# adityabalu/DiffNet

Measured on AMD Instinct MI355X. Metric: elements*gauss_pts/sec (FEM loss+grad), higher is better.
Workload: dtype f32; 1 GPU; 2-D Poisson energy loss + gradient wrt u, Q1, 512^2 nodes, 3^2 Gauss pts, batch 64/GPU, nu+f nodal fields, Dirichlet mask on all boundary faces held as one bit per node and sample (a general mask array), fused single pass (BASELINE.json configs[1] mesh); every step evaluates the next of 4 different batches in rotation (nu, f and the mask stream from HBM with non-temporal loads; of the 4 x 67 MB of; batch_per_gpu=64, parallelism=batch-sharded x1, batches_in_rotation=4, mask_format=bits

## Files before the change

### diffnet_amd/_lib.py

```python
import ctypes as C
import os

HERE = os.path.dirname(os.path.abspath(__file__))
LIB_PATH = os.environ.get("DN_LIB_PATH") or os.path.join(HERE, "libdiffnet_hip.so")
ABI_VERSION = 10

DN_E = {-1: "DN_E_BADARG", -2: "DN_E_UNSUPPORTED", -3: "DN_E_WORKSPACE", -4: "DN_E_HANDOVER"}


class DnMesh(C.Structure):
    _fields_ = [("nsd", C.c_int32), ("degree", C.c_int32), ("ngp", C.c_int32), ("batch", C.c_int32),
                ("nx", C.c_int32), ("ny", C.c_int32), ("nz", C.c_int32),
                ("scale", C.c_float * 3), ("gpw", C.c_float * 4),
                ("basis", (C.c_float * 4) * 4), ("dbasis", (C.c_float * 4) * 4)]


class DnDirichlet(C.Structure):
    _fields_ = [("mask", C.c_void_p), ("field", C.c_void_p), ("value", C.c_float),
                ("mask_kind", C.c_int32), ("mask_batched", C.c_int32), ("field_batched", C.c_int32),
                ("box_faces", C.c_int32), ("row_words", C.c_int32)]


MASK_F32, MASK_U8, MASK_BITS, MASK_BOX = 0, 1, 2, 3
FACE_XLO, FACE_XHI, FACE_YLO, FACE_YHI, FACE_ZLO, FACE_ZHI = 1, 2, 4, 8, 16, 32


class DnPoissonArgs(C.Structure):
    _fields_ = [("u", C.c_void_p), ("nu", C.c_void_p), ("f", C.c_void_p), ("f_gp", C.c_void_p),
                ("nu_batched", C.c_int32), ("f_batched", C.c_int32),
                ("bc", DnDirichlet * 2),
                ("alpha", C.c_float), ("beta", C.c_float), ("c", C.c_float), ("wscale", C.c_float),
                ("out_scale", C.c_float),
                ("out", C.c_void_p), ("energy", C.c_void_p), ("sumsq", C.c_void_p),
                ("workspace", C.c_void_p), ("workspace_bytes", C.c_int64),
                ("energy_f32", C.c_void_p), ("energy_scale", C.c_double), ("strip_select", C.c_int32), ("accumulate_sums", C.c_int32), ("defer_sums", C.c_int32),
                ("fold_prev", C.c_void_p), ("f_is_load", C.c_int32)]


class DnFsdtArgs(C.Structure):
    _fields_ = [("w", C.c_void_p), ("phi_x", C.c_void_p), ("phi_y", C.c_void_p),
                ("bc_mask", C.c_void_p), ("mask_is_u8", C.c_int32), ("mask_batched", C.c_int32),
                ("bc_field", C.c_void_p * 3), ("bc_field_batched", C.c_int32 * 3), ("bc_value", C.c_float * 3),
                ("D11", C.c_float), ("D12", C.c_float), ("D22", C.c_float), ("D66", C.c_float), ("A44", C.c_float),
                ("A55", C.c_float), ("q", C.c_float), ("wscale", C.c_float),
                ("out", C.c_void_p * 3), ("sumsq", C.c_void_p), ("workspace", C.c_void_p), ("workspace_bytes", C.c_int64),
                ("in_scale", C.c_void_p), ("norms", C.c_void_p), ("in_num", C.c_void_p), ("in_den", C.c_void_p),
                ("defer_sums", C.c_int32), ("den_ticket", C.c_int32), ("den_workspace", C.c_void_p)]


class DnStokesArgs(C.Structure):
    _fields_ = [("u", C.c_void_p), ("v", C.c_void_p), ("p", C.c_void_p),
                ("bc_mask", C.c_void_p * 3), ("mask_is_u8", C.c_int32 * 3), ("mask_batched", C.c_int32 * 3),
                ("bc_field", C.c_void_p * 3), ("bc_field_batched", C.c_int32 * 3), ("bc_value", C.c_float * 3),
                ("f_gp", C.c_void_p * 2), ("f_batched", C.c_int32 * 2), ("f_value", C.c_float * 2),
                ("visco", C.c_float), ("pspg", C.c_float), ("wscale", C.c_float), ("transpose", C.c_int32),
                ("out", C.c_void_p * 3), ("sumsq", C.c_void_p), ("norms", C.c_void_p), ("in_num", C.c_void_p), ("in_den", C.c_void_p),
                ("workspace", C.c_void_p), ("workspace_bytes", C.c_int64)]


class DnNsArgs(C.Structure):
    _fields_ = [("u", C.c_void_p), ("v", C.c_void_p), ("p", C.c_void_p),
                ("bc_mask", C.c_void_p * 3), ("mask_is_u8", C.c_int32 * 3), ("mask_batched", C.c_int32 * 3),
                ("bc_field", C.c_void_p * 3), ("bc_field_batched", C.c_int32 * 3), ("bc_value", C.c_float * 3),
                ("f_gp", C.c_void_p * 2), ("f_batched", C.c_int32 * 2), ("f_value", C.c_float * 2),
                ("visco", C.c_float), ("wscale", C.c_float), ("tau_h", C.c_float * 2), ("cinv", C.c_float), ("vjp", C.c_int32),
                ("cot", C.c_void_p * 3),
                ("out", C.c_void_p * 3), ("sumsq", C.c_void_p), ("norms", C.c_void_p), ("in_num", C.c_void_p), ("in_den", C.c_void_p),
                ("workspace", C.c_void_p), ("workspace_bytes", C.c_int64)]


class DnTransportArgs(C.Structure):
    _fields_ = [("u", C.c_void_p), ("nu", C.c_void_p), ("nu_batched", C.c_int32), ("r_first_wins", C.c_int32),
                ("bc_mask", C.c_void_p * 2), ("mask_is_u8", C.c_int32 * 2), ("mask_batched", C.c_int32 * 2),
                ("bc_field", C.c_void_p * 2), ("bc_field_batched", C.c_int32 * 2), ("bc_value", C.c_float * 2),
                ("f_gp", C.c_void_p), ("f_batched", C.c_int32), ("f_value", C.c_float),
                ("adv", C.c_float * 2), ("kappa", C.c_float * 2), ("tau", C.c_float), ("react", C.c_float * 4), ("wscale", C.c_float),
                ("vjp", C.c_int32),
                ("cot", C.c_void_p), ("out", C.c_void_p), ("sumsq", C.c_void_p), ("norm", C.c_void_p),
                ("in_num", C.c_void_p), ("in_den", C.c_void_p), ("workspace", C.c_void_p), ("workspace_bytes", C.c_int64)]


class DnStrongformArgs(C.Structure):
    _fields_ = [("u", C.c_void_p), ("f", C.c_void_p), ("f_gp", C.c_void_p), ("f_batched", C.c_int32), ("f_value", C.c_float),
                ("bc", DnDirichlet * 2),
                ("ax", C.c_float), ("ay", C.c_float), ("b", C.c_float), ("dxx", C.c_float), ("dyy", C.c_float), ("fs", C.c_float),
                ("wscale", C.c_float), ("out_scale", C.c_float), ("d2basis", (C.c_float * 4) * 4),
                ("in_scale", C.c_void_p), ("grad", C.c_void_p), ("sum", C.c_void_p), ("workspace", C.c_void_p), ("workspace_bytes", C.c_int64)]


class DnFoslsArgs(C.Structure):
    _fields_ = [("u", C.c_void_p), ("mx", C.c_void_p), ("my", C.c_void_p), ("field_stride", C.c_int64),
                ("nu", C.c_void_p), ("nu_batched", C.c_int32), ("nu_value", C.c_float),
                ("f", C.c_void_p), ("f_gp", C.c_void_p), ("f_batched", C.c_int32), ("f_value", C.c_float),
                ("bc", DnDirichlet * 2),
                ("wq", C.c_float), ("wd", C.c_float), ("fs", C.c_float), ("wscale", C.c_float), ("out_scale", C.c_float),
                ("in_scale", C.c_void_p), ("grad_u", C.c_void_p), ("grad_mx", C.c_void_p), ("grad_my", C.c_void_p), ("grad_stride", C.c_int64),
                ("sum", C.c_void_p), ("workspace", C.c_void_p), ("workspace_bytes", C.c_int64)]


class DnHelmholtzArgs(C.Structure):
    _fields_ = [("u", C.c_void_p), ("nu", C.c_void_p), ("sigma", C.c_void_p), ("f", C.c_void_p), ("f_gp", C.c_void_p),
                ("nu_batched", C.c_int32), ("sigma_batched", C.c_int32), ("f_batched", C.c_int32),
                ("sigma_value", C.c_float), ("f_value", C.c_float),
                ("bc", DnDirichlet * 2),
                ("c", C.c_float), ("cr", C.c_float), ("fs", C.c_float), ("alpha", C.c_float), ("gamma", C.c_float), ("beta", C.c_float),
                ("wscale", C.c_float), ("out_scale", C.c_float),
                ("out", C.c_void_p), ("energy", C.c_void_p), ("sumsq", C.c_void_p), ("workspace", C.c_void_p), ("workspace_bytes", C.c_int64)]


class DnEikonalArgs(C.Structure):
    _fields_ = [("u", C.c_void_p), ("bc", DnDirichlet * 2),
                ("f", C.c_void_p), ("f_gp", C.c_void_p), ("f_batched", C.c_int32), ("f_value", C.c_float),
                ("tau", C.c_float), ("sq", C.c_float), ("wscale", C.c_float), ("vjp", C.c_int32),
                ("cot", C.c_void_p), ("in_num", C.c_void_p), ("in_den", C.c_void_p),
                ("out", C.c_void_p), ("sumsq", C.c_void_p), ("norm", C.c_void_p), ("workspace", C.c_void_p), ("workspace_bytes", C.c_int64)]


class DnCoefGradArgs(C.Structure):
    _fields_ = [("u", C.c_void_p), ("v", C.c_void_p), ("bc", DnDirichlet * 2),
                ("a_nu", C.c_float), ("a_f", C.c_float), ("wscale", C.c_float),
                ("in_scale", C.c_void_p), ("g_nu", C.c_void_p), ("g_f", C.c_void_p)]


I32x3 = C.c_int32 * 3

SYMBOLS = {
    "dn_abi_version": (C.c_int, []),
    "dn_build_info": (C.c_char_p, []),
    "dn_config_set": (C.c_int, [C.c_char_p, C.c_char_p]),
    "dn_config_get": (C.c_char_p, [C.c_char_p]),
    "dn_probe_stream": (C.c_int, [C.c_void_p, C.c_void_p, C.c_void_p, C.c_void_p, C.c_int64, C.c_int32, C.c_void_p]),
    "dn_probe_march": (C.c_int, [C.c_void_p, C.c_void_p, C.c_void_p, C.c_void_p, C.c_int32, C.c_int32, C.c_int32, C.c_int32, C.c_int32, C.c_void_p]),
    "dn_probe_tile": (C.c_int, [C.c_void_p, C.c_void_p, C.c_void_p, C.c_void_p, C.c_int32, C.c_int32, C.c_int32, C.c_int32, C.c_int32, C.c_void_p]),
    "dn_poisson_workspace_bytes": (C.c_int64, [C.POINTER(DnMesh)]),
    "dn_poisson_apply": (C.c_int, [C.POINTER(DnMesh), C.POINTER(DnPoissonArgs), C.c_void_p]),
    "dn_poisson_finish_sums": (C.c_int, [C.POINTER(DnMesh), C.POINTER(DnPoissonArgs), C.c_void_p]),
    "dn_workspace_status": (C.c_int, [C.c_void_p, C.c_void_p]),
    "dn_gauss_pt_eval_fwd": (C.c_int, [C.c_void_p, C.c_void_p, C.c_void_p, C.c_int32, C.c_int32, I32x3, C.c_int32,
                                       C.c_int32, C.c_int32, C.c_void_p]),
    "dn_gauss_pt_eval_bwd": (C.c_int, [C.c_void_p, C.c_void_p, C.c_void_p, C.c_int32, C.c_int32, I32x3, C.c_int32,
                                       C.c_int32, C.c_int32, C.c_void_p]),
    "dn_assemble": (C.c_int, [C.c_void_p, C.c_void_p, C.c_int32, C.c_int32, I32x3, C.c_int32, C.c_int32, C.c_int32,
                              C.c_void_p]),
    "dn_assemble_bwd": (C.c_int, [C.c_void_p, C.c_void_p, C.c_int32, C.c_int32, I32x3, C.c_int32, C.c_int32,
                                  C.c_void_p]),
    "dn_fdm_stencil_fwd": (C.c_int, [C.c_void_p, C.c_void_p, C.c_int32, C.c_int32, C.c_int32, C.POINTER(C.c_float), C.c_int32,
                                     C.c_float, C.c_float, C.c_void_p]),
    "dn_fdm_stencil_bwd": (C.c_int, [C.c_void_p, C.c_void_p, C.c_int32, C.c_int32, C.c_int32, C.POINTER(C.c_float), C.c_int32,
                                     C.c_float, C.c_float, C.c_void_p]),
    "dn_fdm_fused_fwd": (C.c_int, [C.c_void_p, C.c_void_p, C.c_int32, C.c_int32, C.c_int32, C.POINTER(C.c_float), C.c_int32,
                                   C.c_float, C.c_float, C.c_void_p]),
    "dn_fdm_fused_bwd": (C.c_int, [C.c_void_p, C.c_void_p, C.c_int32, C.c_int32, C.c_int32, C.POINTER(C.c_float), C.c_int32,
                                   C.c_float, C.c_float, C.c_void_p]),
    "dn_fsdt_workspace_bytes": (C.c_int64, [C.POINTER(DnMesh)]),
    "dn_fsdt_apply": (C.c_int, [C.POINTER(DnMesh), C.POINTER(DnFsdtArgs), C.c_void_p]),
    "dn_stokes_workspace_bytes": (C.c_int64, [C.POINTER(DnMesh)]),
    "dn_stokes_apply": (C.c_int, [C.POINTER(DnMesh), C.POINTER(DnStokesArgs), C.c_void_p]),
    "dn_ns_workspace_bytes": (C.c_int64, [C.POINTER(DnMesh)]),
    "dn_ns_apply": (C.c_int, [C.POINTER(DnMesh), C.POINTER(DnNsArgs), C.c_void_p]),
    "dn_transport_workspace_bytes": (C.c_int64, [C.POINTER(DnMesh)]),
    "dn_transport_apply": (C.c_int, [C.POINTER(DnMesh), C.POINTER(DnTransportArgs), C.c_void_p]),
    "dn_strongform_workspace_bytes": (C.c_int64, [C.POINTER(DnMesh)]),
    "dn_strongform_apply": (C.c_int, [C.POINTER(DnMesh), C.POINTER(DnStrongformArgs), C.c_void_p]),
    "dn_fosls_workspace_bytes": (C.c_int64, [C.POINTER(DnMesh)]),
    "dn_fosls_apply": (C.c_int, [C.POINTER(DnMesh), C.POINTER(DnFoslsArgs), C.c_void_p]),
    "dn_helmholtz_workspace_bytes": (C.c_int64, [C.POINTER(DnMesh)]),
    "dn_helmholtz_apply": (C.c_int, [C.POINTER(DnMesh), C.POINTER(DnHelmholtzArgs), C.c_void_p]),
    "dn_eikonal_workspace_bytes": (C.c_int64, [C.POINTER(DnMesh)]),
    "dn_eikonal_apply": (C.c_int, [C.POINTER(DnMesh), C.POINTER(DnEikonalArgs), C.c_void_p]),
    "dn_eikonal3d_workspace_bytes": (C.c_int64, [C.POINTER(DnMesh)]),
    "dn_eikonal3d_apply": (C.c_int, [C.POINTER(DnMesh), C.POINTER(DnEikonalArgs), C.c_void_p]),
    "dn_poisson_coef_grad": (C.c_int, [C.POINTER(DnMesh), C.POINTER(DnCoefGradArgs), C.c_void_p]),
    "dn_upconv_out_workspace_bytes": (C.c_int64, [C.c_int64, C.c_int64, C.c_int64, C.c_int64]),
    "dn_upconv_out_fwd": (C.c_int, [C.c_void_p, C.c_void_p, C.c_void_p, C.c_void_p, C.c_int64, C.c_int64, C.c_int64, C.c_int64, C.c_int,
                                    C.c_void_p, C.c_int64, C.c_void_p]),
    "dn_upconv_out_bwd": (C.c_int, [C.c_void_p, C.c_void_p, C.c_void_p, C.c_void_p, C.c_void_p, C.c_void_p, C.c_void_p, C.c_int64,
                                    C.c_int64, C.c_int64, C.c_int64, C.c_int, C.c_void_p, C.c_int64, C.c_void_p]),
    "dn_upconv3d_out_workspace_bytes": (C.c_int64, [C.c_int64] * 5),
    "dn_upconv3d_out_fwd": (C.c_int, [C.c_void_p, C.c_void_p, C.c_void_p, C.c_void_p, C.c_int64, C.c_int64, C.c_int64, C.c_int64, C.c_int64,
                                      C.c_int, C.c_void_p, C.c_int64, C.c_void_p]),
    "dn_upconv3d_out_bwd": (C.c_int, [C.c_void_p, C.c_void_p, C.c_void_p, C.c_void_p, C.c_void_p, C.c_void_p, C.c_void_p, C.c_int64,
                                      C.c_int64, C.c_int64, C.c_int64, C.c_int64, C.c_int, C.c_void_p, C.c_int64, C.c_void_p]),
    "dn_conv3d_k4s2_wrw_workspace_bytes": (C.c_int64, [C.c_int64] * 6),
    "dn_conv3d_k4s2_wrw": (C.c_int, [C.c_void_p, C.c_void_p, C.c_void_p, C.c_int64, C.c_int64, C.c_int64, C.c_int64, C.c_int64, C.c_int64,
                                     C.c_void_p, C.c_int64, C.c_void_p]),
    "dn_conv2d_k4s2_down": (C.c_int, [C.c_void_p, C.c_void_p, C.c_void_p] + [C.c_int64] * 5 + [C.c_void_p]),
    "dn_conv2d_k4s2_up": (C.c_int, [C.c_void_p, C.c_void_p, C.c_void_p] + [C.c_int64] * 5 + [C.c_void_p]),
    "dn_conv2d_k4s2_wrw_workspace_bytes": (C.c_int64, [C.c_int64] * 5),
    "dn_conv2d_k4s2_wrw": (C.c_int, [C.c_void_p, C.c_void_p, C.c_void_p] + [C.c_int64] * 5 + [C.c_void_p, C.c_int64, C.c_void_p]),
    "dn_conv3d_k4s2_down": (C.c_int, [C.c_void_p, C.c_void_p, C.c_void_p] + [C.c_int64] * 6 + [C.c_void_p]),
    "dn_conv3d_k4s2_up": (C.c_int, [C.c_void_p, C.c_void_p, C.c_void_p] + [C.c_int64] * 6 + [C.c_void_p]),
    "dn_conv3d_k4s2_workspace_bytes": (C.c_int64, [C.c_int32] + [C.c_int64] * 6),
    "dn_conv3d_k4s2_down_ws": (C.c_int, [C.c_void_p, C.c_void_p, C.c_void_p] + [C.c_int64] * 6 + [C.c_void_p, C.c_int64, C.c_void_p]),
    "dn_conv3d_k4s2_up_ws": (C.c_int, [C.c_void_p, C.c_void_p, C.c_void_p] + [C.c_int64] * 6 + [C.c_void_p, C.c_int64, C.c_void_p]),
    "dn_conv2d_valid_fwd": (C.c_int, [C.c_void_p] * 4 + [C.c_int64] * 6 + [C.c_void_p]),
    "dn_conv2d_valid_bwd_data": (C.c_int, [C.c_void_p] * 3 + [C.c_int64] * 6 + [C.c_void_p]),
    "dn_conv2d_valid_bwd_weight": (C.c_int, [C.c_void_p] * 4 + [C.c_int64] * 6 + [C.c_void_p]),
    "dn_instnorm_workspace_bytes": (C.c_int64, [C.c_int64, C.c_int64]),
    "dn_instnorm_act_fwd": (C.c_int, [C.c_void_p, C.c_void_p, C.c_void_p, C.c_void_p, C.c_int64, C.c_int64, C.c_float, C.c_float,
                                      C.c_void_p, C.c_int64, C.c_void_p]),
    "dn_instnorm_act_bwd": (C.c_int, [C.c_void_p, C.c_void_p, C.c_void_p, C.c_void_p, C.c_void_p, C.c_int64, C.c_int64, C.c_float,
                                      C.c_int64, C.c_int64, C.c_void_p, C.c_int64, C.c_void_p]),
    "dn_pack_mask_bits": (C.c_int, [C.c_void_p, C.c_int32, C.c_int64, C.c_int32, C.c_int32, C.c_void_p, C.c_void_p]),
    "dn_unpack_mask_bits": (C.c_int, [C.c_void_p, C.c_int64, C.c_int32, C.c_int32, C.c_void_p, C.c_void_p]),
    "dn_winding_nodes": (C.c_int, [C.c_void_p, C.c_void_p, C.c_void_p, C.c_void_p, C.c_int32, C.c_int32, C.c_int32, C.c_int32,
                                   C.c_void_p]),
}

_LIB = None


class DiffNetHipError(RuntimeError):
    pass


def lib():
    global _LIB
    if _LIB is not None:
        return _LIB
    if not os.path.exists(LIB_PATH):
        raise DiffNetHipError(
            f"{LIB_PATH} is missing: build it with `python -m diffnet_amd.build` (hipcc, gfx950). "
            "There is no CPU fallback for the FEM hot path.")
    try:
        h = C.CDLL(LIB_PATH)
    except OSError as e:
        raise DiffNetHipError(f"cannot load {LIB_PATH}: {e}") from e
    for name, (res, args) in SYMBOLS.items():
        try:
            fn = getattr(h, name)
        except AttributeError as e:
            raise DiffNetHipError(f"{LIB_PATH} does not export {name}; rebuild it") from e
        fn.restype = res
        fn.argtypes = args
    v = h.dn_abi_version()
    if v != ABI_VERSION:
        raise DiffNetHipError(f"ABI mismatch: library {v}, binding {ABI_VERSION}")
    _LIB = h
    return h


_HIP = None


def hip_runtime():
    global _HIP
    if _HIP is None:
        path = next((ln.split()[-1] for ln in open("/proc/self/maps") if "libamdhip64.so" in ln), None)
        if path is None:
            raise DiffNetHipError("the HIP runtime is not loaded in this process (no GPU build of torch?)")
        h = C.CDLL(path)
        h.hipEventCreateWithFlags.argtypes = [C.POINTER(C.c_void_p), C.c_uint]
        h.hipEventRecord.argtypes = [C.c_void_p, C.c_void_p]
        h.hipStreamWaitEvent.argtypes = [C.c_void_p, C.c_void_p, C.c_uint]
        h.hipEventSynchronize.argtypes = [C.c_void_p]
        h.hipEventDestroy.argtypes = [C.c_void_p]
        _HIP = h
    return _HIP


def new_event():
    e = C.c_void_p()
    rc = hip_runtime().hipEventCreateWithFlags(C.byref(e), C.c_uint(0x2 | 0x20000000))
    if rc != 0:
        raise DiffNetHipError(f"hipEventCreateWithFlags: hipError_t {rc}")
    return e


def check(rc, what):
    if rc == 0:
        return
    if rc < 0:
        if rc == -4:
            raise DiffNetHipError(f"{what}: DN_E_HANDOVER (a chained-strip launch ran a bounded LDS hand-over poll to its limit: its results are NaN)")
        raise DiffNetHipError(f"{what}: {DN_E.get(rc, rc)} (argument not supported by the HIP kernels)")
    raise DiffNetHipError(f"{what}: hipError_t {rc}")


CONFIG_MIRROR = {k[3:]: v for k, v in os.environ.items() if k.startswith("DN_")}


def config_set(key, value):
    rc = lib().dn_config_set(key.encode(), (value or "").encode())
    if rc != 0:
        raise DiffNetHipError(f"dn_config_set: unknown switch {key!r} or value too long")
    CONFIG_MIRROR[key] = value or ""
    import sys
    ops = sys.modules.get(__package__ + ".ops")
    if ops is not None:
        ops.call_cache_clear()


def config_get(key):
    v = lib().dn_config_get(key.encode())
    if v is None:
        raise DiffNetHipError(f"dn_config_get: unknown switch {key!r}")
    return v.decode()
```

### diffnet_amd/csrc/dn_api.hip

```cpp
#include <cstdlib>
#include <cstring>

#include "dn_reduce.h"

#define DN_STR2(x) #x
#define DN_STR(x) DN_STR2(x)

extern "C" int dn_abi_version(void) { return DN_ABI_VERSION; }

extern "C" const char* dn_build_info(void) {
    return "libdiffnet_hip abi " DN_STR(DN_ABI_VERSION) " target gfx950 (CDNA4, wave64) hip " DN_STR(HIP_VERSION_MAJOR) "." DN_STR(
        HIP_VERSION_MINOR) " built " __DATE__;
}

namespace {
const char* const kKeys[dn::CFG_COUNT] = {"PLAN2D", "PLAN3D", "PLAN_FSDT", "Q1_RULE_KERNEL", "GPE_GATHER", "GPE_TILED", "Q1_3D_T16", "Q1_3D_E1SUM", "FSDT_GENERIC", "Q1_3D_E1", "HANDOVER_SPIN_LIMIT", "CONV2D_V1", "CONV_WRW_WGS", "Q1_3D_N2", "FSDT_FORM"};
constexpr int kHostCount = 1;
const char* const kHostKeys[kHostCount] = {"COEF_GRAD"};
constexpr int kAllCount = dn::CFG_COUNT + kHostCount;
char g_cfg[kAllCount][64];

const char* key_name(int k) { return k < dn::CFG_COUNT ? kKeys[k] : kHostKeys[k - dn::CFG_COUNT]; }

int key_index(const char* key) {
    if (!key) return -1;
    for (int k = 0; k < kAllCount; ++k)
        if (std::strcmp(key, key_name(k)) == 0) return k;
    return -1;
}

struct ConfigInit {
    ConfigInit() {
        for (int k = 0; k < kAllCount; ++k) {
            char name[80] = "DN_";
            std::strncat(name, key_name(k), sizeof(name) - 4);
            const char* e = std::getenv(name);
            g_cfg[k][0] = 0;
            if (e && std::strlen(e) < sizeof(g_cfg[k])) std::strcpy(g_cfg[k], e);
        }
    }
} g_cfg_init;
}

namespace dn {
const char* config(ConfigKey k) { return g_cfg[k][0] ? g_cfg[k] : nullptr; }
}

extern "C" int dn_config_set(const char* key, const char* value) {
    const int k = key_index(key);
    if (k < 0) return DN_E_BADARG;
    if (value && std::strlen(value) >= sizeof(g_cfg[k])) return DN_E_BADARG;
    g_cfg[k][0] = 0;
    if (value) std::strcpy(g_cfg[k], value);
    return 0;
}

extern "C" const char* dn_config_get(const char* key) {
    const int k = key_index(key);
    return k < 0 ? nullptr : g_cfg[k];
}

extern "C" int dn_workspace_status(void* workspace, void* stream) {
    if (!workspace) return DN_E_BADARG;
    hipStream_t s = reinterpret_cast<hipStream_t>(stream);
    unsigned* word = reinterpret_cast<unsigned*>(workspace) + dn::DN_WS_ERRWORD;
    unsigned v = 0u;
    hipError_t e = hipMemcpyAsync(&v, word, sizeof(v), hipMemcpyDeviceToHost, s);
    if (e == hipSuccess) e = hipStreamSynchronize(s);
    if (e != hipSuccess) return (int)e;
    if (v == 0u) return 0;
    e = hipMemsetAsync(word, 0, sizeof(v), s);
    if (e == hipSuccess) e = hipStreamSynchronize(s);
    if (e != hipSuccess) return (int)e;
    return DN_E_HANDOVER;
}

namespace dn {
__global__ void __launch_bounds__(256) pack_mask_bits_kernel(const void* __restrict__ mask, int is_u8, long long rows, int nx, int row_words,
                                                             uint32_t* __restrict__ bits) {
    const long long w = (long long)blockIdx.x * blockDim.x + threadIdx.x;
    if (w >= rows * row_words) return;
    const long long row = w / row_words;
    const int x0 = (int)(w % row_words) * 32;
    uint32_t v = 0u;
    for (int i = 0; i < 32 && x0 + i < nx; ++i) {
        const long long idx = row * nx + x0 + i;
        const bool set = is_u8 ? reinterpret_cast<const uint8_t*>(mask)[idx] != 0 : reinterpret_cast<const float*>(mask)[idx] > 0.5f;
        v |= set ? (1u << i) : 0u;
    }
    bits[w] = v;
}
__global__ void __launch_bounds__(256) unpack_mask_bits_kernel(const uint32_t* __restrict__ bits, long long rows, int nx, int row_words,
                                                               uint8_t* __restrict__ mask) {
    const long long i = (long long)blockIdx.x * blockDim.x + threadIdx.x;
    if (i >= rows * nx) return;
    const long long row = i / nx;
    const int x = (int)(i % nx);
    mask[i] = (uint8_t)((bits[row * row_words + (x >> 5)] >> (x & 31)) & 1u);
}
}

extern "C" int dn_pack_mask_bits(const void* mask, int32_t mask_kind, int64_t rows, int32_t nx, int32_t row_words, uint32_t* bits, void* stream) {
    if (!mask || !bits || rows < 0 || nx < 1 || row_words < (nx + 31) / 32 || (mask_kind != DN_MASK_F32 && mask_kind != DN_MASK_U8)) return DN_E_BADARG;
    const long long n = (long long)rows * row_words;
    if (n == 0) return 0;
    if ((n + 255) / 256 >= (1ll << 31)) return DN_E_UNSUPPORTED;
    hipLaunchKernelGGL(dn::pack_mask_bits_kernel, dim3((unsigned)((n + 255) / 256)), dim3(256), 0, reinterpret_cast<hipStream_t>(stream), mask,
                       (int)(mask_kind == DN_MASK_U8), (long long)rows, (int)nx, (int)row_words, bits);
    DN_LAUNCH_CHECK();
    return 0;
}

extern "C" int dn_unpack_mask_bits(const uint32_t* bits, int64_t rows, int32_t nx, int32_t row_words, uint8_t* mask_u8, void* stream) {
    if (!mask_u8 || !bits || rows < 0 || nx < 1 || row_words < (nx + 31) / 32) return DN_E_BADARG;
    const long long n = (long long)rows * nx;
    if (n == 0) return 0;
    if ((n + 255) / 256 >= (1ll << 31)) return DN_E_UNSUPPORTED;
    hipLaunchKernelGGL(dn::unpack_mask_bits_kernel, dim3((unsigned)((n + 255) / 256)), dim3(256), 0, reinterpret_cast<hipStream_t>(stream), bits,
                       (long long)rows, (int)nx, (int)row_words, mask_u8);
    DN_LAUNCH_CHECK();
    return 0;
}
```

### diffnet_amd/csrc/dn_common.h

```cpp
#pragma once
#include <hip/hip_runtime.h>
#include <stdint.h>

#include "../../include/diffnet_hip.h"

#define DN_WAVE 64

#define DN_LAUNCH_CHECK()                         \
    do {                                          \
        hipError_t e__ = hipGetLastError();       \
        if (e__ != hipSuccess) return (int)e__;   \
    } while (0)

namespace dn {

enum ConfigKey : int { CFG_PLAN2D = 0, CFG_PLAN3D, CFG_PLAN_FSDT, CFG_Q1_RULE_KERNEL, CFG_GPE_GATHER, CFG_GPE_TILED, CFG_Q1_3D_T16, CFG_Q1_3D_E1SUM, CFG_FSDT_GENERIC, CFG_Q1_3D_E1, CFG_HANDOVER_SPIN_LIMIT, CFG_CONV2D_V1, CFG_CONV_WRW_WGS, CFG_Q1_3D_N2, CFG_FSDT_FORM, CFG_COUNT };
const char* config(ConfigKey k);

__device__ __forceinline__ double wave_sum(double v) {
#pragma unroll
    for (int off = DN_WAVE / 2; off > 0; off >>= 1) v += __shfl_down(v, off, DN_WAVE);
    return v;
}

__device__ __forceinline__ double block_sum(double v, double* scratch, int tid, int nthreads) {
    v = wave_sum(v);
    const int lane = tid & (DN_WAVE - 1), wave = tid / DN_WAVE;
    if (lane == 0) scratch[wave] = v;
    __syncthreads();
    double r = 0.0;
    if (tid == 0) {
        const int nw = (nthreads + DN_WAVE - 1) / DN_WAVE;
        for (int w = 0; w < nw; ++w) r += scratch[w];
    }
    __syncthreads();
    return r;
}

__device__ __forceinline__ void block_sum2(double& a, double& b, double* scratch, int tid, int nthreads) {
    a = wave_sum(a);
    b = wave_sum(b);
    const int lane = tid & (DN_WAVE - 1), wave = tid / DN_WAVE;
    const int nw = (nthreads + DN_WAVE - 1) / DN_WAVE;
    if (lane == 0) { scratch[wave] = a; scratch[nw + wave] = b; }
    __syncthreads();
    double ra = 0.0, rb = 0.0;
    if (tid == 0) {
        for (int w = 0; w < nw; ++w) { ra += scratch[w]; rb += scratch[nw + w]; }
    }
    __syncthreads();
    a = ra; b = rb;
}

template <int N>
struct VecT;
template <>
struct VecT<1> { using type = float; };
template <>
struct VecT<2> { using type = float2; };
template <>
struct VecT<4> { using type = float4; };

#ifndef DN_NT_STORES
#define DN_NT_STORES 0
#endif
template <typename V, typename T>
__device__ __forceinline__ V ld_at(const T* __restrict__ base, unsigned index) {
    return *reinterpret_cast<const V*>(reinterpret_cast<const char*>(base) + (index * (unsigned)sizeof(T)));
}
template <typename V, typename T>
__device__ __forceinline__ void st_at(T* __restrict__ base, unsigned index, const V& v) {
#if DN_NT_STORES
    char* a = reinterpret_cast<char*>(base) + (index * (unsigned)sizeof(T));
    if constexpr (sizeof(V) == 16) {
        typedef float v4f __attribute__((ext_vector_type(4)));
        __builtin_nontemporal_store(__builtin_bit_cast(v4f, v), reinterpret_cast<v4f*>(a));
    } else if constexpr (sizeof(V) == 8) {
        typedef float v2f __attribute__((ext_vector_type(2)));
        __builtin_nontemporal_store(__builtin_bit_cast(v2f, v), reinterpret_cast<v2f*>(a));
    } else {
        __builtin_nontemporal_store(v, reinterpret_cast<V*>(a));
    }
#else
    *reinterpret_cast<V*>(reinterpret_cast<char*>(base) + (index * (unsigned)sizeof(T))) = v;
#endif
}

template <int NW, bool VEC, typename T>
__device__ __forceinline__ void load_seg(const T* __restrict__ base, unsigned rowoff, int x0, int nx, T (&dst)[NW + 1]) {
    if constexpr (VEC && (NW == 2 || NW == 4)) {
        const unsigned xl = (unsigned)min(x0, nx - NW);
        if constexpr (sizeof(T) == 4) {
            using V = typename VecT<NW>::type;
            const V v = ld_at<V>(base, rowoff + xl);
            const T* vf = reinterpret_cast<const T*>(&v);
#pragma unroll
            for (int k = 0; k < NW; ++k) dst[k] = vf[k];
        } else {
            static_assert(sizeof(T) == 1, "load_seg: 1- or 4-byte elements");
            if constexpr (NW == 4) {
                const uint32_t w = ld_at<uint32_t>(base, rowoff + xl);
#pragma unroll
                for (int k = 0; k < 4; ++k) dst[k] = (T)((w >> (8 * k)) & 0xffu);
            } else {
                const uint16_t w = ld_at<uint16_t>(base, rowoff + xl);
                dst[0] = (T)(w & 0xffu);
                dst[1] = (T)(w >> 8);
            }
        }
    } else {
#pragma unroll
        for (int k = 0; k < NW; ++k) dst[k] = ld_at<T>(base, rowoff + (unsigned)min(x0 + k, nx - 1));
    }
    dst[NW] = ld_at<T>(base, rowoff + (unsigned)min(x0 + NW, nx - 1));
}

template <int NW, bool VEC, typename T>
__device__ __forceinline__ void load_seg_stream(const T* __restrict__ base, unsigned rowoff, int x0, int nx, T (&dst)[NW + 1]) {
    if constexpr (VEC && NW == 4 && sizeof(T) == 4) {
        typedef T v4t __attribute__((ext_vector_type(4)));
        const unsigned xl = (unsigned)min(x0, nx - NW);
        const v4t v = __builtin_nontemporal_load(reinterpret_cast<const v4t*>(reinterpret_cast<const char*>(base) + (rowoff + xl) * 4u));
        dst[0] = v.x; dst[1] = v.y; dst[2] = v.z; dst[3] = v.w;
        dst[NW] = ld_at<T>(base, rowoff + (unsigned)min(x0 + NW, nx - 1));
    } else if constexpr (VEC && NW == 4 && sizeof(T) == 1) {
        const unsigned xl = (unsigned)min(x0, nx - NW);
        const uint32_t w = __builtin_nontemporal_load(reinterpret_cast<const uint32_t*>(reinterpret_cast<const char*>(base) + (rowoff + xl)));
#pragma unroll
        for (int k = 0; k < 4; ++k) dst[k] = (T)((w >> (8 * k)) & 0xffu);
        dst[NW] = ld_at<T>(base, rowoff + (unsigned)min(x0 + NW, nx - 1));
    } else {
        load_seg<NW, VEC>(base, rowoff, x0, nx, dst);
    }
}

template <int NW, bool VEC, typename T>
__device__ __forceinline__ void load_own(const T* __restrict__ base, unsigned rowoff, int x0, int nx, T (&dst)[NW]) {
    if constexpr (VEC && (NW == 2 || NW == 4)) {
        const unsigned xl = (unsigned)min(x0, nx - NW);
        if constexpr (sizeof(T) == 4) {
            using V = typename VecT<NW>::type;
            const V v = ld_at<V>(base, rowoff + xl);
            const T* vf = reinterpret_cast<const T*>(&v);
#pragma unroll
            for (int k = 0; k < NW; ++k) dst[k] = vf[k];
        } else {
            if constexpr (NW == 4) {
                const uint32_t w = ld_at<uint32_t>(base, rowoff + xl);
#pragma unroll
                for (int k = 0; k < 4; ++k) dst[k] = (T)((w >> (8 * k)) & 0xffu);
            } else {
                const uint16_t w = ld_at<uint16_t>(base, rowoff + xl);
                dst[0] = (T)(w & 0xffu);
                dst[1] = (T)(w >> 8);
            }
        }
    } else {
#pragma unroll
        for (int k = 0; k < NW; ++k) dst[k] = ld_at<T>(base, rowoff + (unsigned)min(x0 + k, nx - 1));
    }
}

template <int NW, bool VEC>
__device__ __forceinline__ void store_seg(float* __restrict__ base, unsigned rowoff, int x0, int nx, const float (&src)[NW]) {
    if constexpr (VEC && (NW == 2 || NW == 4)) {
        if (x0 + NW <= nx) {
            using V = typename VecT<NW>::type;
            V v;
            float* vf = reinterpret_cast<float*>(&v);
#pragma unroll
            for (int k = 0; k < NW; ++k) vf[k] = src[k];
            st_at<V>(base, rowoff + (unsigned)x0, v);
        }
    } else {
#pragma unroll
        for (int k = 0; k < NW; ++k)
            if (x0 + k < nx) st_at<float>(base, rowoff + (unsigned)(x0 + k), src[k]);
    }
}

}
```

### diffnet_amd/csrc/poisson2d_q1_cf.hip

```cpp
#include <cstdlib>
#include <type_traits>

#define DN_NT_STORES 1
#include "poisson_common.h"

namespace dn {

enum : int { CF_NU = 1, CF_F = 2, CF_BC = 8, CF_BC_U8C = 16, CF_BC_PACKED = 32, CF_PK_NB1 = 64, CF_PK_NB2 = 128, CF_UA = 256, CF_ONE = 512 };

template <int E>
struct CfRow {
    float u[E + 1], n[E + 1], f[E + 1];
    float g[E + 1];
    float du[E], pn[E];
    float keep[E];
    float keepx;
    BcRaw<E> bc;
    uint32_t m8[2][2];
    uint32_t mb[2];
    uint32_t bx[2];
};

constexpr int CF_W = 4;
constexpr int CF_TS = 128;
constexpr int CF_NSLOT = 64;
constexpr unsigned CF_SPIN_MAX = 1u << 20;

__device__ __forceinline__ unsigned lds_addr(const void* p) { return (unsigned)(uintptr_t)(__attribute__((address_space(3))) const void*)p; }
__device__ __forceinline__ void lds_st(unsigned a, float v) { asm volatile("ds_write_b32 %0, %1" ::"v"(a), "v"(v) : "memory"); }
__device__ __forceinline__ void lds_st(unsigned a, unsigned v) { asm volatile("ds_write_b32 %0, %1" ::"v"(a), "v"(v) : "memory"); }
__device__ __forceinline__ void lds_ld_nowait(float& d, unsigned a) { asm volatile("ds_read_b32 %0, %1" : "=v"(d) : "v"(a) : "memory"); }
__device__ __forceinline__ unsigned lds_ld_u(unsigned a) {
    unsigned d;
    asm volatile("ds_read_b32 %0, %1\n\ts_waitcnt lgkmcnt(0)" : "=v"(d) : "v"(a) : "memory");
    return d;
}
__device__ __forceinline__ float lds_ld(unsigned a) {
    float d;
    asm volatile("ds_read_b32 %0, %1\n\ts_waitcnt lgkmcnt(0)" : "=v"(d) : "v"(a) : "memory");
    return d;
}
template <int N>
__device__ __forceinline__ void lds_wait(float (&v)[N]) {
    if constexpr (N == 5) asm volatile("s_waitcnt lgkmcnt(0)" : "+v"(v[0]), "+v"(v[1]), "+v"(v[2]), "+v"(v[3]), "+v"(v[4])::"memory");
    else if constexpr (N == 4) asm volatile("s_waitcnt lgkmcnt(0)" : "+v"(v[0]), "+v"(v[1]), "+v"(v[2]), "+v"(v[3])::"memory");
    else if constexpr (N == 3) asm volatile("s_waitcnt lgkmcnt(0)" : "+v"(v[0]), "+v"(v[1]), "+v"(v[2])::"memory");
    else if constexpr (N == 2) asm volatile("s_waitcnt lgkmcnt(0)" : "+v"(v[0]), "+v"(v[1])::"memory");
    else { static_assert(N == 1, "lds_wait: 1..5 values"); asm volatile("s_waitcnt lgkmcnt(0)" : "+v"(v[0])::"memory"); }
}

template <int E, bool VEC, int FL, int W>
__global__ void __launch_bounds__(W > 1 ? CF_TS * W : 256, W > 1 ? 4 : 2) poisson2d_q1_cf_kernel(const PoissonParams p) {
    constexpr int NW = E;
    constexpr bool HAS_NU = (FL & CF_NU) != 0, HAS_F = (FL & CF_F) != 0;
    constexpr bool BC_ANY = (FL & (CF_BC | CF_BC_U8C | CF_BC_PACKED)) != 0, BC_U8C = (FL & CF_BC_U8C) != 0, BC_PACKED = (FL & CF_BC_PACKED) != 0;
    constexpr bool UA = (FL & CF_UA) != 0, ONE = (FL & CF_ONE) != 0;
    static_assert(!ONE || ((BC_PACKED || BC_U8C) && (FL & CF_PK_NB2) == 0), "CF_ONE: one packed or uint8-constant condition");
    static_assert(!UA || (E == 4 && VEC && W == 1), "CF_UA: four elements per thread, vector accesses, one strip per workgroup");
    const int T = W > 1 ? CF_TS : (int)blockDim.x;
    const int sub = W > 1 ? __builtin_amdgcn_readfirstlane((int)threadIdx.x / CF_TS) : 0;
    const int tid = W > 1 ? (int)threadIdx.x - sub * CF_TS : (int)threadIdx.x;
    const int chunk = blockIdx.x, strip = W > 1 ? (int)blockIdx.y * W + sub : selected_strip(p, (int)blockIdx.y), b = blockIdx.z;
    const bool active = W == 1 || strip < p.nstrips;
    const bool chain_dn = W > 1 && sub > 0;
    const bool chain_up = W > 1 && sub + 1 < W && strip + 1 < p.nstrips;
    const int q = chunk * (T - 1) + tid;
    const int ex0 = q * E;
    const int x0 = ex0;
    const bool col_owner = !(chunk > 0 && tid == 0);
    const bool lastcol = UA && x0 + NW == p.nx - 1;
    const int64_t nps = (int64_t)p.nx * p.ny;
    const SampleBases sb = sample_bases(p, b, nps);
    const int R = p.rows_per_strip;
    const int sb0 = strip * R, sc0 = min(sb0 + R, p.nely);
    const int ey_begin = (sb0 > 0 && !chain_dn) ? sb0 - 1 : sb0;
    const int ey_end = sc0;
    const int r_from = sb0;
    const int e_from = sb0, e_until = p.nely;
    const bool top_row = sc0 == p.nely;

    __shared__ float xch[2][256];
    __shared__ double red[W > 1 ? 4 * W : 8];
    __shared__ int last_flag;
    constexpr int CW = W > 1 ? W : 2, SEAM_WORDS = 6 * (E + 1);
    __shared__ float cf_edge[W > 1 ? W : 1][W > 1 ? CF_NSLOT : 1];
    __shared__ unsigned cf_xflag[W > 1 ? W : 1];
    __shared__ float cf_seam[CW - 1][W > 1 ? SEAM_WORDS : 1][W > 1 ? CF_TS : 1];
    __shared__ unsigned cf_sflag[CW - 1][2][2];
    const int lane = tid & 63, wv = __builtin_amdgcn_readfirstlane(tid >> 6);
    unsigned seq = 0u;
    if constexpr (W > 1) {
        static_assert(CF_TS == 128, "two waves per sub-strip");
        if (threadIdx.x < (unsigned)W) cf_xflag[threadIdx.x] = 0u;
        if (threadIdx.x < 4u * (W - 1)) (&cf_sflag[0][0][0])[threadIdx.x] = 0u;
        __syncthreads();
    }
    if ((blockIdx.x | blockIdx.y | blockIdx.z) == 0u) fold_prev_sums(p, (int)threadIdx.x, (int)blockDim.x, red);
    float spin_poison = 0.f;
    auto spin_until = [&](const unsigned* flag, unsigned want) {
        const unsigned fa = lds_addr(flag);
        const unsigned lim = p.spin_limit > 0 ? (unsigned)p.spin_limit : CF_SPIN_MAX;
        unsigned n = 0;
        for (; n < lim; ++n) {
            if ((unsigned)__builtin_amdgcn_readfirstlane((int)lds_ld_u(fa)) >= want) break;
            __builtin_amdgcn_s_sleep(1);
        }
        if (n == lim) spin_poison = __builtin_nanf("");
    };

    const bool has_mask[2] = {sb.mask[0] != nullptr, sb.mask[1] != nullptr};
    const uint8_t* mask8[2];
    mask8[0] = reinterpret_cast<const uint8_t*>(has_mask[0] ? sb.mask[0] : sb.mask[1]);
    mask8[1] = reinterpret_cast<const uint8_t*>(has_mask[1] ? sb.mask[1] : sb.mask[0]);

    constexpr unsigned NBITS = (1u << (NW + 1)) - 1u;
    constexpr int NB = !BC_PACKED ? 0 : ((FL & CF_PK_NB2) ? 2 : ((FL & CF_PK_NB1) ? 1 : 0));
    const bool isbits[2] = {p.bc[0].kind == DN_MASK_BITS, p.bc[1].kind == DN_MASK_BITS};
    const unsigned bsel[2] = {isbits[0] ? NBITS : 0u, isbits[1] ? NBITS : 0u};
    const int src0 = (NB == 2 || isbits[0]) ? 0 : 1;
    const int kone = p.bc[0].kind >= 0 ? 0 : 1;
    const uint32_t* bptr[2] = {reinterpret_cast<const uint32_t*>(sb.mask[src0]), reinterpret_cast<const uint32_t*>(sb.mask[1])};
    const unsigned brow[2] = {(unsigned)p.bc[src0].row_bytes / 4u, (unsigned)p.bc[1].row_bytes / 4u};
    unsigned bw0[2], bw1[2];
#pragma unroll
    for (int j = 0; j < 2; ++j) {
        const int rw = max((int)brow[j], 1);
        bw0[j] = (unsigned)min(x0 >> 5, rw - 1);
        bw1[j] = (unsigned)min((x0 >> 5) + 1, rw - 1);
    }
    const unsigned bsh = (unsigned)x0 & 31u;
    unsigned boxx[2] = {0u, 0u};
#pragma unroll
    for (int k = 0; k < 2; ++k) {
        const int faces = p.bc[k].kind == DN_MASK_BOX ? p.bc[k].box_faces : 0;
#pragma unroll
        for (int n = 0; n <= NW; ++n) {
            const bool on = ((faces & DN_FACE_XLO) && x0 + n == 0) || ((faces & DN_FACE_XHI) && x0 + n == p.nx - 1);
            boxx[k] |= on ? (1u << n) : 0u;
        }
    }
    const int ylo[2] = {(p.bc[0].kind == DN_MASK_BOX && (p.bc[0].box_faces & DN_FACE_YLO)) ? 0 : -1,
                        (p.bc[1].kind == DN_MASK_BOX && (p.bc[1].box_faces & DN_FACE_YLO)) ? 0 : -1};
    const int yhi[2] = {(p.bc[0].kind == DN_MASK_BOX && (p.bc[0].box_faces & DN_FACE_YHI)) ? p.ny - 1 : -1,
                        (p.bc[1].kind == DN_MASK_BOX && (p.bc[1].box_faces & DN_FACE_YHI)) ? p.ny - 1 : -1};
    auto packed_issue = [&](int yc, CfRow<E>& r) {
#pragma unroll
        for (int j = 0; j < NB; ++j) {
            const unsigned ro = (unsigned)yc * brow[j];
            const uint32_t w0 = ld_at<uint32_t>(bptr[j], ro + bw0[j]), w1 = ld_at<uint32_t>(bptr[j], ro + bw1[j]);
            r.mb[j] = __builtin_amdgcn_alignbit(w1, w0, bsh);
        }
        if constexpr (ONE) {
            if constexpr (NB == 0) r.bx[0] = (yc == (kone ? ylo[1] : ylo[0]) || yc == (kone ? yhi[1] : yhi[0])) ? NBITS : (kone ? boxx[1] : boxx[0]);
        } else {
#pragma unroll
            for (int k = 0; k < 2; ++k) r.bx[k] = (yc == ylo[k] || yc == yhi[k]) ? NBITS : boxx[k];
        }
    };

    auto row_issue = [&](int yr, CfRow<E>& r) {
        const int yp = min(yr, p.ny - 1);
        const unsigned rowoff = (unsigned)yp * (unsigned)p.nx;
        load_seg<NW, VEC>(sb.u, rowoff, x0, p.nx, r.u);
        if constexpr (HAS_NU) load_seg_stream<NW, VEC>(sb.nu, rowoff, x0, p.nx, r.n);
        if constexpr (HAS_F) load_seg_stream<NW, VEC>(sb.f, rowoff, x0, p.nx, r.f);
        if constexpr (BC_PACKED) {
            packed_issue(yp, r);
        } else if constexpr (BC_U8C && ONE) {
            uint8_t t[NW + 1];
            load_seg_stream<NW, VEC>(mask8[0], rowoff, x0, p.nx, t);
            uint32_t w = 0u;
#pragma unroll
            for (int n = 0; n < NW; ++n) w |= (uint32_t)t[n] << (8 * n);
            r.m8[0][0] = w;
            r.m8[0][1] = t[NW];
        } else if constexpr (BC_U8C) {
#pragma unroll
            for (int k = 0; k < 2; ++k) {
                if (has_mask[k]) {
                    uint8_t t[NW + 1];
                    load_seg_stream<NW, VEC>(mask8[k], rowoff, x0, p.nx, t);
                    uint32_t w = 0u;
#pragma unroll
                    for (int n = 0; n < NW; ++n) w |= (uint32_t)t[n] << (8 * n);
                    r.m8[k][0] = w;
                    r.m8[k][1] = t[NW];
                }
            }
        } else if constexpr (BC_ANY) {
            bc_issue<NW, VEC>(p, sb, rowoff, x0, r.bc);
        }
    };
    auto row_bc = [&](CfRow<E>& r) {
#pragma unroll
        for (int n = 0; n < NW; ++n) r.keep[n] = 1.f;
        if constexpr (UA) r.keepx = 1.f;
        if constexpr ((BC_PACKED || BC_U8C) && ONE) {
            const float v = kone ? p.bc[1].value : p.bc[0].value;
            unsigned b = 0u;
            if constexpr (BC_PACKED) b = NB == 1 ? r.mb[0] : r.bx[0];
#pragma unroll
            for (int n = 0; n <= NW; ++n) {
                bool set;
                if constexpr (BC_PACKED) set = (b & (1u << n)) != 0u;
                else set = n < NW ? ((r.m8[0][0] >> (8 * n)) & 0xffu) != 0u : r.m8[0][1] != 0u;
                r.u[n] = set ? v : r.u[n];
                if (n < NW) r.keep[n] = set ? 0.f : 1.f;
                else if constexpr (UA) r.keepx = set ? 0.f : 1.f;
            }
        } else if constexpr (BC_PACKED) {
            unsigned b0 = r.bx[0], b1 = r.bx[1];
            if constexpr (NB == 2) { b0 |= r.mb[0] & bsel[0]; b1 |= r.mb[1] & bsel[1]; }
            if constexpr (NB == 1) { b0 |= r.mb[0] & bsel[0]; b1 |= r.mb[0] & bsel[1]; }
            const float v0 = p.bc[0].value, v1 = p.bc[1].value;
#pragma unroll
            for (int n = 0; n <= NW; ++n) {
                r.u[n] = (b0 & (1u << n)) ? v0 : r.u[n];
                r.u[n] = (b1 & (1u << n)) ? v1 : r.u[n];
                if (n < NW) r.keep[n] = ((b0 | b1) & (1u << n)) ? 0.f : 1.f;
            }
            if constexpr (UA) r.keepx = ((b0 | b1) & (1u << NW)) ? 0.f : 1.f;
        } else if constexpr (BC_U8C) {
#pragma unroll
            for (int k = 0; k < 2; ++k) {
                if (has_mask[k]) {
                    const float val = p.bc[k].value;
#pragma unroll
                    for (int n = 0; n <= NW; ++n) {
                        const bool set = has_mask[k] && (n < NW ? ((r.m8[k][0] >> (8 * n)) & 0xffu) != 0u : r.m8[k][1] != 0u);
                        r.u[n] = set ? val : r.u[n];
                        if (n < NW) r.keep[n] = set ? 0.f : r.keep[n];
                        else if constexpr (UA) r.keepx = set ? 0.f : r.keepx;
                    }
                }
            }
        } else if constexpr (BC_ANY) {
            if constexpr (UA) {
                float k5[NW + 1];
                bc_apply_all<NW>(p, sb, r.bc, r.u, k5);
#pragma unroll
                for (int n = 0; n < NW; ++n) r.keep[n] = k5[n];
                r.keepx = k5[NW];
            } else {
                bc_apply<NW>(p, sb, r.bc, r.u, r.keep);
            }
        }
    };

    float e1_acc = 0.f, e2_acc = 0.f, sq_acc = 0.f;
    int par = 0;

    float pend_v[NW];
    unsigned pend_row = 0u;
    bool pend_st = false;
    float pend_x = 0.f;
    auto flush_store = [&]() {
        if (pend_st) store_seg<NW, VEC>(sb.out, pend_row, x0, p.nx, pend_v);
        if constexpr (UA) {
            if (pend_st && lastcol) st_at<float>(sb.out, pend_row + (unsigned)(p.nx - 1), pend_x);
        }
        pend_st = false;
    };
    auto emit_row = [&](const float (&o)[NW + 1], const float (&keep)[NW], int yr, bool owned_row, float keepx = 1.f) {
        float left;
        if constexpr (W > 1) {
            const float up = __shfl_up(o[NW], 1, 64);
            const unsigned ea = lds_addr(&cf_edge[sub][seq & (CF_NSLOT - 1)]);
            float edge = 0.f;
            if (wv == 0) {
                if (lane == 63) { lds_st(ea, o[NW]); lds_st(lds_addr(&cf_xflag[sub]), seq + 1u); }
            } else {
                spin_until(&cf_xflag[sub], seq + 1u);
                edge = lds_ld(ea);
            }
            left = lane > 0 ? up : edge;
            ++seq;
        } else {
            xch[par][tid] = o[NW];
            asm volatile("s_waitcnt lgkmcnt(0)\n\ts_barrier" ::: "memory");
            left = (tid > 0) ? xch[par][tid - 1] : 0.f;
            par ^= 1;
        }
        const bool st = owned_row && col_owner && (!UA || x0 + NW <= p.nx - 1);
#pragma unroll
        for (int n = 0; n < NW; ++n) {
            const float t = (o[n] + (n == 0 ? left : 0.f)) * keep[n];
            sq_acc = st ? fmaf(t, t, sq_acc) : sq_acc;
            pend_v[n] = t * p.out_scale;
            if constexpr (W > 1) pend_v[n] += spin_poison;
        }
        if constexpr (UA) {
            const float t = o[NW] * keepx;
            sq_acc = (st && lastcol) ? fmaf(t, t, sq_acc) : sq_acc;
            pend_x = t * p.out_scale;
        }
        pend_row = (unsigned)yr * (unsigned)p.nx;
        pend_st = st && sb.out != nullptr;
        flush_store();
    };

    const float mx0 = p.T.mxs[0], mx1 = p.T.mxs[1], mx2 = p.T.mxs[2], mx3 = p.T.mxs[3];
    const float my0 = p.T.m[0], my1 = p.T.m[1], my2 = p.T.m[2], my3 = p.T.m[3];
    const float k0 = p.T.q1c[0], k1 = p.T.q1c[1], h0 = p.T.q1c[2], h1 = p.T.q1c[3], nb = -p.T.beta;
    constexpr bool ROWSTAGED = (FL & CF_BC) == 0, STAGE_DU = W == 1;
    const float xm[4] = {p.T.q1xm[0], p.T.q1xm[1], p.T.q1xm[2], p.T.q1xm[3]}, ym[4] = {p.T.q1ym[0], p.T.q1ym[1], p.T.q1ym[2], p.T.q1ym[3]};
    const float px0 = p.T.q1px[0], px1 = p.T.q1px[1], sy0 = p.T.q1sy[0], sy1 = p.T.q1sy[1];

    constexpr bool FMASS = HAS_F && ROWSTAGED;
    const float cx00 = p.T.q1mx[0], cx01 = p.T.q1mx[1], cx11 = p.T.q1mx[2], cy00 = p.T.q1my[0], cy01 = p.T.q1my[1], cy11 = p.T.q1my[2];
    const float alpha = p.T.alpha;
    auto fstage = [&](CfRow<E>& r) {
        if constexpr (FMASS) {
#pragma unroll
            for (int n = 0; n <= NW; ++n) r.g[n] = 0.f;
#pragma unroll
            for (int e = 0; e < E; ++e) {
                if (ex0 + e < p.nelx) {
                    r.g[e] = fmaf(cx01, r.f[e + 1], fmaf(cx00, r.f[e], r.g[e]));
                    r.g[e + 1] = fmaf(cx11, r.f[e + 1], cx01 * r.f[e]);
                }
            }
        }
    };

    auto sstage = [&](CfRow<E>& r) {
        if constexpr (ROWSTAGED) {
#pragma unroll
            for (int e = 0; e < E; ++e) {
                if constexpr (HAS_NU) {
                    q1cf_stage(px0, px1, r.u[e], r.u[e + 1], r.n[e], r.n[e + 1], r.du[e], r.pn[e]);
                } else {
                    r.du[e] = r.u[e + 1] - r.u[e];
                    r.pn[e] = mx0;
                }
            }
        }
    };

    auto layer = [&](auto fresh, int ey, const CfRow<E>& L, CfRow<E>& U, const float (&cin)[NW + 1], float (&cout)[NW + 1]) {
        const bool own_layer = ey >= e_from && ey <= e_until;
        const float cnt = (own_layer && col_owner) ? 1.f : 0.f;
        if constexpr (decltype(fresh)::value) { row_bc(U); fstage(U); }
        sstage(U);
        float o[NW + 1], le1 = 0.f, le2 = 0.f;
#pragma unroll
        for (int n = 0; n <= NW; ++n) { o[n] = cin[n]; cout[n] = 0.f; }
        if constexpr (FMASS) {
#pragma unroll
            for (int n = 0; n <= NW; ++n) {
                const float tlo = fmaf(cy01, U.g[n], cy00 * L.g[n]), tup = fmaf(cy11, U.g[n], cy01 * L.g[n]);
                o[n] = fmaf(nb, tlo, o[n]);
                cout[n] = nb * tup;
                le2 = fmaf(U.u[n], tup, fmaf(L.u[n], tlo, le2));
            }
        }
        if constexpr (ROWSTAGED) {
            float V[NW + 1], S[NW + 1];
#pragma unroll
            for (int n = 0; n <= NW; ++n) {
                V[n] = U.u[n] - L.u[n];
                S[n] = HAS_NU ? fmaf(sy1, U.n[n], sy0 * L.n[n]) : my0;
            }
#pragma unroll
            for (int e = 0; e < E; ++e) {
                if (ex0 + e < p.nelx) {
                    const float a = STAGE_DU ? L.du[e] : L.u[e + 1] - L.u[e], b = STAGE_DU ? U.du[e] : U.u[e + 1] - U.u[e];
                    q1cf_elem(xm, ym, a, b, L.pn[e], U.pn[e], V[e], V[e + 1], S[e], S[e + 1], alpha, o[e], o[e + 1], cout[e], cout[e + 1], le1);
                }
            }
        } else {
#pragma unroll
            for (int e = 0; e < E; ++e) {
                if (ex0 + e < p.nelx) {
                    const float U0 = L.u[e], UX = L.u[e + 1] - L.u[e], UY = U.u[e] - L.u[e], UXY = (U.u[e + 1] - U.u[e]) - UX;
                    float P = mx0, Q = 0.f, Pp = my0, Qp = 0.f;
                    if constexpr (HAS_NU) {
                        const float N0 = L.n[e], NX = L.n[e + 1] - N0, NY = U.n[e] - N0, NXY = (U.n[e + 1] - U.n[e]) - NX;
                        P = fmaf(mx1, NX, mx0 * N0);
                        Q = fmaf(mx1, NXY, mx0 * NY);
                        Pp = fmaf(my1, NY, my0 * N0);
                        Qp = fmaf(my1, NXY, my0 * NX);
                    }
                    const float A0 = fmaf(Q, my1, P * my0), A1 = fmaf(Q, my2, P * my1), A2 = fmaf(Q, my3, P * my2);
                    const float B0 = fmaf(Qp, mx1, Pp * mx0), B1 = fmaf(Qp, mx2, Pp * mx1), B2 = fmaf(Qp, mx3, Pp * mx2);
                    const float tX0 = fmaf(UXY, A1, UX * A0), tX1 = fmaf(UXY, A2, UX * A1);
                    const float tY0 = fmaf(UXY, B1, UY * B0), tY1 = fmaf(UXY, B2, UY * B1);
                    le1 += fmaf(h1, fmaf(UXY, tY1, UY * tY0), h0 * fmaf(UXY, tX1, UX * tX0));
                    float cU0 = 0.f, cUX = k0 * tX0, cUY = k1 * tY0, cUXY = fmaf(k0, tX1, k1 * tY1);
                    if constexpr (HAS_F) {
                        const float F0 = L.f[e], FX = L.f[e + 1] - F0, FY = U.f[e] - F0, FXY = (U.f[e + 1] - U.f[e]) - FX;
                        const float S0 = fmaf(mx1, FX, mx0 * F0), S1 = fmaf(mx1, FXY, mx0 * FY);
                        const float T0 = fmaf(mx2, FX, mx1 * F0), T1 = fmaf(mx2, FXY, mx1 * FY);
                        const float L0 = fmaf(my1, S1, my0 * S0), LX = fmaf(my1, T1, my0 * T0);
                        const float LY = fmaf(my2, S1, my1 * S0), LXY = fmaf(my2, T1, my1 * T0);
                        le2 += fmaf(LXY, UXY, fmaf(LY, UY, fmaf(LX, UX, L0 * U0)));
                        cU0 = nb * L0;
                        cUX = fmaf(nb, LX, cUX);
                        cUY = fmaf(nb, LY, cUY);
                        cUXY = fmaf(nb, LXY, cUXY);
                    }
                    const float g01 = cUX - cUXY, g10 = cUY - cUXY;
                    o[e] += (cU0 - cUX) - g10;
                    o[e + 1] += g01;
                    cout[e] += g10;
                    cout[e + 1] += cUXY;
                }
            }
        }
        e1_acc = fmaf(cnt, le1, e1_acc);
        e2_acc = fmaf(cnt, le2, e2_acc);
        if (W > 1 && chain_dn && ey == sb0) {
            const unsigned s0 = lds_addr(&cf_seam[W > 1 ? sub - 1 : 0][0][tid]);
#pragma unroll
            for (int n = 0; n <= NW; ++n) lds_st(s0 + (4 * NW + 4 + n) * CF_TS * 4, o[n]);
#pragma unroll
            for (int n = 0; n < NW; ++n) lds_st(s0 + (5 * NW + 5 + n) * CF_TS * 4, L.keep[n]);
        } else {
            emit_row(o, L.keep, ey, ey >= r_from, L.keepx);
        }
    };
    auto publish_row = [&](const CfRow<E>& r) {
        const unsigned s0 = lds_addr(&cf_seam[W > 1 ? sub - 1 : 0][0][tid]);
#pragma unroll
        for (int n = 0; n <= NW; ++n) {
            lds_st(s0 + n * CF_TS * 4, r.u[n]);
            if constexpr (HAS_NU) lds_st(s0 + (NW + 1 + n) * CF_TS * 4, r.n[n]);
            if constexpr (FMASS) lds_st(s0 + (2 * NW + 2 + n) * CF_TS * 4, r.g[n]);
            else if constexpr (HAS_F) lds_st(s0 + (2 * NW + 2 + n) * CF_TS * 4, r.f[n]);
        }
        if (lane == 0) lds_st(lds_addr(&cf_sflag[W > 1 ? sub - 1 : 0][0][wv]), 1u);
    };
    auto fetch_row = [&](CfRow<E>& r) {
        spin_until(&cf_sflag[sub][0][wv], 1u);
        const unsigned s0 = lds_addr(&cf_seam[sub][0][tid]);
#pragma unroll
        for (int n = 0; n <= NW; ++n) lds_ld_nowait(r.u[n], s0 + n * CF_TS * 4);
        lds_wait(r.u);
        if constexpr (HAS_NU) {
#pragma unroll
            for (int n = 0; n <= NW; ++n) lds_ld_nowait(r.n[n], s0 + (NW + 1 + n) * CF_TS * 4);
            lds_wait(r.n);
        }
        if constexpr (FMASS) {
#pragma unroll
            for (int n = 0; n <= NW; ++n) lds_ld_nowait(r.g[n], s0 + (2 * NW + 2 + n) * CF_TS * 4);
            lds_wait(r.g);
        } else if constexpr (HAS_F) {
#pragma unroll
            for (int n = 0; n <= NW; ++n) lds_ld_nowait(r.f[n], s0 + (2 * NW + 2 + n) * CF_TS * 4);
            lds_wait(r.f);
        }
    };
    auto publish_carry = [&](const float (&c)[NW + 1]) {
        const unsigned s0 = lds_addr(&cf_seam[sub][0][tid]);
#pragma unroll
        for (int n = 0; n <= NW; ++n) lds_st(s0 + (3 * NW + 3 + n) * CF_TS * 4, c[n]);
        if (lane == 0) lds_st(lds_addr(&cf_sflag[sub][1][wv]), 1u);
    };

    auto set_prio = [&](int e) {
        switch (((ey_end - e) >> 1) & 3) {
            case 0: __builtin_amdgcn_s_setprio(0); break;
            case 1: __builtin_amdgcn_s_setprio(1); break;
            case 2: __builtin_amdgcn_s_setprio(2); break;
            default: __builtin_amdgcn_s_setprio(3); break;
        }
    };

    constexpr std::true_type FRESH{};
    constexpr std::false_type LANDED{};
    if (active) {
    CfRow<E> RA, RB;
    float carryA[NW + 1], carryB[NW + 1];
#pragma unroll
    for (int n = 0; n <= NW; ++n) carryA[n] = carryB[n] = 0.f;
    row_issue(ey_begin, RA);
    row_bc(RA);
    fstage(RA);
    sstage(RA);
    if constexpr (W > 1) {
        if (chain_dn) publish_row(RA);
    }
    int ey = ey_begin;
    bool odd = false;
    const int n_main = chain_up ? ey_end - 1 : ey_end;
    for (; ey + 1 < n_main; ey += 2) {
        set_prio(ey);
        row_issue(ey + 1, RB);
        layer(FRESH, ey, RA, RB, carryA, carryB);
        row_issue(ey + 2, RA);
        layer(FRESH, ey + 1, RB, RA, carryB, carryA);
    }
    if (ey < n_main) {
        set_prio(ey);
        row_issue(ey + 1, RB);
        layer(FRESH, ey, RA, RB, carryA, carryB);
        odd = true;
        ++ey;
    }
    if constexpr (W > 1) {
        if (chain_up) {
            __builtin_amdgcn_s_setprio(0);
            if (odd) { fetch_row(RA); layer(LANDED, ey, RB, RA, carryB, carryA); publish_carry(carryA); }
            else { fetch_row(RB); layer(LANDED, ey, RA, RB, carryA, carryB); publish_carry(carryB); }
        }
    }
    if (top_row) {
        float o[NW + 1], keep[NW];
#pragma unroll
        for (int n = 0; n <= NW; ++n) o[n] = odd ? carryB[n] : carryA[n];
#pragma unroll
        for (int n = 0; n < NW; ++n) keep[n] = odd ? RB.keep[n] : RA.keep[n];
        emit_row(o, keep, p.ny - 1, true, odd ? RB.keepx : RA.keepx);
        flush_store();
    }
    if constexpr (W > 1) {
        if (chain_dn) {
            spin_until(&cf_sflag[sub - 1][1][wv], 1u);
            const unsigned s0 = lds_addr(&cf_seam[sub - 1][0][tid]);
            float o[NW + 1], cy[NW + 1], keep[NW];
#pragma unroll
            for (int n = 0; n <= NW; ++n) lds_ld_nowait(o[n], s0 + (4 * NW + 4 + n) * CF_TS * 4);
            lds_wait(o);
#pragma unroll
            for (int n = 0; n <= NW; ++n) lds_ld_nowait(cy[n], s0 + (3 * NW + 3 + n) * CF_TS * 4);
            lds_wait(cy);
#pragma unroll
            for (int n = 0; n < NW; ++n) lds_ld_nowait(keep[n], s0 + (5 * NW + 5 + n) * CF_TS * 4);
            lds_wait(keep);
#pragma unroll
            for (int n = 0; n <= NW; ++n) o[n] += cy[n];
            emit_row(o, keep, sb0, true);
            flush_store();
        }
    }
    }

    if constexpr (W > 1) {
        e1_acc += spin_poison;
        sq_acc += spin_poison;
        if (spin_poison != spin_poison && p.counter != nullptr && (threadIdx.x & 63u) == 0u) atomicOr(p.counter + DN_WS_ERRWORD, 1u);
    }
    if (p.want_sums) finish_sums(p, e1_acc, e2_acc, sq_acc, (int)threadIdx.x, (int)blockDim.x, red, &last_flag);
}

template <int E, bool VEC, int FL>
static void cf_launch_one(const PoissonParams& pp, const Geom2D& g, int batch, hipStream_t s) {
    if constexpr (E == 4 && VEC && (FL & CF_UA) == 0) {
        if (g.W == CF_W) {
            hipLaunchKernelGGL((poisson2d_q1_cf_kernel<E, VEC, FL, CF_W>), dim3(g.chunks, (g.strips + CF_W - 1) / CF_W, batch),
                               dim3(CF_TS * CF_W), 0, s, pp);
            return;
        }
    }
    hipLaunchKernelGGL((poisson2d_q1_cf_kernel<E, VEC, FL, 1>), dim3(g.chunks, g.strips, batch), dim3(g.T), 0, s, pp);
}

template <int E, bool VEC, int UAF = 0>
static void cf_launch_flags(const PoissonParams& pp, const Geom2D& g, int batch, hipStream_t s) {
    const bool any = pp.bc[0].kind >= 0 || pp.bc[1].kind >= 0;
    bool u8c = any, packed = false;
    for (int k = 0; k < 2; ++k) {
        if (pp.bc[k].kind >= 0 && (!pp.bc[k].mask_is_u8 || pp.bc[k].field)) u8c = false;
        if (pp.bc[k].kind == DN_MASK_BITS || pp.bc[k].kind == DN_MASK_BOX) packed = true;
    }
    const int nbits = (pp.bc[0].kind == DN_MASK_BITS) + (pp.bc[1].kind == DN_MASK_BITS);
    const bool one = (pp.bc[0].kind >= 0) != (pp.bc[1].kind >= 0);
    const int nf = (pp.nu ? CF_NU : 0) | (pp.f ? CF_F : 0);
#define DN_CF(FLAGS)                                                                         \
    (!any ? cf_launch_one<E, VEC, (FLAGS) | UAF>(pp, g, batch, s)                                  \
          : packed ? (nbits == 2 ? cf_launch_one<E, VEC, (FLAGS) | UAF | CF_BC_PACKED | CF_PK_NB2>(pp, g, batch, s)          \
                     : nbits == 1 ? (one ? cf_launch_one<E, VEC, (FLAGS) | UAF | CF_BC_PACKED | CF_PK_NB1 | CF_ONE>(pp, g, batch, s)        \
                                         : cf_launch_one<E, VEC, (FLAGS) | UAF | CF_BC_PACKED | CF_PK_NB1>(pp, g, batch, s))        \
                     : one ? cf_launch_one<E, VEC, (FLAGS) | UAF | CF_BC_PACKED | CF_ONE>(pp, g, batch, s)                   \
                           : cf_launch_one<E, VEC, (FLAGS) | UAF | CF_BC_PACKED>(pp, g, batch, s))                   \
          : u8c ? (one ? cf_launch_one<E, VEC, (FLAGS) | UAF | CF_BC_U8C | CF_ONE>(pp, g, batch, s)                \
                       : cf_launch_one<E, VEC, (FLAGS) | UAF | CF_BC_U8C>(pp, g, batch, s))                \
                : cf_launch_one<E, VEC, (FLAGS) | UAF | CF_BC>(pp, g, batch, s))
    switch (nf) {
        case 0: DN_CF(0); break;
        case CF_NU: DN_CF(CF_NU); break;
        case CF_F: DN_CF(CF_F); break;
        default: DN_CF(CF_NU | CF_F); break;
    }
#undef DN_CF
}

int poisson2d_q1_cf_chain() { return CF_W; }

int launch_poisson2d_q1_cf(const PoissonParams& pp, const Geom2D& g, int batch, bool vec, hipStream_t s) {
    if (g.W > 1 && !(g.W == poisson2d_q1_cf_chain() && g.E == 4 && vec && g.T == CF_TS && g.R + 3 <= CF_NSLOT)) return DN_E_BADARG;
    if (g.ua) {
        if (g.E != 4 || g.W != 1 || (pp.nx & 3) != 1 || pp.nx < 9) return DN_E_BADARG;
        cf_launch_flags<4, true, CF_UA>(pp, g, batch, s);
        return 0;
    }
    if (g.E == 4 && vec) { cf_launch_flags<4, true>(pp, g, batch, s); return 0; }
    if (g.E == 2 && vec) { cf_launch_flags<2, true>(pp, g, batch, s); return 0; }
    if (g.E == 2) { cf_launch_flags<2, false>(pp, g, batch, s); return 0; }
    return DN_E_UNSUPPORTED;
}

}
```

### diffnet_amd/csrc/poisson_common.h

```cpp
#pragma once
#include "dn_reduce.h"
#include "poisson_elem.h"

namespace dn {

struct DirichletDev {
    const void* mask;
    const float* field;
    float value;
    int mask_is_u8, mask_batched, field_batched;
    int kind;
    int box_faces;
    int row_bytes;
};

struct PoissonParams {
    ElemTab T;
    const float* u;
    const float* nu;
    const float* f;
    const float* fgp;
    int nu_batched, f_batched;
    int f_is_load;
    DirichletDev bc[2];
    float out_scale;
    float* out;
    double* part_energy;
    double* part_sumsq;
    unsigned* counter;
    double* energy;
    double* sumsq;
    float* energy_f32;
    double energy_scale;
    int nx, ny, nz;
    int nelx, nely, nelz;
    int rows_per_strip;
    int nstrips;
    int strip_sel;
    int acc_sums;
    int defer_sums;
    int want_sums;
    const double* fold_pe;
    const double* fold_ps;
    double* fold_energy;
    double* fold_sumsq;
    float* fold_energy_f32;
    double fold_scale;
    int fold_n, fold_acc;
    int spin_limit;
};

__device__ __forceinline__ void write_sums(double e, double s, int acc, double* energy, double* sumsq, float* energy_f32, double energy_scale) {
    if (acc) { e += *energy; s += *sumsq; }
    if (energy) *energy = e;
    if (sumsq) *sumsq = s;
    if (energy_f32) *energy_f32 = (float)(e * energy_scale);
}

__device__ __forceinline__ int selected_strip(const PoissonParams& p, int idx) {
    return p.strip_sel == 1 ? (idx == 0 ? 0 : p.nstrips - 1) : (p.strip_sel == 2 ? idx + 1 : idx);
}

struct SampleBases {
    const float* u;
    const float* nu;
    const float* f;
    float* out;
    const void* mask[2];
    const float* field[2];
};

__device__ __forceinline__ SampleBases sample_bases(const PoissonParams& p, int b, int64_t nps) {
    SampleBases s;
    s.u = p.u + (int64_t)b * nps;
    s.nu = p.nu ? p.nu + (p.nu_batched ? (int64_t)b * nps : 0) : nullptr;
    s.f = p.f ? p.f + (p.f_batched ? (int64_t)b * nps : 0) : nullptr;
    s.out = p.out ? p.out + (int64_t)b * nps : nullptr;
#pragma unroll
    for (int k = 0; k < 2; ++k) {
        const DirichletDev& d = p.bc[k];
        const int64_t mo = d.mask_batched ? (int64_t)b * nps : 0;
        if (d.kind == DN_MASK_BITS)
            s.mask[k] = reinterpret_cast<const uint8_t*>(d.mask) + (d.mask_batched ? (int64_t)b * ((int64_t)p.ny * p.nz) * d.row_bytes : 0);
        else
            s.mask[k] = d.mask ? (d.mask_is_u8 ? (const void*)(reinterpret_cast<const uint8_t*>(d.mask) + mo)
                                               : (const void*)(reinterpret_cast<const float*>(d.mask) + mo))
                               : nullptr;
        s.field[k] = d.field ? d.field + (d.field_batched ? (int64_t)b * nps : 0) : nullptr;
    }
    return s;
}

template <int NW, bool VEC>
__device__ __forceinline__ unsigned load_apply_bc(const PoissonParams& p, const SampleBases& sb, unsigned rowoff, int x0,
                                                  float (&u)[NW + 1]) {
    uint8_t m8[2][NW + 1];
    float mf[2][NW + 1], fv[2][NW + 1];
#pragma unroll
    for (int k = 0; k < 2; ++k) {
        if (sb.mask[k] != nullptr) {
            if (p.bc[k].mask_is_u8) load_seg<NW, VEC>(reinterpret_cast<const uint8_t*>(sb.mask[k]), rowoff, x0, p.nx, m8[k]);
            else load_seg<NW, VEC>(reinterpret_cast<const float*>(sb.mask[k]), rowoff, x0, p.nx, mf[k]);
            if (sb.field[k]) load_seg<NW, VEC>(sb.field[k], rowoff, x0, p.nx, fv[k]);
        }
    }
    unsigned bits = 0u;
#pragma unroll
    for (int k = 0; k < 2; ++k) {
        if (sb.mask[k] != nullptr) {
            unsigned kb = 0u;
            if (p.bc[k].mask_is_u8) {
#pragma unroll
                for (int n = 0; n <= NW; ++n) kb |= (m8[k][n] != 0) ? (1u << n) : 0u;
            } else {
#pragma unroll
                for (int n = 0; n <= NW; ++n) kb |= (mf[k][n] > 0.5f) ? (1u << n) : 0u;
            }
            if (sb.field[k]) {
#pragma unroll
                for (int n = 0; n <= NW; ++n) u[n] = (kb & (1u << n)) ? fv[k][n] : u[n];
            } else {
                const float val = p.bc[k].value;
#pragma unroll
                for (int n = 0; n <= NW; ++n) u[n] = (kb & (1u << n)) ? val : u[n];
            }
            bits |= kb;
        }
    }
    return bits;
}

__device__ __forceinline__ void finish_sums(const PoissonParams& p, float e1, float e2, float sq, int tid, int nthreads,
                                            double* red, int* flag, double escale = 1.0) {
    double mine[2] = {escale * ((double)p.T.c * (double)e1 - (double)e2), (double)sq}, tot[2];
    block_sum2(mine[0], mine[1], red, tid, nthreads);
    double* const part[2] = {p.part_energy, p.part_sumsq};
    if (p.defer_sums) {
        if (tid == 0) store_partials<2, false>(part, workgroup_index(), mine);
        return;
    }
    if (!last_arriver_sums<2, 16, true, false>(part, p.counter, mine, tid, nthreads, flag, tot)) return;
    block_sum2(tot[0], tot[1], red, tid, nthreads);
    if (tid == 0) {
        write_sums(tot[0], tot[1], p.acc_sums, p.energy, p.sumsq, p.energy_f32, p.energy_scale);
        arrival_reset(p.counter);
    }
}

__device__ __forceinline__ void fold_prev_sums(const PoissonParams& p, int tid, int nthreads, double* red) {
    if (p.fold_n <= 0) return;
    const double* const part[2] = {p.fold_pe, p.fold_ps};
    double tot[2];
    sum_partials<2, 16, false, false>(part, p.fold_n, tid, nthreads, tot);
    block_sum2(tot[0], tot[1], red, tid, nthreads);
    if (tid == 0) write_sums(tot[0], tot[1], p.fold_acc, p.fold_energy, p.fold_sumsq, p.fold_energy_f32, p.fold_scale);
}

template <int NW>
struct BcRaw {
    uint32_t m[2][NW + 1];
    float fv[2][NW + 1];
};

template <int NW, bool VEC>
__device__ __forceinline__ void bc_issue(const PoissonParams& p, const SampleBases& sb, unsigned rowoff, int x0, BcRaw<NW>& r) {
#pragma unroll
    for (int k = 0; k < 2; ++k) {
        if (sb.mask[k] != nullptr) {
            if (p.bc[k].mask_is_u8) {
                uint8_t t[NW + 1];
                load_seg_stream<NW, VEC>(reinterpret_cast<const uint8_t*>(sb.mask[k]), rowoff, x0, p.nx, t);
#pragma unroll
                for (int n = 0; n <= NW; ++n) r.m[k][n] = t[n];
            } else {
                load_seg_stream<NW, VEC>(reinterpret_cast<const uint32_t*>(sb.mask[k]), rowoff, x0, p.nx, r.m[k]);
            }
            if (sb.field[k]) load_seg<NW, VEC>(sb.field[k], rowoff, x0, p.nx, r.fv[k]);
        }
    }
}

template <int NW>
__device__ __forceinline__ void bc_apply_all(const PoissonParams& p, const SampleBases& sb, const BcRaw<NW>& r, float (&u)[NW + 1],
                                             float (&keep)[NW + 1]) {
#pragma unroll
    for (int n = 0; n <= NW; ++n) keep[n] = 1.f;
#pragma unroll
    for (int k = 0; k < 2; ++k) {
        if (sb.mask[k] != nullptr) {
            const bool u8 = p.bc[k].mask_is_u8 != 0;
            const bool hasf = sb.field[k] != nullptr;
            const float val = p.bc[k].value;
#pragma unroll
            for (int n = 0; n <= NW; ++n) {
                const bool set = u8 ? (r.m[k][n] != 0u) : (__uint_as_float(r.m[k][n]) > 0.5f);
                u[n] = set ? (hasf ? r.fv[k][n] : val) : u[n];
                keep[n] = set ? 0.f : keep[n];
            }
        }
    }
}

template <int NW>
__device__ __forceinline__ void bc_apply(const PoissonParams& p, const SampleBases& sb, const BcRaw<NW>& r, float (&u)[NW + 1],
                                         float (&keep)[NW]) {
    float k[NW + 1];
    bc_apply_all<NW>(p, sb, r, u, k);
#pragma unroll
    for (int n = 0; n < NW; ++n) keep[n] = k[n];
}

template <int N, bool VEC>
__device__ __forceinline__ void bc_nodes(const PoissonParams& p, const SampleBases& sb, unsigned rowoff, int x0, float (&u)[N],
                                         float (&keep)[N]) {
    uint32_t m[2][N];
    float fv[2][N];
#pragma unroll
    for (int k = 0; k < 2; ++k) {
        if (sb.mask[k] != nullptr) {
            if (p.bc[k].mask_is_u8) {
                uint8_t t[N];
                load_own<N, VEC>(reinterpret_cast<const uint8_t*>(sb.mask[k]), rowoff, x0, p.nx, t);
#pragma unroll
                for (int n = 0; n < N; ++n) m[k][n] = t[n];
            } else {
                load_own<N, VEC>(reinterpret_cast<const uint32_t*>(sb.mask[k]), rowoff, x0, p.nx, m[k]);
            }
            if (sb.field[k]) load_own<N, VEC>(sb.field[k], rowoff, x0, p.nx, fv[k]);
        }
    }
#pragma unroll
    for (int n = 0; n < N; ++n) keep[n] = 1.f;
#pragma unroll
    for (int k = 0; k < 2; ++k) {
        if (sb.mask[k] != nullptr) {
            const bool u8 = p.bc[k].mask_is_u8 != 0;
            const bool hasf = sb.field[k] != nullptr;
            const float val = p.bc[k].value;
#pragma unroll
            for (int n = 0; n < N; ++n) {
                const bool set = u8 ? (m[k][n] != 0u) : (__uint_as_float(m[k][n]) > 0.5f);
                u[n] = set ? (hasf ? fv[k][n] : val) : u[n];
                keep[n] = set ? 0.f : keep[n];
            }
        }
    }
}

struct Geom2D { int T, E, chunks, strips, R, W = 1; bool ua = false; };
struct Geom3D { int TX, TY, E, chunks, tiles, strips, R; };

int launch_poisson2d_q1_g2(const PoissonParams& pp, const Geom2D& g, int batch, bool vec, hipStream_t s);
int launch_poisson2d_q1_g3(const PoissonParams& pp, const Geom2D& g, int batch, bool vec, hipStream_t s);
int launch_poisson2d_q1_g4(const PoissonParams& pp, const Geom2D& g, int batch, bool vec, hipStream_t s);
int launch_poisson2d_q1_cf(const PoissonParams& pp, const Geom2D& g, int batch, bool vec, hipStream_t s);
int poisson2d_q1_cf_chain();
int launch_poisson3d_q1_g2(const PoissonParams& pp, const Geom3D& g, int batch, bool vec, hipStream_t s);
int launch_poisson3d_q1_g3(const PoissonParams& pp, const Geom3D& g, int batch, bool vec, hipStream_t s);
int launch_poisson3d_q1_g4(const PoissonParams& pp, const Geom3D& g, int batch, bool vec, hipStream_t s);

bool poisson3d_q1_cf_ok(const PoissonParams& pp);
int launch_poisson3d_q1_cf(const PoissonParams& pp, const Geom3D& g, int batch, hipStream_t s);

void gen3d_layout(const dn_mesh* m, long long& n1, long long& n2, long long& elem_floats);
int launch_poisson3d_gen(const PoissonParams& pp, const dn_mesh* m, void* workspace, int64_t workspace_bytes, hipStream_t s);

}
```

### diffnet_amd/csrc/poisson_elem.h

```cpp
#pragma once
#include "dn_common.h"

namespace dn {

typedef float v2f __attribute__((ext_vector_type(2)));
__device__ __forceinline__ float vfma(float a, float b, float c) { return fmaf(a, b, c); }
__device__ __forceinline__ v2f vfma(v2f a, v2f b, v2f c) { return __builtin_elementwise_fma(a, b, c); }
__device__ __forceinline__ v2f vfma(float a, v2f b, v2f c) { return __builtin_elementwise_fma((v2f)(a), b, c); }

struct ElemTab {
    float b[4][4];
    float dx[4][4];
    float dy[4][4];
    float dz[4][4];
    float w[4];
    float wx[4];
    float w2[4][4];
    float hs[3];
    float ahs[3];
    float alpha, beta, c;
    float m[4];
    float mxs[4];
    float kx[3][4];
    float q1c[4];
    float wb[4];
    float kap[3];
    float hs2[3];
    float m01, m12;
    float esc;
    float nbw;
    float q1mx[3], q1my[3];
    float q1xm[4];
    float q1ym[4];
    float q1px[2];
    float q1sy[2];
};

template <int P, int NGP, bool FGP>
__device__ __forceinline__ void elem2d(const ElemTab& T, const float (&u)[P + 1][P + 1], const float (&nu)[P + 1][P + 1],
                                       const float (&f)[P + 1][P + 1], const float* fg, float (&g)[P + 1][P + 1],
                                       float& e1, float& e2) {
    constexpr int NB = P + 1;
    float a1 = 0.f, a2 = 0.f;
    static_assert(P >= 2, "Q1 elements run through the marching kernels (q1_layer_2d / q1_layer_3d)");
#pragma unroll
    for (int jb = 0; jb < NB; ++jb)
#pragma unroll
        for (int ib = 0; ib < NB; ++ib) g[jb][ib] = 0.f;
#pragma unroll
    for (int ig = 0; ig < NGP; ++ig) {
        float tv[NB], td[NB], tn[NB], tf[NB], rv[NB], rd[NB];
#pragma unroll
        for (int jb = 0; jb < NB; ++jb) {
            float a = 0.f, d = 0.f, n = 0.f, q = 0.f;
#pragma unroll
            for (int ib = 0; ib < NB; ++ib) {
                a = fmaf(T.b[ig][ib], u[jb][ib], a);
                d = fmaf(T.dx[ig][ib], u[jb][ib], d);
                n = fmaf(T.b[ig][ib], nu[jb][ib], n);
                if constexpr (!FGP) q = fmaf(T.b[ig][ib], f[jb][ib], q);
            }
            tv[jb] = a; td[jb] = d; tn[jb] = n; tf[jb] = q; rv[jb] = 0.f; rd[jb] = 0.f;
        }
#pragma unroll
        for (int jg = 0; jg < NGP; ++jg) {
            float val = 0.f, ux = 0.f, uy = 0.f, nuv = 0.f, fv = 0.f;
#pragma unroll
            for (int jb = 0; jb < NB; ++jb) {
                val = fmaf(T.b[jg][jb], tv[jb], val);
                ux = fmaf(T.b[jg][jb], td[jb], ux);
                uy = fmaf(T.dy[jg][jb], tv[jb], uy);
                nuv = fmaf(T.b[jg][jb], tn[jb], nuv);
                if constexpr (!FGP) fv = fmaf(T.b[jg][jb], tf[jb], fv);
            }
            if constexpr (FGP) fv = fg[jg * NGP + ig];
            const float Wn = T.w2[jg][ig] * nuv, Wf = T.w2[jg][ig] * fv;
            a1 = fmaf(Wn, ux * ux + uy * uy, a1);
            a2 = fmaf(Wf, val, a2);
            const float qx = T.alpha * Wn * ux, qy = T.alpha * Wn * uy, qv = -T.beta * Wf;
#pragma unroll
            for (int jb = 0; jb < NB; ++jb) {
                rv[jb] = fmaf(T.b[jg][jb], qv, rv[jb]);
                rv[jb] = fmaf(T.dy[jg][jb], qy, rv[jb]);
                rd[jb] = fmaf(T.b[jg][jb], qx, rd[jb]);
            }
        }
#pragma unroll
        for (int jb = 0; jb < NB; ++jb)
#pragma unroll
            for (int ib = 0; ib < NB; ++ib) {
                g[jb][ib] = fmaf(T.b[ig][ib], rv[jb], g[jb][ib]);
                g[jb][ib] = fmaf(T.dx[ig][ib], rd[jb], g[jb][ib]);
            }
    }
    e1 = a1;
    e2 = a2;
}

template <int NGP, bool FGP>
__device__ __forceinline__ void q1_layer_2d(const ElemTab& T, const float (&TU0)[NGP], const float (&TU1)[NGP], const float DX0,
                                            const float DX1, const float (&TN0)[NGP], const float (&TN1)[NGP],
                                            const float (&TF0)[NGP], const float (&TF1)[NGP], const float* fg,
                                            float (&ct0)[NGP], float (&ct1)[NGP], float& cdx0, float& cdx1, float& e1,
                                            float& e2) {
    float a1x = 0.f, a1y = 0.f, a2 = 0.f;
    float S0 = 0.f, S1 = 0.f, dyn[NGP];
#pragma unroll
    for (int i = 0; i < NGP; ++i) {
        dyn[i] = TN1[i] - TN0[i];
        S0 = fmaf(T.wx[i], TN0[i], S0);
        S1 = fmaf(T.wx[i], dyn[i], S1);
    }
    const float ddx = DX1 - DX0;
    float c1s = 0.f, css = 0.f;
#pragma unroll
    for (int jg = 0; jg < NGP; ++jg) {
        const float r = fmaf(T.b[jg][1], ddx, DX0);
        const float t = fmaf(T.b[jg][1], S1, S0) * r;
        a1x = fmaf(T.w[jg] * t, r, a1x);
        const float cx = T.w[jg] * t;
        css += cx;
        c1s = fmaf(T.b[jg][1], cx, c1s);
    }
    const float kx = T.q1c[0];
    cdx1 = kx * c1s;
    cdx0 = kx * css - cdx1;
    const float nb = -T.beta, ky = T.q1c[1];
#pragma unroll
    for (int ig = 0; ig < NGP; ++ig) {
        const float dyv = TU1[ig] - TU0[ig];
        const float t = fmaf(T.kx[1][ig], dyn[ig], T.kx[0][ig] * TN0[ig]) * dyv;
        a1y = fmaf(t, dyv, a1y);
        float cs, c1;
        if constexpr (FGP) {
            cs = 0.f; c1 = 0.f;
#pragma unroll
            for (int jg = 0; jg < NGP; ++jg) {
                const float wf = T.w2[jg][ig] * fg[jg * NGP + ig];
                cs += wf;
                c1 = fmaf(T.b[jg][1], wf, c1);
            }
        } else {
            const float dyf = TF1[ig] - TF0[ig];
            cs = fmaf(T.kx[1][ig], dyf, T.kx[0][ig] * TF0[ig]);
            c1 = fmaf(T.kx[2][ig], dyf, T.kx[1][ig] * TF0[ig]);
        }
        a2 = fmaf(cs, TU0[ig], a2);
        a2 = fmaf(c1, dyv, a2);
        ct1[ig] = fmaf(nb, c1, ky * t);
        ct0[ig] = fmaf(nb, cs, -ct1[ig]);
    }
    e1 = fmaf(T.q1c[2], a1x, T.q1c[3] * a1y);
    e2 = a2;
}

__host__ __device__ __forceinline__ void q1cf_stage(const float px0, const float px1, const float u0, const float u1, const float n0, const float n1,
                                                    float& du, float& pn) {
    du = u1 - u0;
    pn = fmaf(px1, n1, px0 * n0);
}

__host__ __device__ __forceinline__ void q1cf_elem(const float (&xm)[4], const float (&ym)[4], const float a, const float b, const float p,
                                                   const float q, const float V0, const float V1, const float S0, const float S1,
                                                   const float alpha, float& gL0, float& gL1, float& gU0, float& gU1, float& e) {
    const float X0 = fmaf(q, xm[1], p * xm[0]), X1 = fmaf(q, xm[2], p * xm[1]), X2 = fmaf(q, xm[3], p * xm[2]);
    const float ta = fmaf(b, X1, a * X0), tb = fmaf(b, X2, a * X1);
    const float Y0 = fmaf(S1, ym[1], S0 * ym[0]), Y1 = fmaf(S1, ym[2], S0 * ym[1]), Y2 = fmaf(S1, ym[3], S0 * ym[2]);
    const float t0 = fmaf(V1, Y1, V0 * Y0), t1 = fmaf(V1, Y2, V0 * Y1);
    e = fmaf(b, tb, fmaf(a, ta, e));
    e = fmaf(V1, t1, fmaf(V0, t0, e));
    gL0 = fmaf(-alpha, ta + t0, gL0);
    gL1 = fmaf(alpha, ta - t1, gL1);
    gU0 = fmaf(alpha, t0 - tb, gU0);
    gU1 = fmaf(alpha, tb + t1, gU1);
}

template <int NGP, bool FGP>
__device__ __forceinline__ void q1_layer_3d(const ElemTab& T, const float (&LU)[NGP][NGP], const float (&UU)[NGP][NGP],
                                            const float (&LX)[NGP], const float (&UX)[NGP], const float (&LY)[NGP],
                                            const float (&UY)[NGP], const float (&LN)[NGP][NGP], const float (&UN)[NGP][NGP],
                                            const float (&LF)[NGP][NGP], const float (&UF)[NGP][NGP], const float* fg,
                                            float (&cUL)[NGP][NGP], float (&cUU)[NGP][NGP], float (&cXL)[NGP], float (&cXU)[NGP],
                                            float (&cYL)[NGP], float (&cYU)[NGP], float& e1, float& e2) {
    float a1 = 0.f, a2 = 0.f;
    float A0[NGP], A1[NGP], B0[NGP], B1[NGP];
#pragma unroll
    for (int i = 0; i < NGP; ++i) A0[i] = A1[i] = B0[i] = B1[i] = 0.f;
    const float nb = -T.beta;
#pragma unroll
    for (int jg = 0; jg < NGP; ++jg) {
#pragma unroll
        for (int ig = 0; ig < NGP; ++ig) {
            const float w2 = T.w2[jg][ig];
            const float dzu = UU[jg][ig] - LU[jg][ig];
            const float uz = T.hs[2] * dzu;
            const float dzn = UN[jg][ig] - LN[jg][ig];
            const float wn0 = w2 * LN[jg][ig], wn1 = w2 * dzn;
            A0[jg] += wn0; A1[jg] += wn1; B0[ig] += wn0; B1[ig] += wn1;
            const float Qz = fmaf(T.m[1], wn1, T.m[0] * wn0);
            const float qzu = Qz * uz;
            a1 = fmaf(qzu, uz, a1);
            const float cz = T.ahs[2] * qzu;
            float cs, c1;
            if constexpr (FGP) {
                cs = 0.f; c1 = 0.f;
#pragma unroll
                for (int kg = 0; kg < NGP; ++kg) {
                    const float wf = T.w[kg] * w2 * fg[(kg * NGP + jg) * NGP + ig];
                    cs += wf;
                    c1 = fmaf(T.b[kg][1], wf, c1);
                }
            } else {
                const float dzf = UF[jg][ig] - LF[jg][ig];
                const float wf0 = w2 * LF[jg][ig], wf1 = w2 * dzf;
                cs = fmaf(T.m[1], wf1, T.m[0] * wf0);
                c1 = fmaf(T.m[2], wf1, T.m[1] * wf0);
            }
            a2 = fmaf(cs, LU[jg][ig], a2);
            a2 = fmaf(c1, dzu, a2);
            cUU[jg][ig] = fmaf(nb, c1, cz);
            cUL[jg][ig] = fmaf(nb, cs, -cUU[jg][ig]);
        }
    }
#pragma unroll
    for (int jg = 0; jg < NGP; ++jg) {
        const float dv = UX[jg] - LX[jg];
        float sx = 0.f, tx = 0.f;
#pragma unroll
        for (int kg = 0; kg < NGP; ++kg) {
            const float ux = T.hs[0] * fmaf(T.b[kg][1], dv, LX[jg]);
            const float Qx = T.w[kg] * fmaf(T.b[kg][1], A1[jg], A0[jg]);
            const float qxu = Qx * ux;
            a1 = fmaf(qxu, ux, a1);
            const float cx = T.ahs[0] * qxu;
            sx += cx;
            tx = fmaf(T.b[kg][1], cx, tx);
        }
        cXU[jg] = tx;
        cXL[jg] = sx - tx;
    }
#pragma unroll
    for (int ig = 0; ig < NGP; ++ig) {
        const float dv = UY[ig] - LY[ig];
        float sy = 0.f, ty = 0.f;
#pragma unroll
        for (int kg = 0; kg < NGP; ++kg) {
            const float uy = T.hs[1] * fmaf(T.b[kg][1], dv, LY[ig]);
            const float Qy = T.w[kg] * fmaf(T.b[kg][1], B1[ig], B0[ig]);
            const float qyu = Qy * uy;
            a1 = fmaf(qyu, uy, a1);
            const float cy = T.ahs[1] * qyu;
            sy += cy;
            ty = fmaf(T.b[kg][1], cy, ty);
        }
        cYU[ig] = ty;
        cYL[ig] = sy - ty;
    }
    e1 = a1;
    e2 = a2;
}

template <int NGP, bool FGP, bool HAS_F, bool UW, typename V = float>
__device__ __forceinline__ void q1_layer_3d_w(const ElemTab& T, const V (&LU)[NGP][NGP], const V (&UU)[NGP][NGP],
                                              const V (&LX)[NGP], const V (&UX)[NGP], const V (&LY)[NGP],
                                              const V (&UY)[NGP], const V (&LN)[NGP][NGP], const V (&UN)[NGP][NGP],
                                              const V (&LF)[NGP][NGP], const V (&UF)[NGP][NGP],
                                              const float* fg, V (&cU)[NGP][NGP], V (&cX)[NGP], V (&cY)[NGP],
                                              V (&tU)[NGP][NGP], V (&tX)[NGP], V (&tY)[NGP], V& e1, V& e2) {
    V a1z = 0.f, a1x = 0.f, a1y = 0.f, a2 = 0.f;
    const float nb = T.nbw;
    V LA[NGP], UA[NGP], LB[NGP], UB[NGP];
#pragma unroll
    for (int j = 0; j < NGP; ++j) {
        V la = 0.f, ua = 0.f, lb = 0.f, ub = 0.f;
#pragma unroll
        for (int i = 0; i < NGP; ++i) { la += LN[j][i]; ua += UN[j][i]; lb += LN[i][j]; ub += UN[i][j]; }
        LA[j] = la; UA[j] = ua; LB[j] = lb; UB[j] = ub;
    }
#pragma unroll
    for (int j = 0; j < NGP; ++j) {
#pragma unroll
        for (int i = 0; i < NGP; ++i) {
            const V dzu = UU[j][i] - LU[j][i];
            const V Qz = vfma(T.m[1], UN[j][i], T.m01 * LN[j][i]);
            const V qz = Qz * dzu;
            a1z = vfma(qz, dzu, a1z);
            V up = T.kap[2] * qz;
            V lo = cU[j][i] - up;
            if constexpr (FGP) {
                V cs = 0.f, c1 = 0.f;
#pragma unroll
                for (int k = 0; k < NGP; ++k) {
                    const float wf = T.w[k] * T.w[j] * T.w[i] * fg[(k * NGP + j) * NGP + i];
                    cs += wf;
                    c1 = vfma(T.b[k][1], wf, c1);
                }
                a2 = vfma(cs, LU[j][i], a2);
                a2 = vfma(c1, dzu, a2);
                up = vfma(nb, c1, up);
                lo = vfma(nb, cs - c1, lo);
            } else if constexpr (HAS_F) {
                const V cs = vfma(T.m[1], UF[j][i], T.m01 * LF[j][i]);
                const V c1 = vfma(T.m[2], UF[j][i], T.m12 * LF[j][i]);
                a2 = vfma(cs, LU[j][i], a2);
                a2 = vfma(c1, dzu, a2);
                up = vfma(nb, c1, up);
                lo = vfma(nb, cs - c1, lo);
            }
            tU[j][i] = lo;
            cU[j][i] = up;
        }
    }
#pragma unroll
    for (int j = 0; j < NGP; ++j) {
        const V dX = UX[j] - LX[j], dA = UA[j] - LA[j];
        V sx = 0.f, tx = 0.f;
#pragma unroll
        for (int k = 0; k < NGP; ++k) {
            const V ux = vfma(T.b[k][1], dX, LX[j]);
            const V Qx = vfma(T.b[k][1], dA, LA[j]);
            const V qx = UW ? Qx * ux : (T.w[k] * Qx) * ux;
            a1x = vfma(qx, ux, a1x);
            sx += qx;
            tx = vfma(T.b[k][1], qx, tx);
        }
        const V up = T.kap[0] * tx;
        tX[j] = vfma(T.kap[0], sx, cX[j] - up);
        cX[j] = up;
    }
#pragma unroll
    for (int i = 0; i < NGP; ++i) {
        const V dY = UY[i] - LY[i], dB = UB[i] - LB[i];
        V sy = 0.f, ty = 0.f;
#pragma unroll
        for (int k = 0; k < NGP; ++k) {
            const V uy = vfma(T.b[k][1], dY, LY[i]);
            const V Qy = vfma(T.b[k][1], dB, LB[i]);
            const V qy = UW ? Qy * uy : (T.w[k] * Qy) * uy;
            a1y = vfma(qy, uy, a1y);
            sy += qy;
            ty = vfma(T.b[k][1], qy, ty);
        }
        const V up = T.kap[1] * ty;
        tY[i] = vfma(T.kap[1], sy, cY[i] - up);
        cY[i] = up;
    }
    e1 = vfma(T.hs2[2], a1z, vfma(T.hs2[0], a1x, T.hs2[1] * a1y));
    e2 = a2;
}

}
```

### diffnet_amd/csrc/poisson_fused.hip

```cpp
#include <algorithm>
#include <cmath>
#include <cstdio>
#include <cstdlib>

#include "poisson_common.h"

namespace dn {

template <int P, int NGP, int E, bool VEC, bool FGP>
__global__ void __launch_bounds__(256) poisson2d_kernel(const PoissonParams p) {
    constexpr int NB = P + 1;
    constexpr int NW = E * P;
    const int T = blockDim.x;
    const int tid = threadIdx.x;
    const int chunk = blockIdx.x, strip = selected_strip(p, (int)blockIdx.y), b = blockIdx.z;
    const int q = chunk * (T - 1) + tid;
    const int ex0 = q * E;
    const int x0 = ex0 * P;
    const bool col_owner = !(chunk > 0 && tid == 0);
    const int64_t nps = (int64_t)p.nx * p.ny;
    const unsigned eps = (unsigned)(p.nelx * p.nely);
    const SampleBases sb = sample_bases(p, b, nps);
    const float* fgp = FGP ? p.fgp + (p.f_batched ? (int64_t)b * eps * (NGP * NGP) : 0) : nullptr;
    const int R = p.rows_per_strip;
    const int ey_own = strip * R;
    const int ey_begin = ey_own > 0 ? ey_own - 1 : 0;
    const int ey_end = min(ey_own + R, p.nely);
    const bool any_bc = sb.mask[0] != nullptr || sb.mask[1] != nullptr;

    __shared__ float xch[2][P][256];
    __shared__ double red[8];
    __shared__ int last_flag;

    float cu[NB][NW + 1], cn[NB][NW + 1], cf[NB][NW + 1];
    unsigned fixed[NB];
    float acc[NB][NW + 1];
#pragma unroll
    for (int r = 0; r < NB; ++r) {
        fixed[r] = 0u;
#pragma unroll
        for (int n = 0; n <= NW; ++n) { acc[r][n] = 0.f; cn[r][n] = 1.f; cf[r][n] = 0.f; }
    }

    auto load_row = [&](int r, int yr) {
        const unsigned rowoff = (unsigned)yr * (unsigned)p.nx;
        load_seg<NW, VEC>(sb.u, rowoff, x0, p.nx, cu[r]);
        if (sb.nu) load_seg<NW, VEC>(sb.nu, rowoff, x0, p.nx, cn[r]);
        if (sb.f) load_seg<NW, VEC>(sb.f, rowoff, x0, p.nx, cf[r]);
        fixed[r] = any_bc ? load_apply_bc<NW, VEC>(p, sb, rowoff, x0, cu[r]) : 0u;
    };

    float e1_acc = 0.f, e2_acc = 0.f, sq_acc = 0.f;
    int par = 0;

    auto emit_row = [&](int r, int yr, bool owned_row) {
        xch[par][r % P][tid] = acc[r][NW];
        asm volatile("s_waitcnt lgkmcnt(0)\n\ts_barrier" ::: "memory");
        const float left = (tid > 0) ? xch[par][r % P][tid - 1] : 0.f;
        if (owned_row && col_owner) {
            float o[NW];
#pragma unroll
            for (int n = 0; n < NW; ++n) {
                float v = acc[r][n] + (n == 0 ? left : 0.f);
                v = (fixed[r] & (1u << n)) ? 0.f : v;
                sq_acc = (x0 + n < p.nx) ? fmaf(v, v, sq_acc) : sq_acc;
                o[n] = v * p.out_scale;
            }
            if (sb.out) store_seg<NW, VEC>(sb.out, (unsigned)yr * (unsigned)p.nx, x0, p.nx, o);
        }
    };

    load_row(0, ey_begin * P);
    for (int ey = ey_begin; ey < ey_end; ++ey) {
#pragma unroll
        for (int r = 1; r <= P; ++r) load_row(r, ey * P + r);
        const bool own_layer = ey >= ey_own;
        const bool count = own_layer && col_owner;
#pragma unroll
        for (int e = 0; e < E; ++e) {
            if (ex0 + e < p.nelx) {
                float lu[NB][NB], ln[NB][NB], lf[NB][NB], g[NB][NB];
#pragma unroll
                for (int jb = 0; jb < NB; ++jb)
#pragma unroll
                    for (int ib = 0; ib < NB; ++ib) {
                        lu[jb][ib] = cu[jb][e * P + ib];
                        ln[jb][ib] = cn[jb][e * P + ib];
                        lf[jb][ib] = cf[jb][e * P + ib];
                    }
                float fg[NGP * NGP];
                if constexpr (FGP) {
                    const unsigned eo = (unsigned)ey * (unsigned)p.nelx + (unsigned)(ex0 + e);
#pragma unroll
                    for (int gi = 0; gi < NGP * NGP; ++gi) fg[gi] = fgp[eo + (unsigned)gi * eps];
                }
                float e1, e2;
                elem2d<P, NGP, FGP>(p.T, lu, ln, lf, fg, g, e1, e2);
                e1_acc += count ? e1 : 0.f;
                e2_acc += count ? e2 : 0.f;
#pragma unroll
                for (int jb = 0; jb < NB; ++jb)
#pragma unroll
                    for (int ib = 0; ib < NB; ++ib) acc[jb][e * P + ib] += g[jb][ib];
            }
        }
#pragma unroll
        for (int r = 0; r < P; ++r) emit_row(r, ey * P + r, own_layer);
        par ^= 1;
#pragma unroll
        for (int n = 0; n <= NW; ++n) {
            cu[0][n] = cu[P][n]; cn[0][n] = cn[P][n]; cf[0][n] = cf[P][n];
            acc[0][n] = acc[P][n];
#pragma unroll
            for (int r = 1; r <= P; ++r) acc[r][n] = 0.f;
        }
        fixed[0] = fixed[P];
    }
    if (ey_end == p.nely) emit_row(0, p.ny - 1, true);

    if (p.want_sums) finish_sums(p, e1_acc, e2_acc, sq_acc, tid, T, red, &last_flag);
}

}

namespace dn {


static inline int ceil_div(int a, int b) { return (a + b - 1) / b; }


static int chunks_for(int logical_threads, int T) {
    return logical_threads <= T ? 1 : ceil_div(logical_threads - 1, T - 1);
}

static Geom2D plan2d(const dn_mesh* m, int P, bool allow_e4 = true, bool chain_ok = false, bool allow_ua = false) {
    Geom2D g;
    const int nx = m->nx, nely = (m->ny - 1) / P;
    const bool ua = allow_ua && P == 1 && (nx & 3) == 1 && nx >= 321;
    const int maxE = (P == 1) ? 4 : (P == 2 ? 2 : 1);
    const int minE = (P == 1) ? 2 : 1;
    double best = -1.0;
    g.T = 64; g.E = minE; g.chunks = 1;
    for (int E = minE; E <= maxE; E *= 2) {
        const int NW = E * P;
        if (ua && E != 4) continue;
        if (P == 1 && E == 4 && !ua && (nx % 4 != 0 || !allow_e4)) continue;
        const int Q = ua ? (nx - 1) / NW : (nx - 1) / NW + 1;
        for (int T = 64; T <= 256; T += 64) {
            const int chunks = chunks_for(Q, T);
            const double util = (double)Q / ((double)chunks * T);
            const double score = util + 0.02 * NW + 0.0003 * T;
            if (score > best) { best = score; g.T = T; g.E = E; g.chunks = chunks; }
        }
    }
    const long long waves_per_strip = (long long)g.chunks * m->batch * (g.T / 64);
    int R = 32;
    while (R > 4 && waves_per_strip * ceil_div(nely, R) < 4096) R /= 2;
    if (R > nely) R = nely;
    g.R = R < 1 ? 1 : R;
    g.strips = ceil_div(nely, g.R);
    g.W = 1;
    g.ua = ua;
    const int cw = poisson2d_q1_cf_chain();
    if (chain_ok && !ua && P == 1 && cw > 1 && g.E == 4 && g.T == 128 && g.R < 16) {
        int Rc = 2;
        while (Rc < 16 && waves_per_strip * ceil_div(nely, Rc) > 6144) Rc *= 2;
        if (Rc < 16 && ceil_div(nely, Rc) >= cw) { g.R = Rc; g.strips = ceil_div(nely, Rc); g.W = cw; }
    }
    return g;
}

static Geom3D plan3d(const dn_mesh* m, bool allow_e2 = false) {
    Geom3D g;
    const int nx = m->nx, ny = m->ny, nelz = m->nz - 1;
    if (m->ngp == 2 && allow_e2) {
        g.TX = 16; g.TY = 16; g.E = 2;
        g.chunks = chunks_for(nx / 2, 16);
        g.tiles = chunks_for(ny, 16);
        const double cap = 256.0 * 3.0;
        const long long wg_per_strip = (long long)g.chunks * g.tiles * m->batch;
        double bestc = 1e300;
        g.R = nelz < 1 ? 1 : nelz;
        for (int R = 4; R <= 64 && R <= (nelz < 4 ? 4 : nelz); ++R) {
            const int strips = ceil_div(nelz, R);
            const double rounds = std::max(1.0, std::ceil(2.0 * (double)(wg_per_strip * strips) / cap) / 2.0);
            const double layers = (strips == 1 ? nelz : R + 1) + 1.5;
            const double cost = rounds * layers * (1.0 + 0.002 * R);
            if (cost < bestc) { bestc = cost; g.R = R; }
        }
        if (g.R > nelz) g.R = nelz < 1 ? 1 : nelz;
        g.strips = ceil_div(nelz, g.R);
        return g;
    }
    if (m->ngp == 2) {
        g.TX = 16; g.E = 1;
        g.chunks = chunks_for(nx, 16);
        double best = -1.0;
        g.TY = 16;
        for (int TY = 4; TY <= 16; TY += 4) {
            const int tiles = chunks_for(ny, TY);
            const double util = (double)ny / ((double)tiles * TY) + 0.002 * TY;
            if (util > best) { best = util; g.TY = TY; g.tiles = tiles; }
        }
        const double cap = 256.0 * 5.0 * (256.0 / (16.0 * g.TY)) ;
        const long long wg_per_strip = (long long)g.chunks * g.tiles * m->batch;
        double bestc = 1e300;
        g.R = nelz < 1 ? 1 : nelz;
        for (int R = 4; R <= 64 && R <= (nelz < 4 ? 4 : nelz); ++R) {
            const int strips = ceil_div(nelz, R);
            const double rounds = std::max(1.0, std::ceil(2.0 * (double)(wg_per_strip * strips) / cap) / 2.0);
            const double layers = (strips == 1 ? nelz : R + 1) + 1.5;
            const double cost = rounds * layers * (1.0 + 0.002 * R);
            if (cost < bestc) { bestc = cost; g.R = R; }
        }
        if (g.R > nelz) g.R = nelz < 1 ? 1 : nelz;
        g.strips = ceil_div(nelz, g.R);
        return g;
    }
    const int maxE = 1;
    double best = -1.0;
    g.TX = 16; g.TY = 16; g.E = 1; g.chunks = 1; g.tiles = 1;
    for (int E = 1; E <= maxE; E *= 2) {
        const int Q = (nx - 1) / E + 1;
        for (int TX = 8; TX <= 128; ++TX) {
            const int TY = 256 / TX;
            if (TX * TY < 192 || TY < 2) continue;
            const int chunks = chunks_for(Q, TX);
            const int tiles = chunks_for(ny, TY);
            const double util = ((double)Q / ((double)chunks * TX)) * ((double)ny / ((double)tiles * TY));
            const bool pow2 = (TX & (TX - 1)) == 0;
            const double score = util + 0.05 * E + (pow2 ? 0.04 + 0.0005 * TX : 0.0);
            if (score > best) { best = score; g.TX = TX; g.TY = TY; g.E = E; g.chunks = chunks; g.tiles = tiles; }
        }
    }
    const long long wg_per_strip = (long long)g.chunks * g.tiles * m->batch;
    int R = 32;
    while (R > 8 && wg_per_strip * ceil_div(nelz, R) < 2048) R /= 2;
    if (R > nelz) R = nelz;
    g.R = R < 1 ? 1 : R;
    g.strips = ceil_div(nelz, g.R);
    return g;
}

static Geom2D plan2d_env(const dn_mesh* m, int P, bool allow_e4 = true, bool chain_ok = false, bool allow_ua = false) {
    Geom2D g = plan2d(m, P, allow_e4, chain_ok, allow_ua);
    const char* e = config(CFG_PLAN2D);
    int T, E, R, W = 0;
    if (e && sscanf(e, "%d,%d,%d,%d", &T, &E, &R, &W) >= 3 && T >= 64 && T <= 256 && (E == 1 || E == 2 || E == 4) && R >= 1 &&
        !(P == 1 && (E == 1 || (E == 4 && !g.ua && (m->nx % 4 != 0 || !allow_e4)) || (g.ua && E != 4))) && !(P > 1 && E * P > 4)) {
        const int nely = (m->ny - 1) / P;
        g.T = T; g.E = E; g.R = R > nely ? nely : R;
        g.chunks = chunks_for(g.ua ? (m->nx - 1) / 4 : (m->nx - 1) / (E * P) + 1, T);
        g.strips = ceil_div(nely, g.R);
        const int cw = poisson2d_q1_cf_chain();
        g.W = (W >= 2 && !g.ua && cw > 1 && P == 1 && E == 4 && T == 128 && g.R + 3 <= 64 && g.R >= 2) ? cw : 1;
    }
    return g;
}

static Geom3D plan3d_env(const dn_mesh* m, bool allow_e2 = false, bool need_e2 = false) {
    Geom3D g = plan3d(m, allow_e2);
    const char* e = config(CFG_PLAN3D);
    int TX, TY, E, R;
    if (e && sscanf(e, "%d,%d,%d,%d", &TX, &TY, &E, &R) == 4 && TX * TY >= 64 && (E == 1 || (E == 2 && allow_e2 && TX == 16 && TY == 16)) && R >= 1 &&
        TX * TY <= 256 && !(need_e2 && allow_e2 && E == 1)) {
        const int nelz = m->nz - 1;
        g.TX = TX; g.TY = TY; g.E = E; g.R = R > nelz ? nelz : R;
        g.chunks = chunks_for((m->nx - 1) / E + 1, TX);
        g.tiles = chunks_for(m->ny, TY);
        g.strips = ceil_div(nelz, g.R);
    }
    return g;
}

static long long num_workgroups(const dn_mesh* m, bool allow_e4 = true) {
    if (m->nsd == 2) {
        const Geom2D g = plan2d_env(m, m->degree, allow_e4);
        const Geom2D gu = plan2d_env(m, m->degree, allow_e4, false, true);
        return std::max((long long)g.chunks * g.strips, (long long)gu.chunks * gu.strips) * m->batch;
    }
    const Geom3D g = plan3d_env(m, false);
    long long n = (long long)g.chunks * g.tiles * g.strips * m->batch;
    if (m->ngp == 2) {
        const Geom3D g2 = plan3d_env(m, true), g2n = plan3d_env(m, true, true);
        n = std::max(n, (long long)g2.chunks * g2.tiles * g2.strips * m->batch);
        n = std::max(n, (long long)g2n.chunks * g2n.tiles * g2n.strips * m->batch);
    }
    return n;
}

static int validate_mesh(const dn_mesh* m) {
    if (!m) return DN_E_BADARG;
    if (m->nsd != 2 && m->nsd != 3) return DN_E_BADARG;
    if (m->degree < 1 || m->degree > 3 || m->ngp < 1 || m->ngp > 4) return DN_E_BADARG;
    if (m->batch < 1 || m->nx < 2 || m->ny < 2 || (m->nsd == 3 && m->nz < 2)) return DN_E_BADARG;
    if ((m->nx - 1) % m->degree || (m->ny - 1) % m->degree || (m->nsd == 3 && (m->nz - 1) % m->degree)) return DN_E_BADARG;
    if (m->batch > 65535) return DN_E_BADARG;
    return 0;
}

template <int P, int NGP, int E>
static void launch2d_vec(const PoissonParams& pp, const Geom2D& g, int batch, bool vec, hipStream_t s) {
    dim3 grid(g.chunks, g.strips, batch), block(g.T);
    const bool fgp = pp.fgp != nullptr;
    constexpr bool CANVEC = (E * P == 2 || E * P == 4);
    const bool v = vec && CANVEC;
    if constexpr (P == 1) {
        (void)v;
    } else {
        if (v) {
            if (fgp) hipLaunchKernelGGL((poisson2d_kernel<P, NGP, E, CANVEC, true>), grid, block, 0, s, pp);
            else hipLaunchKernelGGL((poisson2d_kernel<P, NGP, E, CANVEC, false>), grid, block, 0, s, pp);
        } else {
            if (fgp) hipLaunchKernelGGL((poisson2d_kernel<P, NGP, E, false, true>), grid, block, 0, s, pp);
            else hipLaunchKernelGGL((poisson2d_kernel<P, NGP, E, false, false>), grid, block, 0, s, pp);
        }
    }
}

template <int P, int NGP>
static int launch2d_e(const PoissonParams& pp, const Geom2D& g, int batch, bool vec, hipStream_t s) {
    if constexpr (P == 1) {
        if (g.E == 4) { launch2d_vec<P, NGP, 4>(pp, g, batch, vec, s); return 0; }
    }
    if constexpr (P <= 2) {
        if (g.E == 2) { launch2d_vec<P, NGP, 2>(pp, g, batch, vec, s); return 0; }
    }
    if (g.E == 1) { launch2d_vec<P, NGP, 1>(pp, g, batch, vec, s); return 0; }
    return DN_E_UNSUPPORTED;
}

static int launch2d(const PoissonParams& pp, const Geom2D& g, int P, int ngp, int batch, bool vec, hipStream_t s) {
    const bool force_rule = config(CFG_Q1_RULE_KERNEL) != nullptr;
    if (P == 1 && pp.fgp == nullptr && !force_rule) return launch_poisson2d_q1_cf(pp, g, batch, vec, s);
    switch (P * 10 + ngp) {
        case 12: return launch_poisson2d_q1_g2(pp, g, batch, vec, s);
        case 13: return launch_poisson2d_q1_g3(pp, g, batch, vec, s);
        case 14: return launch_poisson2d_q1_g4(pp, g, batch, vec, s);
        case 23: return launch2d_e<2, 3>(pp, g, batch, vec, s);
        case 24: return launch2d_e<2, 4>(pp, g, batch, vec, s);
        case 33: return launch2d_e<3, 3>(pp, g, batch, vec, s);
        case 34: return launch2d_e<3, 4>(pp, g, batch, vec, s);
        default: return DN_E_UNSUPPORTED;
    }
}

}

static bool q1n2_ok(const dn_mesh* m, const dn_poisson_args* a) {
    if (m->nsd != 3 || m->degree != 1 || m->ngp != 2 || (m->nx & 1) || a->f_gp) return false;
    if (m->gpw[0] != 1.0f || m->gpw[1] != 1.0f) return false;
    if (dn::config(dn::CFG_Q1_3D_T16) != nullptr || dn::config(dn::CFG_Q1_3D_E1) != nullptr) return false;
    auto al = [](const void* p, uintptr_t bytes) { return p == nullptr || (reinterpret_cast<uintptr_t>(p) % bytes) == 0; };
    if (!al(a->u, 8) || !al(a->nu, 8) || !al(a->f, 8) || !al(a->out, 8)) return false;
    int kinds = 0;
    for (int k = 0; k < 2; ++k) {
        const dn_dirichlet& d = a->bc[k];
        if (!d.mask) continue;
        if (d.field) return false;
        if (d.mask_kind == DN_MASK_U8) { if (!al(d.mask, 2)) return false; kinds |= 1; }
        else if (d.mask_kind == DN_MASK_F32) { if (!al(d.mask, 8)) return false; kinds |= 2; }
        else return false;
    }
    return kinds != 3;
}

static bool q1n2_needed(const dn_poisson_args* a) {
    for (int k = 0; k < 2; ++k)
        if (a->bc[k].mask_kind == DN_MASK_BOX && a->bc[k].box_faces != 0) return true;
    return a->fold_prev != nullptr || (a->f_is_load && a->f);
}

namespace dn {
__global__ void __launch_bounds__(256) poisson_finish_sums_kernel(const double* __restrict__ part_energy, const double* __restrict__ part_sumsq, int n,
                                                                  double* energy, double* sumsq, float* energy_f32, double energy_scale, int acc) {
    __shared__ double red[2 * 4];
    const double* const part[2] = {part_energy, part_sumsq};
    double tot[2];
    sum_partials<2, 16, false, false>(part, n, (int)threadIdx.x, 256, tot);
    block_sum2(tot[0], tot[1], red, (int)threadIdx.x, 256);
    if (threadIdx.x == 0) write_sums(tot[0], tot[1], acc, energy, sumsq, energy_f32, energy_scale);
}
}

using namespace dn;

extern "C" int64_t dn_poisson_workspace_bytes(const dn_mesh* mesh) {
    if (validate_mesh(mesh) != 0) return DN_E_BADARG;
    if (mesh->nsd == 3 && mesh->degree > 1) {
        long long n1, n2, ef;
        gen3d_layout(mesh, n1, n2, ef);
        return DN_WS_HEADER + (int64_t)sizeof(double) * (n1 + n2) + (int64_t)sizeof(float) * ef;
    }
    const long long n = std::max(num_workgroups(mesh, true), num_workgroups(mesh, false));
    return DN_WS_HEADER + (int64_t)(2 * sizeof(double)) * n;
}

static long long launched_workgroups(const dn_mesh* m, const dn_poisson_args* a);

static bool poisson_vec_ok(const dn_mesh* m, const dn_poisson_args* a, int NW) {
    auto aligned = [](const void* p, int bytes) { return p == nullptr || (reinterpret_cast<uintptr_t>(p) % bytes) == 0; };
    bool ok = (NW == 2 || NW == 4) && (m->nx % NW == 0) && aligned(a->u, 4 * NW) && aligned(a->nu, 4 * NW) && aligned(a->f, 4 * NW) &&
              aligned(a->out, 4 * NW);
    for (int k = 0; k < 2; ++k)
        if (a->bc[k].mask_kind == DN_MASK_F32 || a->bc[k].mask_kind == DN_MASK_U8)
            ok = ok && aligned(a->bc[k].mask, a->bc[k].mask_kind == DN_MASK_U8 ? NW : 4 * NW) && aligned(a->bc[k].field, 4 * NW);
    return ok;
}

extern "C" int dn_poisson_apply(const dn_mesh* m, const dn_poisson_args* a, void* stream) {
    int rc = validate_mesh(m);
    if (rc) return rc;
    if (!a || !a->u) return DN_E_BADARG;
    if (a->f && a->f_gp) return DN_E_BADARG;
    if (!a->out && !a->energy && !a->sumsq && !a->energy_f32) return DN_E_BADARG;
    const int P = m->degree;
    const bool gen3d = m->nsd == 3 && P != 1;
    if (m->ngp < (P == 1 ? 2 : 3)) return DN_E_UNSUPPORTED;
    bool packed_bc = false;
    for (int k = 0; k < 2; ++k) {
        const dn_dirichlet& d = a->bc[k];
        if (d.mask_kind < DN_MASK_F32 || d.mask_kind > DN_MASK_BOX) return DN_E_BADARG;
        const bool present = d.mask_kind == DN_MASK_BOX ? d.box_faces != 0 : d.mask != nullptr;
        if (present && (d.mask_kind == DN_MASK_BITS || d.mask_kind == DN_MASK_BOX)) {
            packed_bc = true;
            if (d.field) return DN_E_BADARG;
            if (d.mask_kind == DN_MASK_BITS && d.row_words < (m->nx + 31) / 32) return DN_E_BADARG;
        }
    }
    if (packed_bc && m->nsd == 3) {
        for (int k = 0; k < 2; ++k)
            if (a->bc[k].mask_kind == DN_MASK_BITS) return DN_E_UNSUPPORTED;
        if (gen3d || !q1n2_ok(m, a)) return DN_E_UNSUPPORTED;
    } else if (packed_bc) {
        if (m->nsd != 2 || P != 1 || a->f_gp || config(CFG_Q1_RULE_KERNEL) != nullptr) return DN_E_UNSUPPORTED;
        for (int k = 0; k < 2; ++k) {
            const dn_dirichlet& d = a->bc[k];
            if (d.mask && (d.mask_kind == DN_MASK_F32 || d.mask_kind == DN_MASK_U8)) return DN_E_UNSUPPORTED;
        }
    }
    const bool want_red = a->energy || a->sumsq || a->energy_f32;
    auto vec_ok = [&](int NW) { return poisson_vec_ok(m, a, NW); };
    const bool allow_e4 = vec_ok(4);
    const long long nwg = gen3d ? 1 : num_workgroups(m, allow_e4);
    if (nwg >= (1ll << 31)) return DN_E_UNSUPPORTED;
    if (!gen3d && want_red && (!a->workspace || a->workspace_bytes < DN_WS_HEADER + (int64_t)(2 * sizeof(double)) * nwg)) return DN_E_WORKSPACE;
    if ((int64_t)m->nx * m->ny * (m->nsd == 3 ? m->nz : 1) >= (1ll << 30)) return DN_E_UNSUPPORTED;

    PoissonParams pp;
    for (int i = 0; i < 4; ++i) {
        for (int j = 0; j < 4; ++j) {
            pp.T.b[i][j] = m->basis[i][j];
            pp.T.dx[i][j] = m->dbasis[i][j] * m->scale[0];
            pp.T.dy[i][j] = m->dbasis[i][j] * m->scale[1];
            pp.T.dz[i][j] = m->dbasis[i][j] * m->scale[2];
        }
        pp.T.w[i] = m->gpw[i];
        pp.T.wx[i] = m->gpw[i] * a->wscale;
    }
    for (int i = 0; i < 4; ++i)
        for (int j = 0; j < 4; ++j) pp.T.w2[i][j] = pp.T.w[i] * pp.T.wx[j];
    for (int d = 0; d < 3; ++d) {
        pp.T.hs[d] = 0.5f * m->scale[d];
        pp.T.ahs[d] = a->alpha * pp.T.hs[d];
    }
    pp.T.q1c[0] = a->alpha * pp.T.hs[0] * pp.T.hs[0]; pp.T.q1c[1] = a->alpha * pp.T.hs[1] * pp.T.hs[1];
    pp.T.q1c[2] = pp.T.hs[0] * pp.T.hs[0];            pp.T.q1c[3] = pp.T.hs[1] * pp.T.hs[1];
    {
        double mm[4] = {0.0, 0.0, 0.0, 0.0};
        for (int g = 0; g < m->ngp; ++g) {
            const double bb = m->basis[g][1];
            mm[0] += m->gpw[g]; mm[1] += m->gpw[g] * bb; mm[2] += m->gpw[g] * bb * bb; mm[3] += m->gpw[g] * bb * bb * bb;
        }
        pp.T.q1my[0] = (float)(mm[0] - 2.0 * mm[1] + mm[2]); pp.T.q1my[1] = (float)(mm[1] - mm[2]); pp.T.q1my[2] = (float)mm[2];
        for (int r = 0; r < 3; ++r) pp.T.q1mx[r] = (float)((double)(r == 0 ? mm[0] - 2.0 * mm[1] + mm[2] : (r == 1 ? mm[1] - mm[2] : mm[2])) * (double)a->wscale);
        {
            const double rr[4] = {mm[0] - 3.0 * mm[1] + 3.0 * mm[2] - mm[3], mm[1] - 2.0 * mm[2] + mm[3], mm[2] - mm[3], mm[3]};
            const double hx = 0.5 * (double)m->scale[0], hy = 0.5 * (double)m->scale[1], ws = a->wscale;
            for (int r = 0; r < 4; ++r) {
                pp.T.q1xm[r] = (float)(hx * hx * rr[r]);
                pp.T.q1ym[r] = (float)(hy * hy * ws * rr[r]);
            }
            pp.T.q1px[0] = (float)((mm[0] - mm[1]) * ws); pp.T.q1px[1] = (float)(mm[1] * ws);
            pp.T.q1sy[0] = (float)(mm[0] - mm[1]);        pp.T.q1sy[1] = (float)mm[1];
        }
        for (int r = 0; r < 4; ++r) {
            pp.T.m[r] = (float)mm[r];
            pp.T.mxs[r] = (float)(mm[r] * (double)a->wscale);
            if (r < 3)
                for (int g = 0; g < 4; ++g) pp.T.kx[r][g] = (float)(mm[r] * (double)m->gpw[g] * (double)a->wscale);
        }
    }
    for (int g = 0; g < 4; ++g) pp.T.wb[g] = m->gpw[g] * m->basis[g][1];
    for (int d = 0; d < 3; ++d) {
        pp.T.hs2[d] = pp.T.hs[d] * pp.T.hs[d];
        pp.T.kap[d] = a->alpha * a->wscale * pp.T.hs2[d];
    }
    pp.T.m01 = pp.T.m[0] - pp.T.m[1]; pp.T.m12 = pp.T.m[1] - pp.T.m[2];
    pp.T.esc = a->wscale; pp.T.nbw = -a->beta * a->wscale;
    pp.T.alpha = a->alpha; pp.T.beta = a->beta; pp.T.c = a->c;
    pp.u = a->u; pp.nu = a->nu; pp.f = a->f; pp.fgp = a->f_gp;
    pp.nu_batched = a->nu_batched; pp.f_batched = a->f_batched;
    pp.f_is_load = (a->f_is_load && a->f) ? 1 : 0;
    if (pp.f_is_load && !(m->nsd == 3 && !gen3d && q1n2_ok(m, a))) return DN_E_UNSUPPORTED;
    for (int k = 0; k < 2; ++k) {
        const dn_dirichlet& d = a->bc[k];
        const bool present = d.mask_kind == DN_MASK_BOX ? d.box_faces != 0 : d.mask != nullptr;
        pp.bc[k].mask = d.mask_kind == DN_MASK_BOX ? nullptr : d.mask; pp.bc[k].field = d.field; pp.bc[k].value = d.value;
        pp.bc[k].mask_is_u8 = d.mask_kind == DN_MASK_U8; pp.bc[k].mask_batched = d.mask_batched;
        pp.bc[k].field_batched = d.field_batched;
        pp.bc[k].kind = present ? d.mask_kind : -1;
        pp.bc[k].box_faces = d.box_faces; pp.bc[k].row_bytes = 4 * d.row_words;
    }
    pp.out_scale = a->out_scale; pp.out = a->out;
    pp.counter = reinterpret_cast<unsigned*>(a->workspace);
    pp.part_energy = a->workspace ? reinterpret_cast<double*>(reinterpret_cast<char*>(a->workspace) + DN_WS_HEADER) : nullptr;
    pp.part_sumsq = pp.part_energy ? pp.part_energy + nwg : nullptr;
    pp.energy = a->energy; pp.sumsq = a->sumsq;
    pp.energy_f32 = a->energy_f32; pp.energy_scale = a->energy_scale;
    pp.nx = m->nx; pp.ny = m->ny; pp.nz = m->nsd == 3 ? m->nz : 1;
    pp.nelx = (m->nx - 1) / P; pp.nely = (m->ny - 1) / P; pp.nelz = m->nsd == 3 ? (m->nz - 1) / P : 1;
    pp.want_sums = want_red ? 1 : 0;
    pp.spin_limit = config(CFG_HANDOVER_SPIN_LIMIT) ? std::atoi(config(CFG_HANDOVER_SPIN_LIMIT)) : 0;
    hipStream_t s = reinterpret_cast<hipStream_t>(stream);
    pp.fold_n = 0;
    if (a->fold_prev) {
        const dn_poisson_args* q = a->fold_prev;
        if (gen3d || !q->defer_sums || !q->workspace || !(q->energy || q->sumsq || q->energy_f32)) return DN_E_BADARG;
        if (q->accumulate_sums && !(q->energy && q->sumsq)) return DN_E_BADARG;
        if (q->workspace == a->workspace && want_red) return DN_E_BADARG;
        const long long qn = launched_workgroups(m, q), qstride = num_workgroups(m, poisson_vec_ok(m, q, 4));
        if (q->workspace_bytes < DN_WS_HEADER + (int64_t)(2 * sizeof(double)) * qstride || qn > qstride) return DN_E_WORKSPACE;
        const bool cf2d = m->nsd == 2 && P == 1 && a->f_gp == nullptr && config(CFG_Q1_RULE_KERNEL) == nullptr;
        if (!cf2d && !(m->nsd == 3 && q1n2_ok(m, a))) return DN_E_UNSUPPORTED;
        pp.fold_pe = reinterpret_cast<const double*>(reinterpret_cast<const char*>(q->workspace) + DN_WS_HEADER);
        pp.fold_ps = pp.fold_pe + qstride;
        pp.fold_n = (int)qn;
        pp.fold_energy = q->energy; pp.fold_sumsq = q->sumsq; pp.fold_energy_f32 = q->energy_f32;
        pp.fold_scale = q->energy_scale;
        pp.fold_acc = q->accumulate_sums ? 1 : 0;
    }

    if (a->strip_select < 0 || a->strip_select > 2) return DN_E_BADARG;
    if (a->accumulate_sums && want_red && !(a->energy && a->sumsq)) return DN_E_BADARG;
    pp.strip_sel = a->strip_select;
    pp.acc_sums = (a->accumulate_sums && want_red && !a->defer_sums) ? 1 : 0;
    pp.defer_sums = (a->defer_sums && want_red) ? 1 : 0;
    auto launched = [&](int total) { return a->strip_select == 1 ? std::min(total, 2) : (a->strip_select == 2 ? std::max(total - 2, 0) : total); };
    auto no_strips = [&]() {
        if (pp.fold_n > 0) {
            hipLaunchKernelGGL(poisson_finish_sums_kernel, dim3(1), dim3(256), 0, s, pp.fold_pe, pp.fold_ps, pp.fold_n, pp.fold_energy, pp.fold_sumsq,
                               pp.fold_energy_f32, pp.fold_scale, pp.fold_acc);
            DN_LAUNCH_CHECK();
        }
        return 0;
    };
    if (gen3d) {
        if (a->strip_select != 0 || a->accumulate_sums || a->defer_sums) return DN_E_UNSUPPORTED;
        rc = launch_poisson3d_gen(pp, m, a->workspace, a->workspace_bytes, s);
        if (rc) return rc;
        DN_LAUNCH_CHECK();
        return 0;
    }
    if (m->nsd == 2) {
        const bool chain_ok = P == 1 && a->f_gp == nullptr && config(CFG_Q1_RULE_KERNEL) == nullptr && a->strip_select == 0;
        const bool cf_kernel = P == 1 && a->f_gp == nullptr && config(CFG_Q1_RULE_KERNEL) == nullptr;
        Geom2D g = plan2d_env(m, P, allow_e4, chain_ok, cf_kernel);
        if (!chain_ok) g.W = 1;
        pp.rows_per_strip = g.R;
        pp.nstrips = g.strips;
        g.strips = launched(g.strips);
        if (g.strips == 0) return no_strips();
        if (want_red && (long long)g.chunks * ((g.strips + g.W - 1) / g.W) * m->batch > nwg) return DN_E_WORKSPACE;
        const int NW = g.E * P;
        const bool vec = vec_ok(NW);
        rc = launch2d(pp, g, P, m->ngp, m->batch, vec, s);
    } else {
        Geom3D g = plan3d_env(m, q1n2_ok(m, a), q1n2_needed(a));
        pp.rows_per_strip = g.R;
        pp.nstrips = g.strips;
        g.strips = launched(g.strips);
        if (g.strips == 0) return no_strips();
        if (want_red && (long long)g.chunks * g.tiles * g.strips * m->batch > nwg) return DN_E_WORKSPACE;
        const int NW = g.E;
        const bool vec = vec_ok(NW);
        switch (m->ngp) {
            case 2: rc = launch_poisson3d_q1_g2(pp, g, m->batch, vec, s); break;
            case 3: rc = launch_poisson3d_q1_g3(pp, g, m->batch, vec, s); break;
            case 4: rc = launch_poisson3d_q1_g4(pp, g, m->batch, vec, s); break;
            default: rc = DN_E_UNSUPPORTED;
        }
    }
    if (rc) return rc;
    DN_LAUNCH_CHECK();
    return 0;
}

static long long launched_workgroups(const dn_mesh* m, const dn_poisson_args* a) {
    const bool e4 = poisson_vec_ok(m, a, 4);
    auto sel = [&](int total) { return a->strip_select == 1 ? std::min(total, 2) : (a->strip_select == 2 ? std::max(total - 2, 0) : total); };
    if (m->nsd == 2) {
        const bool chain_ok = m->degree == 1 && a->f_gp == nullptr && config(CFG_Q1_RULE_KERNEL) == nullptr && a->strip_select == 0;
        const bool cf_kernel = m->degree == 1 && a->f_gp == nullptr && config(CFG_Q1_RULE_KERNEL) == nullptr;
        Geom2D g = plan2d_env(m, m->degree, e4, chain_ok, cf_kernel);
        if (!chain_ok) g.W = 1;
        return (long long)g.chunks * ((sel(g.strips) + g.W - 1) / g.W) * m->batch;
    }
    Geom3D g = plan3d_env(m, q1n2_ok(m, a), q1n2_needed(a));
    return (long long)g.chunks * g.tiles * sel(g.strips) * m->batch;
}

extern "C" int dn_poisson_finish_sums(const dn_mesh* m, const dn_poisson_args* a, void* stream) {
    int rc = validate_mesh(m);
    if (rc) return rc;
    if (!a || !a->workspace || !(a->energy || a->sumsq || a->energy_f32)) return DN_E_BADARG;
    if (!a->defer_sums) return DN_E_BADARG;
    if (m->nsd == 3 && m->degree > 1) return DN_E_UNSUPPORTED;
    if (a->accumulate_sums && !(a->energy && a->sumsq)) return DN_E_BADARG;
    const long long n = launched_workgroups(m, a);
    if (n <= 0) return 0;
    const long long nall = num_workgroups(m, true) > num_workgroups(m, false) ? num_workgroups(m, true) : num_workgroups(m, false);
    if (a->workspace_bytes < DN_WS_HEADER + (int64_t)(2 * sizeof(double)) * nall) return DN_E_WORKSPACE;
    const double* pe = reinterpret_cast<const double*>(reinterpret_cast<const char*>(a->workspace) + DN_WS_HEADER);
    const long long stride = num_workgroups(m, poisson_vec_ok(m, a, 4));
    hipLaunchKernelGGL(poisson_finish_sums_kernel, dim3(1), dim3(256), 0, reinterpret_cast<hipStream_t>(stream), pe, pe + stride, (int)n, a->energy,
                       a->sumsq, a->energy_f32, a->energy_scale, (int)(a->accumulate_sums != 0));
    DN_LAUNCH_CHECK();
    return 0;
}
```

### diffnet_amd/ops.py

```python
import ctypes as C
import math

import torch
from torch.autograd.function import once_differentiable

from . import _lib
from ._lib import DnCoefGradArgs, DnDirichlet, DnEikonalArgs, DnFoslsArgs, DnFsdtArgs, DnHelmholtzArgs, DnMesh, DnNsArgs, DnPoissonArgs, DnStokesArgs, DnStrongformArgs, DnTransportArgs, I32x3, DiffNetHipError


def _require(t, name, ndim=None, strict=False):
    if not isinstance(t, torch.Tensor):
        raise TypeError(f"{name} must be a torch.Tensor")
    if not t.is_cuda:
        raise DiffNetHipError(f"{name} is on {t.device}: the FEM ops run on the GPU only (no CPU fallback); move it with .cuda()")
    if t.dtype != torch.float32:
        raise TypeError(f"{name} must be float32, got {t.dtype}")
    if ndim is not None and t.dim() != ndim:
        raise ValueError(f"{name} must have {ndim} dims, got shape {tuple(t.shape)}")
    if strict and not t.is_contiguous():
        raise DiffNetHipError(f"{name} is not contiguous: a prepared launch (PoissonPlan) keeps the pointers it was given; pass a contiguous tensor")
    return t.contiguous()


def _raw_stream(device):
# ... 291 lines not shown
        return m._version
    except RuntimeError:
        return None


def _packed_on_first_use(m):
    ver = _version_of(m)
    if ver is None:
        return None
    key = (m.untyped_storage().data_ptr(), m.storage_offset(), tuple(m.shape), tuple(m.stride()), m.dtype, _raw_stream(m.device))
    with _WS_LOCK:
        ent = _PACK_CACHE.get(key)
        if ent is not None and ent[1] == ver:
            _PACK_CACHE.move_to_end(key)
            _PACK_STATS["hit"] += 1
            return ent[2]
    pm = PackedMask.pack(m)
    _PACK_STATS["pack"] += 1
    with _WS_LOCK:
        _PACK_CACHE[key] = (m, ver, pm)
        _PACK_CACHE.move_to_end(key)
        while len(_PACK_CACHE) > _PACK_CACHE_MAX:
            _PACK_CACHE.popitem(last=False)
    return pm


def _auto_pack(geom, u, f_gp, dl):
    if not (AUTO_PACK_MASKS and geom.nsd == 2 and geom.deg == 1 and f_gp is None and len(dl) > 0 and isinstance(u, torch.Tensor) and u.is_cuda):
        return dl
    if _lib.CONFIG_MIRROR.get("Q1_RULE_KERNEL"):
        return dl
    want = (1, *geom.node_shape)
    for d in dl:
        m = d.mask
        if isinstance(d.value, torch.Tensor):
            return dl
        if isinstance(m, (PackedMask, BoxFaces)):
            continue
        if not (isinstance(m, torch.Tensor) and m.is_cuda and m.device == u.device and m.is_contiguous() and not m.requires_grad and
                m.dtype in (torch.float32, torch.uint8, torch.bool) and m.dim() == u.dim() and tuple(m.shape[1:]) == want and
                m.shape[0] in (1, u.shape[0])):
            return dl
    if any(isinstance(d.mask, torch.Tensor) and _version_of(d.mask) is None for d in dl):
        return dl
    return [d if isinstance(d.mask, (PackedMask, BoxFaces)) else Dirichlet(_packed_on_first_use(d.mask), d.value) for d in dl]


def _norm_dirichlet(dirichlet):
    out = []
    for d in dirichlet or ():
        if isinstance(d, Dirichlet):
            out.append(d)
        else:
            m, v = d
            out.append(Dirichlet(m, v))
    if len(out) > 2:
        raise ValueError("at most two Dirichlet conditions per call are supported; merge masks beforehand")
    return out


_threading = __import__("threading")
_WS = {}
_WS_LOCK = _threading.Lock()
_FSDT_LAUNCH_LOCK = _threading.Lock()
_POISSON_WS_BYTES = {}


_SIDE_STREAMS = {}


def _side_stream(dev):
    s = _SIDE_STREAMS.get(dev.index)
    if s is None:
        s = _SIDE_STREAMS[dev.index] = torch.cuda.Stream(dev)
    return s


def _workspace(dev, nbytes):
    key = (dev.index, _raw_stream(dev))
    with _WS_LOCK:
        ws = _WS.get(key)
        if ws is None or ws.numel() < nbytes:
            ws = torch.zeros(max(nbytes, 1 << 16), dtype=torch.uint8, device=dev)
            _WS[key] = ws
    return ws


def workspace_status(device=None):
    dev = torch.device("cuda", torch.cuda.current_device()) if device is None else torch.device(device)
    with _WS_LOCK:
        items = [(k, w) for d in (_WS, _FSDT_WS) for k, w in d.items() if k[0] == dev.index]
    for (_, stream), ws in items:
        _lib.check(_lib.lib().dn_workspace_status(C.c_void_p(ws.data_ptr()), C.c_void_p(stream)), "dn_workspace_status")


_CALL_CACHE = __import__("collections").OrderedDict()
_CALL_CACHE_MAX = 16
_CALL_STATS = {"hit": 0, "miss": 0, "uncached": 0}


def _tkey(t):
    if t is None:
        return 0
    if not (isinstance(t, torch.Tensor) and t.is_cuda and t.is_contiguous()):
        return None
    return (t.data_ptr(), t.dtype, tuple(t.shape))


def _call_key(geom, u, nu, f, f_gp, dl, scal, want_out, want_sums, out):
    parts = [geom.key, u.device.index, _raw_stream(u.device), scal, want_out, want_sums, isinstance(f, LoadVector)]
    if isinstance(f, LoadVector):
        f = f.tensor
    for t in (u, nu, f, f_gp, out):
        k = _tkey(t)
        if k is None or (k != 0 and k[1] != torch.float32):
            return None
        parts.append(k)
    for d in dl:
        m, v = d.mask, d.value
        if isinstance(m, PackedMask):
            mk = ("bits", m.bits.data_ptr(), m.shape)
        elif isinstance(m, BoxFaces):
            mk = ("box", m.bits)
        else:
            mk = _tkey(m)
            if mk is None or mk == 0 or mk[1] not in (torch.float32, torch.uint8):
                return None
        if isinstance(v, torch.Tensor):
            vk = _tkey(v)
            if vk is None or vk[1] != torch.float32 or len(vk[2]) != u.dim():
                return None
        else:
            vk = float(v)
        parts.append((mk, vk))
    return tuple(parts)


def poisson_apply(geom, u, nu=None, f=None, f_gp=None, dirichlet=(), alpha=1.0, beta=1.0, c=1.0, wscale=1.0,
                  out_scale=1.0, want_out=True, want_sums=True, loss_scale=None, out=None):
    dl = _auto_pack(geom, u, f_gp, _norm_dirichlet(dirichlet))
    key = None
    if isinstance(u, torch.Tensor) and u.is_cuda:
        key = _call_key(geom, u, nu, f, f_gp, dl, (float(alpha), float(beta), float(c), float(wscale), float(out_scale),
                                                   None if loss_scale is None else float(loss_scale)), want_out, want_sums, out)
    if key is None:
        _CALL_STATS["uncached"] += 1
        return PoissonPlan(geom, u, nu, f, f_gp, dl, alpha, beta, c, wscale, out_scale, want_out, want_sums, loss_scale, out, strict=False).launch()
    with _WS_LOCK:
        ent = _CALL_CACHE.get(key)
        if ent is not None:
            _CALL_CACHE.move_to_end(key)
    if ent is None:
        _CALL_STATS["miss"] += 1
        plan = PoissonPlan(geom, u, nu, f, f_gp, dl, alpha, beta, c, wscale, out_scale, want_out, want_sums, loss_scale, out, strict=True)
        res = plan.launch()
        with _WS_LOCK:
            live_ws = list(_WS.values())
        plan.keep = [t for t in plan.keep if any(t is w for w in live_ws)] + [d.mask for d in dl if not isinstance(d.mask, torch.Tensor)]
        plan.result = None
        plan.fresh = (want_out and out is None, want_sums, loss_scale is not None)
        with _WS_LOCK:
            _CALL_CACHE[key] = plan
            while len(_CALL_CACHE) > _CALL_CACHE_MAX:
                _CALL_CACHE.popitem(last=False)
        return res
    _CALL_STATS["hit"] += 1
    a = ent.args
    new_out, has_sums, has_loss = ent.fresh
    o = out
    sums = loss32 = None
    if new_out:
        o = torch.empty_like(u)
    if has_sums:
        sums = torch.empty(2, dtype=torch.float64, device=u.device)
    if has_loss:
        loss32 = torch.empty((), dtype=torch.float32, device=u.device)
    with ent.lock:
        if new_out:
            a.out = o.data_ptr()
        if has_sums:
            a.energy = sums.data_ptr()
            a.sumsq = a.energy + 8
        if has_loss:
            a.energy_f32 = loss32.data_ptr()
        rc = ent._fn(ent._mesh_ref, ent._args_ref, C.c_void_p(key[2]))
    if rc:
        _lib.check(rc, "dn_poisson_apply")
    return (o, sums, loss32) if has_loss else (o, sums)


def call_cache_clear():
    with _WS_LOCK:
        _CALL_CACHE.clear()
        _FSDT_CACHE.clear()
        _STOKES.cache.clear()
        _NS.cache.clear()
        _TRANSPORT.cache.clear()
        _STRONGFORM.cache.clear()
        _FOSLS.cache.clear()
        _HELMHOLTZ.cache.clear()
        _EIKONAL.cache.clear()
        _EIKONAL3D.cache.clear()
        _PACK_CACHE.clear()
    _POISSON_WS_BYTES.clear()
    _FSDT_WS_BYTES.clear()
    _STOKES.ws_bytes.clear()
    _NS.ws_bytes.clear()
    _TRANSPORT.ws_bytes.clear()
    _STRONGFORM.ws_bytes.clear()
    _FOSLS.ws_bytes.clear()
    _HELMHOLTZ.ws_bytes.clear()
    _EIKONAL.ws_bytes.clear()
    _EIKONAL3D.ws_bytes.clear()


class PoissonPlan:

    def __init__(self, geom, u, nu=None, f=None, f_gp=None, dirichlet=(), alpha=1.0, beta=1.0, c=1.0, wscale=1.0,
                 out_scale=1.0, want_out=True, want_sums=True, loss_scale=None, out=None, strict=True, strip_select=0, continues=None,
                 async_sums=False, loss_out=None, pipelined_sums=False):
        if continues is not None:
            out = continues.result[0]
        self.mesh, self.args, self.keep, self.result = _prepare_poisson(geom, u, nu, f, f_gp, dirichlet, alpha, beta, c, wscale, out_scale,
                                                                        want_out, want_sums, loss_scale, out, strict=strict,
                                                                        reuse=None if continues is None else continues.result)
        if loss_out is not None:
            if loss_scale is None or continues is not None:
                raise ValueError("loss_out needs loss_scale and is not for the second launch of a split evaluation")
            if not (isinstance(loss_out, torch.Tensor) and loss_out.is_cuda and loss_out.dtype == torch.float32 and loss_out.numel() == 1
                    and loss_out.device == u.device):
                raise DiffNetHipError("loss_out must be a one-element float32 tensor on the device of u")
            self.args.energy_f32 = loss_out.data_ptr()
            self.keep.append(loss_out)
            self.result = (self.result[0], self.result[1], loss_out)
        self.args.strip_select = int(strip_select)
        self.args.accumulate_sums = int(continues is not None)
        self.async_sums = bool(async_sums) and self.args.workspace is not None and self.args.workspace != 0
        self.pipelined_sums = bool(pipelined_sums) and not self.async_sums and self.args.workspace is not None and self.args.workspace != 0
        self._folds = None
        if self.pipelined_sums:
            self.args.defer_sums = 1
            ws = torch.zeros(int(self.args.workspace_bytes), dtype=torch.uint8, device=u.device)
            self.keep.append(ws)
            self.args.workspace = ws.data_ptr()
        if self.async_sums:
            self.args.defer_sums = 1
            ws = torch.zeros(int(self.args.workspace_bytes), dtype=torch.uint8, device=u.device)
            self.keep.append(ws)
            self._own_ws = ws
            self.args.workspace = ws.data_ptr()
            self.sums_stream = _side_stream(u.device)
            self._side = self.sums_stream.cuda_stream
            self._ev_main, self._ev_done = _lib.new_event(), _lib.new_event()
            self._hip = _lib.hip_runtime()
            self._finish = _lib.lib().dn_poisson_finish_sums
            self._launched = False
        self.device = u.device
        self.stream = _raw_stream(u.device)
        self._fn = _lib.lib().dn_poisson_apply
        self._mesh_ref, self._args_ref = C.byref(self.mesh), C.byref(self.args)
        self.lock = _threading.Lock()
        if self.async_sums:
            for t in [self._own_ws] + [r for r in self.result[1:] if isinstance(r, torch.Tensor)]:
                t.record_stream(self.sums_stream)

    def __del__(self):
        if getattr(self, "async_sums", False):
            try:
                hip = self._hip
                if getattr(self, "_launched", False):
                    hip.hipEventSynchronize(self._ev_done)
                hip.hipEventDestroy(self._ev_main)
                hip.hipEventDestroy(self._ev_done)
            except Exception:
                pass

    def check(self):
        if self.args.workspace:
            _lib.check(_lib.lib().dn_workspace_status(C.c_void_p(self.args.workspace), C.c_void_p(_raw_stream(self.device))), "dn_workspace_status")

    def launch(self):
        cur = _raw_stream(self.device)
        if self.args.workspace and cur != self.stream:
            raise DiffNetHipError("PoissonPlan.launch: prepared on another stream (its reduction workspace is per stream); prepare one plan per stream")
        if self.async_sums:
            hip, side = self._hip, C.c_void_p(self._side)
            if self._launched:
                hip.hipStreamWaitEvent(C.c_void_p(cur), self._ev_done, 0)
            rc = self._fn(self._mesh_ref, self._args_ref, C.c_void_p(cur))
            if rc:
                _lib.check(rc, "dn_poisson_apply")
            hip.hipEventRecord(self._ev_main, C.c_void_p(cur))
            hip.hipStreamWaitEvent(side, self._ev_main, 0)
            rc = self._finish(self._mesh_ref, self._args_ref, side)
            if rc:
                _lib.check(rc, "dn_poisson_finish_sums")
            hip.hipEventRecord(self._ev_done, side)
            self._launched = True
            return self.result
        rc = self._fn(self._mesh_ref, self._args_ref, C.c_void_p(cur))
        if rc:
            _lib.check(rc, "dn_poisson_apply")
        return self.result

    def fold(self, prev):
        if prev is None:
            self.args.fold_prev = None
            self._folds = None
            return self
        if not getattr(prev, "pipelined_sums", False):
            raise DiffNetHipError("PoissonPlan.fold: the other plan must be prepared with pipelined_sums=True")
        if C.string_at(C.addressof(prev.mesh), C.sizeof(prev.mesh)) != C.string_at(C.addressof(self.mesh), C.sizeof(self.mesh)):
            raise DiffNetHipError("PoissonPlan.fold: the other plan was prepared for another mesh or batch size; only a plan on the same mesh "
                                  "and batch can be folded")
        if prev.device != self.device or prev.stream != self.stream:
            raise DiffNetHipError("PoissonPlan.fold: the other plan was prepared on another device or stream; its launch must precede this one "
                                  "on the same stream")
        self._folds = prev
        self.args.fold_prev = C.addressof(prev.args)
        return self

    def finish_sums(self):
        if not self.pipelined_sums:
            return self.result
        rc = _lib.lib().dn_poisson_finish_sums(self._mesh_ref, self._args_ref, C.c_void_p(_raw_stream(self.device)))
        if rc:
            _lib.check(rc, "dn_poisson_finish_sums")
        return self.result

    def wait_sums(self):
        if self.async_sums and self._launched:
            self._hip.hipStreamWaitEvent(C.c_void_p(_raw_stream(self.device)), self._ev_done, 0)


def _prepare_poisson(geom, u, nu, f, f_gp, dirichlet, alpha, beta, c, wscale, out_scale, want_out, want_sums, loss_scale, out, strict=False, reuse=None):
    nsd = geom.nsd
    u = _require(u, "u", nsd + 2, strict)
    B = u.shape[0]
    node_shape = tuple(geom.node_shape)
    if tuple(u.shape[1:]) != (1, *node_shape):
        raise ValueError(f"u has shape {tuple(u.shape)}, expected (B,1,{','.join(map(str, node_shape))})")
    keep = [u]
    args = DnPoissonArgs()
    args.u = u.data_ptr()

    def field(t, name, allow_gp=False):
        t = _require(t, name, nsd + 2, strict)
        if t.shape[0] not in (1, B):
            raise ValueError(f"{name} batch {t.shape[0]} does not broadcast to {B}")
        keep.append(t)
        return t, int(t.shape[0] == B)

    if nu is not None:
        nu, nb_ = field(nu, "nu")
        if tuple(nu.shape[1:]) != (1, *node_shape):
            raise ValueError("nu must be a nodal field")
        args.nu, args.nu_batched = nu.data_ptr(), nb_
    if f is not None and f_gp is not None:
        raise ValueError("give either nodal f or f_gp, not both")
    if isinstance(f, LoadVector):
        args.f_is_load = 1
        f = f.tensor
    if f is not None:
        f, fb = field(f, "f")
        if tuple(f.shape[1:]) != (1, *node_shape):
            raise ValueError("f must be a nodal field")
        args.f, args.f_batched = f.data_ptr(), fb
    if f_gp is not None:
        f_gp, fb = field(f_gp, "f_gp")
        if tuple(f_gp.shape[1:]) != (geom.ngp_total, *geom.elem_shape):
            raise ValueError(f"f_gp must have shape (B|1,{geom.ngp_total},{geom.elem_shape})")
        args.f_gp, args.f_batched = f_gp.data_ptr(), fb
    dl = _norm_dirichlet(dirichlet)
    compact = (nsd == 2 and geom.deg == 1 and f_gp is None and len(dl) > 0 and _lib.lib().dn_config_get(b"Q1_RULE_KERNEL") in (None, b"") and
               all(isinstance(d.mask, (PackedMask, BoxFaces)) and not isinstance(d.value, torch.Tensor) for d in dl))
    box3d = False
    if nsd == 3 and geom.deg == 1 and f_gp is None and any(isinstance(d.mask, BoxFaces) for d in dl):
        mesh0 = geom.mesh_struct(B)
        imgs = [d.mask for d in dl if not isinstance(d.mask, BoxFaces)]
        cfg = _lib.lib().dn_config_get
        box3d = (mesh0.ngp == 2 and mesh0.nx % 2 == 0 and len(imgs) <= 1 and cfg(b"Q1_3D_T16") in (None, b"") and cfg(b"Q1_3D_E1") in (None, b"") and
                 all(not isinstance(d.value, torch.Tensor) for d in dl) and
                 all(isinstance(t, torch.Tensor) and t.is_cuda and t.is_contiguous() and t.dtype in (torch.uint8, torch.float32) and
                     t.data_ptr() % 8 == 0 for t in imgs) and
                 all(t is None or t.data_ptr() % 8 == 0 for t in (u, nu, f, out)))
    for k, d in enumerate(dl):
        m = d.mask
        if box3d and isinstance(m, BoxFaces):
            bc = args.bc[k]
            bc.value = float(d.value)
            bc.mask_kind, bc.box_faces = _lib.MASK_BOX, m.bits
            continue
        if compact:
            bc = args.bc[k]
            bc.value = float(d.value)
            if isinstance(m, BoxFaces):
                bc.mask_kind, bc.box_faces = _lib.MASK_BOX, m.bits
            else:
                if tuple(m.shape[1:]) != (1, *node_shape) or m.shape[0] not in (1, B) or m.bits.device != u.device:
                    raise ValueError(f"packed Dirichlet mask of shape {m.shape} does not match u")
                keep.append(m.bits)
                bc.mask, bc.mask_kind, bc.row_words = m.bits.data_ptr(), _lib.MASK_BITS, m.row_words
                bc.mask_batched = int(m.shape[0] == B)
            continue
        m = _mask_image(m, u)
        if not isinstance(m, torch.Tensor) or not m.is_cuda:
            raise DiffNetHipError("Dirichlet mask must be a CUDA tensor")
        if strict and (m.dtype == torch.bool or not m.is_contiguous()):
            raise DiffNetHipError("PoissonPlan: a bool or non-contiguous Dirichlet mask would be converted into a one-time copy; pass a "
                                  "contiguous float32 / uint8 image (or a PackedMask / BoxFaces)")
        if m.dtype == torch.bool:
            m = m.to(torch.uint8)
        if m.dtype not in (torch.float32, torch.uint8):
            raise TypeError("Dirichlet mask must be float32, uint8 or bool")
        m = m.contiguous()
        if m.dim() != nsd + 2 or tuple(m.shape[1:]) != (1, *node_shape) or m.shape[0] not in (1, B):
            raise ValueError(f"Dirichlet mask shape {tuple(m.shape)} does not match u")
        keep.append(m)
        bc = args.bc[k]
        bc.mask = m.data_ptr()
        bc.mask_kind = _lib.MASK_U8 if m.dtype == torch.uint8 else _lib.MASK_F32
        bc.mask_batched = int(m.shape[0] == B)
        if isinstance(d.value, torch.Tensor):
            v = d.value
            if v.dim() == nsd:
                v = v[(None,) * 2]
            if strict and not v.is_cuda:
                raise DiffNetHipError("PoissonPlan: the Dirichlet value field must live on the GPU (a prepared launch would keep a one-time copy)")
            v = _require(v.to(u.device) if not v.is_cuda else v, "Dirichlet value", nsd + 2, strict)
            if tuple(v.shape[1:]) != (1, *node_shape) or v.shape[0] not in (1, B):
                raise ValueError("Dirichlet value field shape does not match u")
            keep.append(v)
            bc.field = v.data_ptr()
            bc.field_batched = int(v.shape[0] == B)
        else:
            bc.value = float(d.value)
    args.alpha, args.beta, args.c, args.wscale, args.out_scale = alpha, beta, c, wscale, out_scale
    mesh = geom.mesh_struct(B)
    if out is not None:
        if not want_out or out.shape != u.shape or out.dtype != torch.float32 or out.device != u.device or not out.is_contiguous():
            raise ValueError("out= must be a contiguous float32 tensor of u's shape on u's device")
    elif want_out:
        out = torch.empty_like(u)
    sums = None
    if out is not None:
        args.out = out.data_ptr()
    if want_sums or (mesh.nsd == 3 and mesh.degree > 1):
        key = (mesh.nsd, mesh.degree, mesh.ngp, mesh.nx, mesh.ny, mesh.nz, B)
        nbytes = _POISSON_WS_BYTES.get(key)
        if nbytes is None:
            nbytes = _lib.lib().dn_poisson_workspace_bytes(C.byref(mesh))
            if nbytes < 0:
                _lib.check(int(nbytes), "dn_poisson_workspace_bytes")
            _POISSON_WS_BYTES[key] = nbytes
        ws = _workspace(u.device, nbytes)
        keep.append(ws)
        args.workspace, args.workspace_bytes = ws.data_ptr(), ws.numel()
    if want_sums:
        sums = reuse[1] if reuse is not None else torch.empty(2, dtype=torch.float64, device=u.device)
        args.energy = sums.data_ptr()
        args.sumsq = sums.data_ptr() + 8
    loss32 = None
    if loss_scale is not None:
        if not want_sums:
            raise ValueError("loss_scale needs want_sums=True")
        loss32 = reuse[2] if reuse is not None else torch.empty((), dtype=torch.float32, device=u.device)
        args.energy_f32, args.energy_scale = loss32.data_ptr(), float(loss_scale)
    keep += [t for t in (out, sums, loss32) if t is not None]
    return mesh, args, keep, ((out, sums, loss32) if loss_scale is not None else (out, sums))


def _wants_grad(*ts):
    return torch.is_grad_enabled() and any(isinstance(t, torch.Tensor) and t.requires_grad for t in ts)


def _extra_grad_inputs(nu, f, f_gp, dirichlet):
    return _wants_grad(nu, f, f_gp, *[d.value for d in dirichlet])


def _dirichlet_cond(m):
    return (m > 0.5) if m.is_floating_point() else (m != 0)


def _apply_dirichlet(u, dirichlet):
    for d in dirichlet:
        v = d.value
        if isinstance(v, torch.Tensor):
            v = v[(None,) * (u.dim() - v.dim())] if v.dim() < u.dim() else v
            v = v.to(u.device).expand_as(u)
        else:
            v = torch.full_like(u, float(v))
        u = torch.where(_dirichlet_cond(_mask_image(d.mask, u)), v, u)
    return u


def _geom_tables(geom, device):
    cache = geom.__dict__.setdefault("_dev_tables", {})
    hit = cache.get(str(device))
    if hit is None:
        from .tables import nd_tables
        K, _, w = nd_tables(geom.nsd, geom.deg, geom.gpx_1d, geom.gpw_1d, geom.hs)
        names = ["N_gp"] + ["dN_%s_gp" % a for a in "xyz"[:geom.nsd]]
        hit = ({n: torch.from_numpy(K[n].reshape(K[n].shape[0], -1).copy()).to(device) for n in names}, torch.from_numpy(w).to(device))
        cache[str(device)] = hit
    return hit


def composed_energy(geom, u, nu=None, f=None, f_gp=None, dirichlet=(), c=1.0, jac=1.0):
    T, w = _geom_tables(geom, u.device)
    nsd, nbf = geom.nsd, geom.deg + 1
    ev = lambda t, name: _GaussPtEval.apply(t, T[name], nsd, nbf, nbf - 1)
    ub = _apply_dirichlet(u, _norm_dirichlet(dirichlet))
    g2 = sum(ev(ub, "dN_%s_gp" % a) ** 2 for a in "xyz"[:nsd])
    wg = (w * jac).reshape((1, -1) + (1,) * nsd)
    dens = c * g2 if nu is None else c * ev(nu, "N_gp") * g2
    if f is not None or f_gp is not None:
        dens = dens - ev(ub, "N_gp") * (f_gp if f_gp is not None else ev(f, "N_gp"))
    return torch.sum(wg * dens) / (u.shape[0] * geom.nelem_total)


def composed_residual(geom, u, nu=None, f=None, f_gp=None, dirichlet=(), jac=1.0):
    T, w = _geom_tables(geom, u.device)
    nsd, nbf = geom.nsd, geom.deg + 1
    dirichlet = _norm_dirichlet(dirichlet)
    ev = lambda t, name: _GaussPtEval.apply(t, T[name], nsd, nbf, nbf - 1)
    evT = lambda t, name: _GaussPtEvalT.apply(t.contiguous(), T[name], tuple(u.shape), nsd, nbf, nbf - 1)
    ub = _apply_dirichlet(u, dirichlet)
    wg = (w * jac).reshape((1, -1) + (1,) * nsd)
    nug = None if nu is None else ev(nu, "N_gp")
    R = None
    for a in "xyz"[:nsd]:
        q = wg * ev(ub, "dN_%s_gp" % a)
        q = q if nug is None else q * nug
        t = evT(q.expand(u.shape[0], *q.shape[1:]), "dN_%s_gp" % a)
        R = t if R is None else R + t
    if f is not None or f_gp is not None:
        fg = f_gp if f_gp is not None else ev(f, "N_gp")
        R = R - evT((wg * fg).expand(u.shape[0], -1, *fg.shape[2:]), "N_gp")
    for d in dirichlet:
        R = torch.where(_dirichlet_cond(_mask_image(d.mask, R)), torch.zeros_like(R), R)
    return R


class _PoissonFn(torch.autograd.Function):

    @staticmethod
    def forward(ctx, u, nu, f, f_gp, geom, dl, alpha, beta, c, wscale, out_scale, loss_scale):
        out, sums, loss = poisson_apply(geom, u, nu, f, f_gp, dl, alpha=alpha, beta=beta, c=c, wscale=wscale, out_scale=out_scale,
                                        want_out=True, want_sums=True, loss_scale=loss_scale)
        ctx.set_materialize_grads(False)
        ctx.save_for_backward(out, nu, u)
        ctx.meta = (geom, dl, alpha, beta, c, wscale, out_scale, loss_scale)
        ctx.f_shape = tuple(f.shape) if isinstance(f, torch.Tensor) else None
        return out, sums, loss

    @staticmethod
    def backward(ctx, g_out, g_sums, g_loss):
        out, nu, u = ctx.saved_tensors
        geom, dl, alpha, beta, c, wscale, out_scale, loss_scale = ctx.meta
        need_u, need_nu, need_f = ctx.needs_input_grad[:3]
        gnu = gf = None

        def coef_add(v, a_nu, a_f, in_scale=None):
            nonlocal gnu, gf
            tn, tf = _coef(geom, u, v, dl, a_nu, a_f, wscale, need_nu, need_f, in_scale)
            if tn is not None:
                gnu = tn if gnu is None else gnu + tn
            if tf is not None:
                gf = tf if gf is None else gf + tf

        if need_nu or need_f:
            if g_out is not None:
                coef_add(g_out.contiguous(), out_scale * alpha, -out_scale * beta)
            if g_sums is not None:
                coef_add(out * (2.0 / out_scale), alpha, -beta, g_sums[1:2].to(torch.float32))
        hom = tuple(Dirichlet(d.mask, 0.0) for d in dl)

        def K(v, scale):
            return _fused(geom, v, nu, None, None, hom, alpha, 0.0, 0.0, wscale, scale, 0.0)[0]

        gu = None
        if g_out is not None and need_u:
            gu = K(g_out.contiguous(), out_scale)
        coef = None
        if g_loss is not None:
            coef = g_loss * loss_scale
        if g_sums is not None:
            coef = g_sums[0].to(torch.float32) if coef is None else coef + g_sums[0].to(torch.float32)
            if need_u:
                t = K(out * (2.0 / out_scale), 1.0) * g_sums[1].to(torch.float32)
                gu = t if gu is None else gu + t
        if coef is not None:
            if alpha != 2.0 * c or beta != 1.0:
                if g_loss is not None or c != 0.0:
                    raise RuntimeError("poisson_apply: the energy output is differentiable only in the energy-loss form (alpha = 2c, beta = 1)")
            else:
                t = out * (coef / out_scale)
                gu = t if gu is None else gu + t
                if need_nu or need_f:
                    coef_add(None, c, -1.0, coef.reshape(1))
        if gnu is not None and nu.shape[0] != gnu.shape[0]:
            gnu = gnu.sum(0, keepdim=True)
        if gf is not None and ctx.f_shape[0] != gf.shape[0]:
            gf = gf.sum(0, keepdim=True)
        return (gu if need_u else None, gnu, gf) + (None,) * 9

# ... 1438 lines not shown
```

### include/diffnet_hip.h

```cpp
#ifndef DIFFNET_HIP_H
#define DIFFNET_HIP_H

#include <stdint.h>

#ifdef __cplusplus
extern "C" {
#endif

#define DN_ABI_VERSION 10

#define DN_E_BADARG (-1)
#define DN_E_UNSUPPORTED (-2)
#define DN_E_WORKSPACE (-3)
#define DN_E_HANDOVER (-4)

int dn_config_set(const char *key, const char *value);
const char *dn_config_get(const char *key);

typedef struct dn_mesh {
    int32_t nsd;
    int32_t degree;
    int32_t ngp;
    int32_t batch;
    int32_t nx, ny, nz;
    float scale[3];
    float gpw[4];
    float basis[4][4];
    float dbasis[4][4];
} dn_mesh;

enum { DN_MASK_F32 = 0, DN_MASK_U8 = 1, DN_MASK_BITS = 2, DN_MASK_BOX = 3 };
enum { DN_FACE_XLO = 1, DN_FACE_XHI = 2, DN_FACE_YLO = 4, DN_FACE_YHI = 8, DN_FACE_ZLO = 16, DN_FACE_ZHI = 32 };
typedef struct dn_dirichlet {
    const void *mask;
    const float *field;
    float value;
    int32_t mask_kind;
    int32_t mask_batched;
    int32_t field_batched;
    int32_t box_faces;
    int32_t row_words;
} dn_dirichlet;

int dn_pack_mask_bits(const void *mask, int32_t mask_kind, int64_t rows, int32_t nx, int32_t row_words, uint32_t *bits, void *stream);
int dn_unpack_mask_bits(const uint32_t *bits, int64_t rows, int32_t nx, int32_t row_words, uint8_t *mask_u8, void *stream);

typedef struct dn_poisson_args {
    const float *u;
    const float *nu;
    const float *f;
    const float *f_gp;
    int32_t nu_batched;
    int32_t f_batched;
    dn_dirichlet bc[2];
    float alpha, beta, c, wscale;
    float out_scale;
    float *out;
    double *energy;
    double *sumsq;
    void *workspace;
    int64_t workspace_bytes;
    float *energy_f32;
    double energy_scale;
    int32_t strip_select, accumulate_sums;
    int32_t defer_sums;
    const struct dn_poisson_args *fold_prev;
    int32_t f_is_load;
} dn_poisson_args;

int dn_abi_version(void);
const char *dn_build_info(void);

int dn_probe_stream(const float *a, const float *b, const float *c, float *out, int64_t n, int32_t mode, void *stream);
int dn_probe_march(const float *a, const float *b, const float *c, float *out, int32_t B, int32_t ny, int32_t R, int32_t rows_ahead,
                   int32_t flags, void *stream);
int dn_probe_tile(const float *a, const float *b, const float *c, float *out, int32_t B, int32_t ny, int32_t rows_per_tile, int32_t threads,
                  int32_t flags, void *stream);

int64_t dn_poisson_workspace_bytes(const dn_mesh *mesh);
int dn_poisson_apply(const dn_mesh *mesh, const dn_poisson_args *args, void *stream);
int dn_poisson_finish_sums(const dn_mesh *mesh, const dn_poisson_args *args, void *stream);

int dn_workspace_status(void *workspace, void *stream);

int dn_gauss_pt_eval_fwd(const float *in, const float *tables, float *out, int32_t batch, int32_t nsd,
                         const int32_t n[3], int32_t nbf, int32_t stride, int32_t G, void *stream);
int dn_gauss_pt_eval_bwd(const float *grad_out, const float *tables, float *grad_in, int32_t batch, int32_t nsd,
                         const int32_t n[3], int32_t nbf, int32_t stride, int32_t G, void *stream);

int dn_assemble(const float *r_split, float *out, int32_t batch, int32_t nsd, const int32_t n[3], int32_t nbf,
                int32_t stride, int32_t accumulate, void *stream);
int dn_assemble_bwd(const float *grad_out, float *grad_split, int32_t batch, int32_t nsd, const int32_t n[3],
                    int32_t nbf, int32_t stride, void *stream);

int dn_winding_nodes(const float *points, const float *normals, const float *nodes, float *out, int32_t batch,
                     int32_t npts, int32_t ny, int32_t nx, void *stream);

int dn_fdm_stencil_fwd(const float *g_padded, float *out, int32_t batch, int32_t ny, int32_t nx, const float *kernel9,
                       int32_t axis, float a, float b, void *stream);
int dn_fdm_stencil_bwd(const float *grad_out, float *grad_g_padded, int32_t batch, int32_t ny, int32_t nx,
                       const float *kernel9, int32_t axis, float a, float b, void *stream);

typedef struct dn_fsdt_args {
    const float *w, *phi_x, *phi_y;
    const void *bc_mask;
    int32_t mask_is_u8, mask_batched;
    const float *bc_field[3];
    int32_t bc_field_batched[3];
    float bc_value[3];
    float D11, D12, D22, D66, A44, A55, q;
    float wscale;
    float *out[3];
    double *sumsq;
    void *workspace;
    int64_t workspace_bytes;
    const float *in_scale;
    float *norms;
    const float *in_num;
    const float *in_den;
    int32_t defer_sums;
    int32_t den_ticket;
    const void *den_workspace;
} dn_fsdt_args;
int64_t dn_fsdt_workspace_bytes(const dn_mesh *mesh);
int dn_fsdt_apply(const dn_mesh *mesh, const dn_fsdt_args *args, void *stream);

typedef struct dn_stokes_args {
    const float *u, *v, *p;
    const void *bc_mask[3];
    int32_t mask_is_u8[3];
    int32_t mask_batched[3];
    const float *bc_field[3];
    int32_t bc_field_batched[3];
    float bc_value[3];
    const float *f_gp[2];
    int32_t f_batched[2];
    float f_value[2];
    float visco, pspg, wscale;
    int32_t transpose;
    float *out[3];
    double *sumsq;
    float *norms;
    const float *in_num, *in_den;
    void *workspace;
    int64_t workspace_bytes;
} dn_stokes_args;
int64_t dn_stokes_workspace_bytes(const dn_mesh *mesh);
int dn_stokes_apply(const dn_mesh *mesh, const dn_stokes_args *args, void *stream);

typedef struct dn_ns_args {
    const float *u, *v, *p;
    const void *bc_mask[3];
    int32_t mask_is_u8[3];
    int32_t mask_batched[3];
    const float *bc_field[3];
    int32_t bc_field_batched[3];
    float bc_value[3];
    const float *f_gp[2];
    int32_t f_batched[2];
    float f_value[2];
    float visco, wscale;
    float tau_h[2];
    float cinv;
    int32_t vjp;
    const float *cot[3];
    float *out[3];
    double *sumsq;
    float *norms;
    const float *in_num, *in_den;
    void *workspace;
    int64_t workspace_bytes;
} dn_ns_args;
int64_t dn_ns_workspace_bytes(const dn_mesh *mesh);
int dn_ns_apply(const dn_mesh *mesh, const dn_ns_args *args, void *stream);

typedef struct dn_transport_args {
    const float *u;
    const float *nu;
    int32_t nu_batched;
    int32_t r_first_wins;
    const void *bc_mask[2];
    int32_t mask_is_u8[2];
    int32_t mask_batched[2];
    const float *bc_field[2];
    int32_t bc_field_batched[2];
    float bc_value[2];
    const float *f_gp;
    int32_t f_batched;
    float f_value;
    float adv[2];
    float kappa[2];
    float tau;
    float react[4];
    float wscale;
    int32_t vjp;
    const float *cot;
    float *out;
    double *sumsq;
    float *norm;
    const float *in_num, *in_den;
    void *workspace;
    int64_t workspace_bytes;
} dn_transport_args;
int64_t dn_transport_workspace_bytes(const dn_mesh *mesh);
int dn_transport_apply(const dn_mesh *mesh, const dn_transport_args *args, void *stream);

typedef struct dn_strongform_args {
    const float *u;
    const float *f;
    const float *f_gp;
    int32_t f_batched;
    float f_value;
    dn_dirichlet bc[2];
    float ax, ay, b, dxx, dyy, fs;
    float wscale, out_scale;
    float d2basis[4][4];
    const float *in_scale;
    float *grad;
    double *sum;
    void *workspace;
    int64_t workspace_bytes;
} dn_strongform_args;
int64_t dn_strongform_workspace_bytes(const dn_mesh *mesh);
int dn_strongform_apply(const dn_mesh *mesh, const dn_strongform_args *args, void *stream);

typedef struct dn_fosls_args {
    const float *u;
    const float *mx;
    const float *my;
    int64_t field_stride;
    const float *nu;
    int32_t nu_batched;
    float nu_value;
    const float *f;
    const float *f_gp;
    int32_t f_batched;
    float f_value;
    dn_dirichlet bc[2];
    float wq, wd, fs;
    float wscale, out_scale;
    const float *in_scale;
    float *grad_u;
    float *grad_mx;
    float *grad_my;
    int64_t grad_stride;
    double *sum;
    void *workspace;
    int64_t workspace_bytes;
} dn_fosls_args;
int64_t dn_fosls_workspace_bytes(const dn_mesh *mesh);
int dn_fosls_apply(const dn_mesh *mesh, const dn_fosls_args *args, void *stream);

typedef struct dn_helmholtz_args {
    const float *u;
    const float *nu;
    const float *sigma;
    const float *f;
    const float *f_gp;
    int32_t nu_batched;
    int32_t sigma_batched;
    int32_t f_batched;
    float sigma_value;
    float f_value;
    dn_dirichlet bc[2];
    float c, cr, fs;
    float alpha, gamma, beta;
    float wscale, out_scale;
    float *out;
    double *energy;
    double *sumsq;
    void *workspace;
    int64_t workspace_bytes;
} dn_helmholtz_args;
int64_t dn_helmholtz_workspace_bytes(const dn_mesh *mesh);
int dn_helmholtz_apply(const dn_mesh *mesh, const dn_helmholtz_args *args, void *stream);

typedef struct dn_eikonal_args {
    const float *u;
    dn_dirichlet bc[2];
    const float *f;
    const float *f_gp;
    int32_t f_batched;
    float f_value;
    float tau;
    float sq;
    float wscale;
    int32_t vjp;
    const float *cot;
    const float *in_num;
    const float *in_den;
    float *out;
    double *sumsq;
    float *norm;
    void *workspace;
    int64_t workspace_bytes;
} dn_eikonal_args;
int64_t dn_eikonal_workspace_bytes(const dn_mesh *mesh);
int dn_eikonal_apply(const dn_mesh *mesh, const dn_eikonal_args *args, void *stream);

int64_t dn_eikonal3d_workspace_bytes(const dn_mesh *mesh);
int dn_eikonal3d_apply(const dn_mesh *mesh, const dn_eikonal_args *args, void *stream);

typedef struct dn_coef_grad_args {
    const float *u;
    const float *v;
    dn_dirichlet bc[2];
    float a_nu, a_f, wscale;
    const float *in_scale;
    float *g_nu;
    float *g_f;
} dn_coef_grad_args;
int dn_poisson_coef_grad(const dn_mesh *mesh, const dn_coef_grad_args *args, void *stream);

int64_t dn_upconv_out_workspace_bytes(int64_t B, int64_t C, int64_t h, int64_t w);
int dn_upconv_out_fwd(const float *in, const float *weight, const float *bias, float *out, int64_t B, int64_t C, int64_t h,
                      int64_t w, int act, void *workspace, int64_t workspace_bytes, void *stream);
int dn_upconv_out_bwd(const float *in, const float *weight, const float *out, const float *grad_out, float *grad_in,
                      float *grad_weight, float *grad_bias, int64_t B, int64_t C, int64_t h, int64_t w, int act, void *workspace,
                      int64_t workspace_bytes, void *stream);

int64_t dn_upconv3d_out_workspace_bytes(int64_t B, int64_t C, int64_t d, int64_t h, int64_t w);
int dn_upconv3d_out_fwd(const float *in, const float *weight, const float *bias, float *out, int64_t B, int64_t C, int64_t d,
                        int64_t h, int64_t w, int act, void *workspace, int64_t workspace_bytes, void *stream);
int dn_upconv3d_out_bwd(const float *in, const float *weight, const float *out, const float *grad_out, float *grad_in,
                        float *grad_weight, float *grad_bias, int64_t B, int64_t C, int64_t d, int64_t h, int64_t w, int act,
                        void *workspace, int64_t workspace_bytes, void *stream);

int64_t dn_conv3d_k4s2_wrw_workspace_bytes(int64_t B, int64_t CN, int64_t M, int64_t d, int64_t h, int64_t w);
int dn_conv3d_k4s2_wrw(const float *fine, const float *coarse, float *grad_weight, int64_t B, int64_t CN, int64_t M, int64_t d,
                       int64_t h, int64_t w, void *workspace, int64_t workspace_bytes, void *stream);

int64_t dn_instnorm_workspace_bytes(int64_t n_inst, int64_t spatial);
int dn_instnorm_act_fwd(const float *x, float *y, float *mean, float *rstd, int64_t n_inst, int64_t spatial, float eps,
                        float slope, void *workspace, int64_t workspace_bytes, void *stream);
int dn_instnorm_act_bwd(const float *x, const float *mean, const float *rstd, const float *grad_y, float *grad_x,
                        int64_t n_inst, int64_t spatial, float slope, int64_t channels, int64_t grad_y_batch_stride,
                        void *workspace, int64_t workspace_bytes, void *stream);

int dn_conv2d_k4s2_down(const float *fine, const float *w, float *coarse, int64_t B, int64_t C, int64_t M, int64_t H, int64_t W,
                        void *stream);
int dn_conv2d_k4s2_up(const float *coarse, const float *w, float *fine, int64_t B, int64_t C, int64_t M, int64_t H, int64_t W,
                      void *stream);
int64_t dn_conv2d_k4s2_wrw_workspace_bytes(int64_t B, int64_t C, int64_t M, int64_t H, int64_t W);
int dn_conv2d_k4s2_wrw(const float *fine, const float *coarse, float *grad_weight, int64_t B, int64_t C, int64_t M, int64_t H,
                       int64_t W, void *workspace, int64_t workspace_bytes, void *stream);

int dn_conv3d_k4s2_down(const float *fine, const float *w, float *coarse, int64_t B, int64_t C, int64_t M, int64_t D, int64_t H,
                        int64_t W, void *stream);
int dn_conv3d_k4s2_up(const float *coarse, const float *w, float *fine, int64_t B, int64_t C, int64_t M, int64_t D, int64_t H,
                      int64_t W, void *stream);
int64_t dn_conv3d_k4s2_workspace_bytes(int32_t up, int64_t B, int64_t C, int64_t M, int64_t D, int64_t H, int64_t W);
int dn_conv3d_k4s2_down_ws(const float *fine, const float *w, float *coarse, int64_t B, int64_t C, int64_t M, int64_t D, int64_t H,
                           int64_t W, void *workspace, int64_t workspace_bytes, void *stream);
int dn_conv3d_k4s2_up_ws(const float *coarse, const float *w, float *fine, int64_t B, int64_t C, int64_t M, int64_t D, int64_t H,
                         int64_t W, void *workspace, int64_t workspace_bytes, void *stream);

int dn_conv2d_valid_fwd(const float *x, const float *w, const float *bias, float *y, int64_t B, int64_t Ci, int64_t Co, int64_t H, int64_t W,
                        int64_t K, void *stream);
int dn_conv2d_valid_bwd_data(const float *gy, const float *w, float *gx, int64_t B, int64_t Ci, int64_t Co, int64_t H, int64_t W, int64_t K,
                             void *stream);
int dn_conv2d_valid_bwd_weight(const float *x, const float *gy, float *gw, float *gbias, int64_t B, int64_t Ci, int64_t Co, int64_t H, int64_t W,
                               int64_t K, void *stream);

int dn_fdm_fused_fwd(const float *u, float *out, int32_t batch, int32_t ny, int32_t nx, const float *kernel9, int32_t axis, float a,
                     float b, void *stream);
int dn_fdm_fused_bwd(const float *grad_out, float *grad_u, int32_t batch, int32_t ny, int32_t nx, const float *kernel9, int32_t axis,
                     float a, float b, void *stream);

#ifdef __cplusplus
}
#endif
#endif
```

Before: 2706 billion elements*gauss_pts/s.

## Add paired-element packed-math march path for 2-D Q1 closed-form kernel

Adds a PAIRS variant of the 2-D Q1 closed-form Poisson kernel. It processes four elements per thread as two v2f pairs so the element maths can use packed FMA, loads rows with 128-bit (non-temporal for nu/f) vector loads, and writes outputs with a single 128-bit buffer store that is masked through an out-of-range offset. The planner selects this path with 32-row strips when there is enough parallelism, and a config key can disable it. This changes register pressure (launch bounds drop to 2 waves per EU) and the strip geometry, and it adds a plan query API.

```diff
diff --git a/diffnet_amd/_lib.py b/diffnet_amd/_lib.py
--- a/diffnet_amd/_lib.py
+++ b/diffnet_amd/_lib.py
@@ -135,6 +135,7 @@
     "dn_poisson_workspace_bytes": (C.c_int64, [C.POINTER(DnMesh)]),
     "dn_poisson_apply": (C.c_int, [C.POINTER(DnMesh), C.POINTER(DnPoissonArgs), C.c_void_p]),
     "dn_poisson_finish_sums": (C.c_int, [C.POINTER(DnMesh), C.POINTER(DnPoissonArgs), C.c_void_p]),
+    "dn_poisson_plan2d": (C.c_int, [C.POINTER(DnMesh), C.POINTER(DnPoissonArgs), C.POINTER(C.c_int32)]),
     "dn_workspace_status": (C.c_int, [C.c_void_p, C.c_void_p]),
     "dn_gauss_pt_eval_fwd": (C.c_int, [C.c_void_p, C.c_void_p, C.c_void_p, C.c_int32, C.c_int32, I32x3, C.c_int32,
                                        C.c_int32, C.c_int32, C.c_void_p]),
diff --git a/diffnet_amd/csrc/dn_api.hip b/diffnet_amd/csrc/dn_api.hip
--- a/diffnet_amd/csrc/dn_api.hip
+++ b/diffnet_amd/csrc/dn_api.hip
@@ -14,7 +14,7 @@
 }
 
 namespace {
-const char* const kKeys[dn::CFG_COUNT] = {"PLAN2D", "PLAN3D", "PLAN_FSDT", "Q1_RULE_KERNEL", "GPE_GATHER", "GPE_TILED", "Q1_3D_T16", "Q1_3D_E1SUM", "FSDT_GENERIC", "Q1_3D_E1", "HANDOVER_SPIN_LIMIT", "CONV2D_V1", "CONV_WRW_WGS", "Q1_3D_N2", "FSDT_FORM"};
+const char* const kKeys[dn::CFG_COUNT] = {"PLAN2D", "PLAN3D", "PLAN_FSDT", "Q1_RULE_KERNEL", "GPE_GATHER", "GPE_TILED", "Q1_3D_T16", "Q1_3D_E1SUM", "FSDT_GENERIC", "Q1_3D_E1", "HANDOVER_SPIN_LIMIT", "CONV2D_V1", "CONV_WRW_WGS", "Q1_3D_N2", "FSDT_FORM", "Q1_CF_SCALAR"};
 constexpr int kHostCount = 1;
 const char* const kHostKeys[kHostCount] = {"COEF_GRAD"};
 constexpr int kAllCount = dn::CFG_COUNT + kHostCount;
diff --git a/diffnet_amd/csrc/dn_common.h b/diffnet_amd/csrc/dn_common.h
--- a/diffnet_amd/csrc/dn_common.h
+++ b/diffnet_amd/csrc/dn_common.h
@@ -14,7 +14,7 @@
 
 namespace dn {
 
-enum ConfigKey : int { CFG_PLAN2D = 0, CFG_PLAN3D, CFG_PLAN_FSDT, CFG_Q1_RULE_KERNEL, CFG_GPE_GATHER, CFG_GPE_TILED, CFG_Q1_3D_T16, CFG_Q1_3D_E1SUM, CFG_FSDT_GENERIC, CFG_Q1_3D_E1, CFG_HANDOVER_SPIN_LIMIT, CFG_CONV2D_V1, CFG_CONV_WRW_WGS, CFG_Q1_3D_N2, CFG_FSDT_FORM, CFG_COUNT };
+enum ConfigKey : int { CFG_PLAN2D = 0, CFG_PLAN3D, CFG_PLAN_FSDT, CFG_Q1_RULE_KERNEL, CFG_GPE_GATHER, CFG_GPE_TILED, CFG_Q1_3D_T16, CFG_Q1_3D_E1SUM, CFG_FSDT_GENERIC, CFG_Q1_3D_E1, CFG_HANDOVER_SPIN_LIMIT, CFG_CONV2D_V1, CFG_CONV_WRW_WGS, CFG_Q1_3D_N2, CFG_FSDT_FORM, CFG_Q1_CF_SCALAR, CFG_COUNT };
 const char* config(ConfigKey k);
 
 __device__ __forceinline__ double wave_sum(double v) {
diff --git a/diffnet_amd/csrc/poisson2d_q1_cf.hip b/diffnet_amd/csrc/poisson2d_q1_cf.hip
--- a/diffnet_amd/csrc/poisson2d_q1_cf.hip
+++ b/diffnet_amd/csrc/poisson2d_q1_cf.hip
@@ -8,6 +8,7 @@
 
 enum : int { CF_NU = 1, CF_F = 2, CF_BC = 8, CF_BC_U8C = 16, CF_BC_PACKED = 32, CF_PK_NB1 = 64, CF_PK_NB2 = 128, CF_UA = 256, CF_ONE = 512 };
 
+typedef float v4f __attribute__((ext_vector_type(4)));
 template <int E>
 struct CfRow {
     float u[E + 1], n[E + 1], f[E + 1];
@@ -17,8 +18,18 @@
     float keepx;
     BcRaw<E> bc;
     uint32_t m8[2][2];
+    v4f u4, n4, f4;
+    uint32_t mw[2][2];
     uint32_t mb[2];
     uint32_t bx[2];
+};
+
+struct CfRowP {
+    v2f uL[2], uR[2], nL[2], nR[2];
+    v2f gL[2];
+    float g4;
+    v2f du[2], pn[2];
+    v2f keep[2];
 };
 
 constexpr int CF_W = 4;
@@ -49,9 +60,10 @@
     else { static_assert(N == 1, "lds_wait: 1..5 values"); asm volatile("s_waitcnt lgkmcnt(0)" : "+v"(v[0])::"memory"); }
 }
 
-template <int E, bool VEC, int FL, int W>
-__global__ void __launch_bounds__(W > 1 ? CF_TS * W : 256, W > 1 ? 4 : 2) poisson2d_q1_cf_kernel(const PoissonParams p) {
+template <int E, bool VEC, int FL, int W, bool PAIRS = false>
+__global__ void __launch_bounds__(W > 1 ? CF_TS * W : 256, PAIRS ? 2 : (W > 1 ? 4 : 2)) poisson2d_q1_cf_kernel(const PoissonParams p) {
     constexpr int NW = E;
+    static_assert(!PAIRS || (E == 4 && VEC && W == 1 && (FL & (CF_BC | CF_UA)) == 0), "pairs form: four elements per thread, vector accesses, one strip, row-staged");
     constexpr bool HAS_NU = (FL & CF_NU) != 0, HAS_F = (FL & CF_F) != 0;
     constexpr bool BC_ANY = (FL & (CF_BC | CF_BC_U8C | CF_BC_PACKED)) != 0, BC_U8C = (FL & CF_BC_U8C) != 0, BC_PACKED = (FL & CF_BC_PACKED) != 0;
     constexpr bool UA = (FL & CF_UA) != 0, ONE = (FL & CF_ONE) != 0;
@@ -148,7 +160,8 @@
         for (int j = 0; j < NB; ++j) {
             const unsigned ro = (unsigned)yc * brow[j];
             const uint32_t w0 = ld_at<uint32_t>(bptr[j], ro + bw0[j]), w1 = ld_at<uint32_t>(bptr[j], ro + bw1[j]);
-            r.mb[j] = __builtin_amdgcn_alignbit(w1, w0, bsh);
+            if constexpr (PAIRS) { r.mw[j][0] = w0; r.mw[j][1] = w1; }
+            else r.mb[j] = __builtin_amdgcn_alignbit(w1, w0, bsh);
         }
         if constexpr (ONE) {
             if constexpr (NB == 0) r.bx[0] = (yc == (kone ? ylo[1] : ylo[0]) || yc == (kone ? yhi[1] : yhi[0])) ? NBITS : (kone ? boxx[1] : boxx[0]);
@@ -161,9 +174,23 @@
     auto row_issue = [&](int yr, CfRow<E>& r) {
         const int yp = min(yr, p.ny - 1);
         const unsigned rowoff = (unsigned)yp * (unsigned)p.nx;
+        if constexpr (PAIRS) {
+            const unsigned xl = rowoff + (unsigned)min(x0, p.nx - NW), xs = rowoff + (unsigned)min(x0 + NW, p.nx - 1);
+            r.u4 = ld_at<v4f>(sb.u, xl);
+            r.u[NW] = ld_at<float>(sb.u, xs);
+            if constexpr (HAS_NU) {
+                r.n4 = __builtin_nontemporal_load(reinterpret_cast<const v4f*>(reinterpret_cast<const char*>(sb.nu) + xl * 4u));
+                r.n[NW] = ld_at<float>(sb.nu, xs);
+            }
+            if constexpr (HAS_F) {
+                r.f4 = __builtin_nontemporal_load(reinterpret_cast<const v4f*>(reinterpret_cast<const char*>(sb.f) + xl * 4u));
+                r.f[NW] = ld_at<float>(sb.f, xs);
+            }
+        } else {
         load_seg<NW, VEC>(sb.u, rowoff, x0, p.nx, r.u);
         if constexpr (HAS_NU) load_seg_stream<NW, VEC>(sb.nu, rowoff, x0, p.nx, r.n);
         if constexpr (HAS_F) load_seg_stream<NW, VEC>(sb.f, rowoff, x0, p.nx, r.f);
+        }
         if constexpr (BC_PACKED) {
             packed_issue(yp, r);
         } else if constexpr (BC_U8C && ONE) {
@@ -177,7 +204,7 @@
         } else if constexpr (BC_U8C) {
 #pragma unroll
             for (int k = 0; k < 2; ++k) {
-                if (has_mask[k]) {
+                if (PAIRS || has_mask[k]) {
                     uint8_t t[NW + 1];
                     load_seg_stream<NW, VEC>(mask8[k], rowoff, x0, p.nx, t);
                     uint32_t w = 0u;
@@ -260,6 +287,18 @@
             if (pend_st && lastcol) st_at<float>(sb.out, pend_row + (unsigned)(p.nx - 1), pend_x);
         }
         pend_st = false;
+    };
+    typedef unsigned cf_v4u __attribute__((ext_vector_type(4)));
+    constexpr unsigned CF_STORE_NOWHERE = 0x80000000u;
+    __amdgpu_buffer_rsrc_t orsrc;
+    if constexpr (PAIRS) orsrc = __builtin_amdgcn_make_buffer_rsrc(sb.out, (short)0, sb.out != nullptr ? (int)(nps * 4) : 0, 0x00020000);
+    auto flush_store_p = [&]() {
+        if constexpr (PAIRS) {
+            const unsigned off = pend_st ? (pend_row + (unsigned)x0) * 4u : CF_STORE_NOWHERE;
+            const cf_v4u v = {__float_as_uint(pend_v[0]), __float_as_uint(pend_v[1]), __float_as_uint(pend_v[2]), __float_as_uint(pend_v[3])};
+            __builtin_amdgcn_raw_buffer_store_b128(v, orsrc, (int)off, 0, DN_NT_STORES ? 2 : 0);
+            pend_st = false;
+        }
     };
     auto emit_row = [&](const float (&o)[NW + 1], const float (&keep)[NW], int yr, bool owned_row, float keepx = 1.f) {
         float left;
@@ -467,9 +506,158 @@
         }
     };
 
+
+    v2f xmP[2][4], ymP[2][4];
+    if constexpr (PAIRS) {
+#pragma unroll
+        for (int k = 0; k < 2; ++k) {
+            const float v0 = ex0 + 2 * k < p.nelx ? 1.f : 0.f, v1 = ex0 + 2 * k + 1 < p.nelx ? 1.f : 0.f;
+#pragma unroll
+            for (int i = 0; i < 4; ++i) {
+                xmP[k][i] = v2f{v0 != 0.f ? xm[i] : 0.f, v1 != 0.f ? xm[i] : 0.f};
+                ymP[k][i] = v2f{v0 != 0.f ? ym[i] : 0.f, v1 != 0.f ? ym[i] : 0.f};
+            }
+        }
+    }
+    auto pstage = [&](CfRow<E>& r, CfRowP& P) {
+        if constexpr (PAIRS) {
+#pragma unroll
+        for (int j = 0; j < NB; ++j) r.mb[j] = __builtin_amdgcn_alignbit(r.mw[j][1], r.mw[j][0], bsh);
+#pragma unroll
+        for (int n = 0; n < 4; ++n) {
+            r.u[n] = r.u4[n];
+            if constexpr (HAS_NU) r.n[n] = r.n4[n];
+            if constexpr (HAS_F) r.f[n] = r.f4[n];
+        }
+        row_bc(r);
+        fstage(r);
+#pragma unroll
+        for (int k = 0; k < 2; ++k) {
+            P.uL[k] = v2f{r.u[2 * k], r.u[2 * k + 1]};
+            P.uR[k] = v2f{r.u[2 * k + 1], r.u[2 * k + 2]};
+            P.keep[k] = v2f{r.keep[2 * k], r.keep[2 * k + 1]};
+            if constexpr (HAS_NU) {
+                P.nL[k] = v2f{r.n[2 * k], r.n[2 * k + 1]};
+                P.nR[k] = v2f{r.n[2 * k + 1], r.n[2 * k + 2]};
+                q1cf_stage(px0, px1, P.uL[k], P.uR[k], P.nL[k], P.nR[k], P.du[k], P.pn[k]);
+            } else {
+                P.du[k] = P.uR[k] - P.uL[k];
+                P.pn[k] = (v2f)(mx0);
+            }
+            if constexpr (FMASS) P.gL[k] = v2f{r.g[2 * k], r.g[2 * k + 1]};
+        }
+        if constexpr (FMASS) P.g4 = r.g[NW];
+        }
+    };
+    auto emit_row_p = [&](const v2f (&o)[2], float o4, const v2f (&keep)[2], int yr, bool owned_row) {
+        if constexpr (PAIRS) {
+        xch[par][tid] = o4;
+        asm volatile("s_waitcnt lgkmcnt(0)\n\ts_barrier" ::: "memory");
+        const float left = (tid > 0) ? xch[par][tid - 1] : 0.f;
+        par ^= 1;
+        const bool st = owned_row && col_owner;
+        const v2f t0 = (o[0] + v2f{left, 0.f}) * keep[0], t1 = (o[1] + v2f{0.f, 0.f}) * keep[1];
+        const float sq = fmaf(t1.y, t1.y, fmaf(t1.x, t1.x, fmaf(t0.y, t0.y, fmaf(t0.x, t0.x, sq_acc))));
+        sq_acc = st ? sq : sq_acc;
+        const v2f s0 = t0 * p.out_scale, s1 = t1 * p.out_scale;
+        pend_v[0] = s0.x; pend_v[1] = s0.y; pend_v[2] = s1.x; pend_v[3] = s1.y;
+        pend_row = (unsigned)yr * (unsigned)p.nx;
+        pend_st = st && sb.out != nullptr && x0 + NW <= p.nx;
+        }
+    };
+    auto player = [&](int ey, const CfRowP& L, const CfRowP& U, const v2f (&cin)[2], float cin4, v2f (&cout)[2], float& cout4) {
+        const bool own_layer = ey >= e_from && ey <= e_until;
+        const float cnt = (own_layer && col_owner) ? 1.f : 0.f;
+        v2f o[2] = {cin[0], cin[1]};
+        float o4 = cin4, le1 = 0.f, le2 = 0.f;
+        cout[0] = cout[1] = (v2f)(0.f);
+        cout4 = 0.f;
+        if constexpr (FMASS) {
+#pragma unroll
+            for (int k = 0; k < 2; ++k) {
+                const v2f tlo = vfma(cy01, U.gL[k], cy00 * L.gL[k]), tup = vfma(cy11, U.gL[k], cy01 * L.gL[k]);
+                o[k] = vfma(nb, tlo, o[k]);
+                cout[k] = nb * tup;
+                le2 = fmaf(U.uL[k].x, tup.x, fmaf(L.uL[k].x, tlo.x, le2));
+                le2 = fmaf(U.uL[k].y, tup.y, fmaf(L.uL[k].y, tlo.y, le2));
+            }
+            const float tlo = fmaf(cy01, U.g4, cy00 * L.g4), tup = fmaf(cy11, U.g4, cy01 * L.g4);
+            o4 = fmaf(nb, tlo, o4);
+            cout4 = nb * tup;
+            le2 = fmaf(U.uR[1].y, tup, fmaf(L.uR[1].y, tlo, le2));
+        }
+#pragma unroll
+        for (int k = 0; k < 2; ++k) {
+            const v2f V0 = U.uL[k] - L.uL[k], V1 = U.uR[k] - L.uR[k];
+            v2f S0 = (v2f)(my0), S1 = (v2f)(my0);
+            if constexpr (HAS_NU) {
+                S0 = vfma(sy1, U.nL[k], sy0 * L.nL[k]);
+                S1 = vfma(sy1, U.nR[k], sy0 * L.nR[k]);
+            }
+            v2f ta, tb, t0, t1;
+            q1cf_cot(xmP[k], ymP[k], L.du[k], U.du[k], L.pn[k], U.pn[k], V0, V1, S0, S1, ta, tb, t0, t1);
+            q1cf_energy(L.du[k], U.du[k], V0, V1, ta, tb, t0, t1, le1);
+            const v2f dL0 = ta + t0, dL1 = ta - t1, dU0 = t0 - tb, dU1 = tb + t1;
+            o[k].y = fmaf(alpha, dL1.x, o[k].y);
+            cout[k].y = fmaf(alpha, dU1.x, cout[k].y);
+            if (k == 0) {
+                o[1].x = fmaf(alpha, dL1.y, o[1].x);
+                cout[1].x = fmaf(alpha, dU1.y, cout[1].x);
+            } else {
+                o4 = fmaf(alpha, dL1.y, o4);
+                cout4 = fmaf(alpha, dU1.y, cout4);
+            }
+            o[k] = vfma(-alpha, dL0, o[k]);
+            cout[k] = vfma(alpha, dU0, cout[k]);
+        }
+        e1_acc = fmaf(cnt, le1, e1_acc);
+        e2_acc = fmaf(cnt, le2, e2_acc);
+        emit_row_p(o, o4, L.keep, ey, ey >= r_from);
+    };
+    auto pairs_march = [&]() {
+        CfRow<E> W0, W1;
+        CfRowP PA, PB;
+        v2f cA[2] = {(v2f)(0.f), (v2f)(0.f)}, cB[2] = {(v2f)(0.f), (v2f)(0.f)};
+        float cA4 = 0.f, cB4 = 0.f;
+        row_issue(ey_begin, W0);
+        row_issue(min(ey_begin + 1, ey_end), W1);
+        pstage(W0, PA);
+        int ey = ey_begin;
+        bool odd = false;
+        for (; ey + 1 < ey_end; ey += 2) {
+            set_prio(ey);
+            row_issue(min(ey + 2, ey_end), W0);
+            flush_store_p();
+            pstage(W1, PB);
+            player(ey, PA, PB, cA, cA4, cB, cB4);
+            row_issue(min(ey + 3, ey_end), W1);
+            flush_store_p();
+            pstage(W0, PA);
+            player(ey + 1, PB, PA, cB, cB4, cA, cA4);
+        }
+        if (ey < ey_end) {
+            set_prio(ey);
+            flush_store_p();
+            pstage(W1, PB);
+            player(ey, PA, PB, cA, cA4, cB, cB4);
+            odd = true;
+        }
+        flush_store_p();
+        if (top_row) {
+            v2f o[2], keep[2];
+#pragma unroll
+            for (int k = 0; k < 2; ++k) { o[k] = odd ? cB[k] : cA[k]; keep[k] = odd ? PB.keep[k] : PA.keep[k]; }
+            emit_row_p(o, odd ? cB4 : cA4, keep, p.ny - 1, true);
+            flush_store_p();
+        }
+    };
+
     constexpr std::true_type FRESH{};
     constexpr std::false_type LANDED{};
     if (active) {
+    if constexpr (PAIRS) {
+        pairs_march();
+    } else {
     CfRow<E> RA, RB;
     float carryA[NW + 1], carryB[NW + 1];
 #pragma unroll
@@ -535,6 +723,7 @@
         }
     }
     }
+    }
 
     if constexpr (W > 1) {
         e1_acc += spin_poison;
@@ -550,6 +739,12 @@
         if (g.W == CF_W) {
             hipLaunchKernelGGL((poisson2d_q1_cf_kernel<E, VEC, FL, CF_W>), dim3(g.chunks, (g.strips + CF_W - 1) / CF_W, batch),
                                dim3(CF_TS * CF_W), 0, s, pp);
+            return;
+        }
+    }
+    if constexpr (E == 4 && VEC && (FL & (CF_UA | CF_BC)) == 0) {
+        if (g.pairs) {
+            hipLaunchKernelGGL((poisson2d_q1_cf_kernel<E, VEC, FL, 1, true>), dim3(g.chunks, g.strips, batch), dim3(g.T), 0, s, pp);
             return;
         }
     }
diff --git a/diffnet_amd/csrc/poisson_common.h b/diffnet_amd/csrc/poisson_common.h
--- a/diffnet_amd/csrc/poisson_common.h
+++ b/diffnet_amd/csrc/poisson_common.h
@@ -247,7 +247,7 @@
     }
 }
 
-struct Geom2D { int T, E, chunks, strips, R, W = 1; bool ua = false; };
+struct Geom2D { int T, E, chunks, strips, R, W = 1; bool ua = false; bool pairs = false; };
 struct Geom3D { int TX, TY, E, chunks, tiles, strips, R; };
 
 int launch_poisson2d_q1_g2(const PoissonParams& pp, const Geom2D& g, int batch, bool vec, hipStream_t s);
diff --git a/diffnet_amd/csrc/poisson_elem.h b/diffnet_amd/csrc/poisson_elem.h
--- a/diffnet_amd/csrc/poisson_elem.h
+++ b/diffnet_amd/csrc/poisson_elem.h
@@ -4,9 +4,10 @@
 namespace dn {
 
 typedef float v2f __attribute__((ext_vector_type(2)));
-__device__ __forceinline__ float vfma(float a, float b, float c) { return fmaf(a, b, c); }
-__device__ __forceinline__ v2f vfma(v2f a, v2f b, v2f c) { return __builtin_elementwise_fma(a, b, c); }
-__device__ __forceinline__ v2f vfma(float a, v2f b, v2f c) { return __builtin_elementwise_fma((v2f)(a), b, c); }
+__host__ __device__ __forceinline__ float vfma(float a, float b, float c) { return fmaf(a, b, c); }
+__host__ __device__ __forceinline__ v2f vfma(v2f a, v2f b, v2f c) { return __builtin_elementwise_fma(a, b, c); }
+__host__ __device__ __forceinline__ v2f vfma(float a, v2f b, v2f c) { return __builtin_elementwise_fma((v2f)(a), b, c); }
+__host__ __device__ __forceinline__ v2f vfma(v2f a, float b, v2f c) { return __builtin_elementwise_fma(a, (v2f)(b), c); }
 
 struct ElemTab {
     float b[4][4];
@@ -154,21 +155,40 @@
     e2 = a2;
 }
 
-__host__ __device__ __forceinline__ void q1cf_stage(const float px0, const float px1, const float u0, const float u1, const float n0, const float n1,
-                                                    float& du, float& pn) {
+template <typename V, typename C>
+__host__ __device__ __forceinline__ void q1cf_stage(const C px0, const C px1, const V u0, const V u1, const V n0, const V n1, V& du, V& pn) {
     du = u1 - u0;
-    pn = fmaf(px1, n1, px0 * n0);
+    pn = vfma(px1, n1, px0 * n0);
+}
+
+template <typename V, typename C>
+__host__ __device__ __forceinline__ void q1cf_cot(const C (&xm)[4], const C (&ym)[4], const V a, const V b, const V p, const V q, const V V0,
+                                                  const V V1, const V S0, const V S1, V& ta, V& tb, V& t0, V& t1) {
+    const V X0 = vfma(q, xm[1], p * xm[0]), X1 = vfma(q, xm[2], p * xm[1]), X2 = vfma(q, xm[3], p * xm[2]);
+    ta = vfma(b, X1, a * X0);
+    tb = vfma(b, X2, a * X1);
+    const V Y0 = vfma(S1, ym[1], S0 * ym[0]), Y1 = vfma(S1, ym[2], S0 * ym[1]), Y2 = vfma(S1, ym[3], S0 * ym[2]);
+    t0 = vfma(V1, Y1, V0 * Y0);
+    t1 = vfma(V1, Y2, V0 * Y1);
+}
+
+__host__ __device__ __forceinline__ void q1cf_energy(const float a, const float b, const float V0, const float V1, const float ta, const float tb,
+                                                     const float t0, const float t1, float& e) {
+    e = fmaf(b, tb, fmaf(a, ta, e));
+    e = fmaf(V1, t1, fmaf(V0, t0, e));
+}
+__host__ __device__ __forceinline__ void q1cf_energy(const v2f a, const v2f b, const v2f V0, const v2f V1, const v2f ta, const v2f tb, const v2f t0,
+                                                     const v2f t1, float& e) {
+    q1cf_energy(a.x, b.x, V0.x, V1.x, ta.x, tb.x, t0.x, t1.x, e);
+    q1cf_energy(a.y, b.y, V0.y, V1.y, ta.y, tb.y, t0.y, t1.y, e);
 }
 
 __host__ __device__ __forceinline__ void q1cf_elem(const float (&xm)[4], const float (&ym)[4], const float a, const float b, const float p,
                                                    const float q, const float V0, const float V1, const float S0, const float S1,
                                                    const float alpha, float& gL0, float& gL1, float& gU0, float& gU1, float& e) {
-    const float X0 = fmaf(q, xm[1], p * xm[0]), X1 = fmaf(q, xm[2], p * xm[1]), X2 = fmaf(q, xm[3], p * xm[2]);
-    const float ta = fmaf(b, X1, a * X0), tb = fmaf(b, X2, a * X1);
-    const float Y0 = fmaf(S1, ym[1], S0 * ym[0]), Y1 = fmaf(S1, ym[2], S0 * ym[1]), Y2 = fmaf(S1, ym[3], S0 * ym[2]);
-    const float t0 = fmaf(V1, Y1, V0 * Y0), t1 = fmaf(V1, Y2, V0 * Y1);
-    e = fmaf(b, tb, fmaf(a, ta, e));
-    e = fmaf(V1, t1, fmaf(V0, t0, e));
+    float ta, tb, t0, t1;
+    q1cf_cot(xm, ym, a, b, p, q, V0, V1, S0, S1, ta, tb, t0, t1);
+    q1cf_energy(a, b, V0, V1, ta, tb, t0, t1, e);
     gL0 = fmaf(-alpha, ta + t0, gL0);
     gL1 = fmaf(alpha, ta - t1, gL1);
     gU0 = fmaf(alpha, t0 - tb, gU0);
diff --git a/diffnet_amd/csrc/poisson_fused.hip b/diffnet_amd/csrc/poisson_fused.hip
--- a/diffnet_amd/csrc/poisson_fused.hip
+++ b/diffnet_amd/csrc/poisson_fused.hip
@@ -133,7 +133,7 @@
     return logical_threads <= T ? 1 : ceil_div(logical_threads - 1, T - 1);
 }
 
-static Geom2D plan2d(const dn_mesh* m, int P, bool allow_e4 = true, bool chain_ok = false, bool allow_ua = false) {
+static Geom2D plan2d(const dn_mesh* m, int P, bool allow_e4 = true, bool chain_ok = false, bool allow_ua = false, bool pairs_ok = false) {
     Geom2D g;
     const int nx = m->nx, nely = (m->ny - 1) / P;
     const bool ua = allow_ua && P == 1 && (nx & 3) == 1 && nx >= 321;
@@ -167,6 +167,11 @@
         while (Rc < 16 && waves_per_strip * ceil_div(nely, Rc) > 6144) Rc *= 2;
         if (Rc < 16 && ceil_div(nely, Rc) >= cw) { g.R = Rc; g.strips = ceil_div(nely, Rc); g.W = cw; }
     }
+    if (pairs_ok && !ua && P == 1 && g.E == 4 && g.W == 1 && waves_per_strip * ceil_div(nely, 32) >= 2048) {
+        g.R = nely < 32 ? nely : 32;
+        g.strips = ceil_div(nely, g.R);
+        g.pairs = true;
+    }
     return g;
 }
 
@@ -242,8 +247,8 @@
     return g;
 }
 
-static Geom2D plan2d_env(const dn_mesh* m, int P, bool allow_e4 = true, bool chain_ok = false, bool allow_ua = false) {
-    Geom2D g = plan2d(m, P, allow_e4, chain_ok, allow_ua);
+static Geom2D plan2d_env(const dn_mesh* m, int P, bool allow_e4 = true, bool chain_ok = false, bool allow_ua = false, bool pairs_ok = false) {
+    Geom2D g = plan2d(m, P, allow_e4, chain_ok, allow_ua, pairs_ok);
     const char* e = config(CFG_PLAN2D);
     int T, E, R, W = 0;
     if (e && sscanf(e, "%d,%d,%d,%d", &T, &E, &R, &W) >= 3 && T >= 64 && T <= 256 && (E == 1 || E == 2 || E == 4) && R >= 1 &&
@@ -254,6 +259,7 @@
         g.strips = ceil_div(nely, g.R);
         const int cw = poisson2d_q1_cf_chain();
         g.W = (W >= 2 && !g.ua && cw > 1 && P == 1 && E == 4 && T == 128 && g.R + 3 <= 64 && g.R >= 2) ? cw : 1;
+        g.pairs = pairs_ok && !g.ua && P == 1 && E == 4 && g.W == 1;
     }
     return g;
 }
@@ -406,6 +412,34 @@
         if (a->bc[k].mask_kind == DN_MASK_F32 || a->bc[k].mask_kind == DN_MASK_U8)
             ok = ok && aligned(a->bc[k].mask, a->bc[k].mask_kind == DN_MASK_U8 ? NW : 4 * NW) && aligned(a->bc[k].field, 4 * NW);
     return ok;
+}
+
+static bool q1cf_pairs_ok(const dn_mesh* m, const dn_poisson_args* a) {
+    if (m->nsd != 2 || m->degree != 1 || a->f_gp || config(CFG_Q1_RULE_KERNEL) != nullptr || config(CFG_Q1_CF_SCALAR) != nullptr) return false;
+    if (a->strip_select != 0 || !poisson_vec_ok(m, a, 4) || (int64_t)m->nx * m->ny >= (1ll << 29)) return false;
+    for (int k = 0; k < 2; ++k) {
+        const dn_dirichlet& d = a->bc[k];
+        if (d.mask && (d.mask_kind == DN_MASK_F32 || (d.mask_kind == DN_MASK_U8 && d.field))) return false;
+    }
+    return true;
+}
+
+static Geom2D poisson_plan2d(const dn_mesh* m, const dn_poisson_args* a) {
+    const int P = m->degree;
+    const bool chain_ok = P == 1 && a->f_gp == nullptr && config(CFG_Q1_RULE_KERNEL) == nullptr && a->strip_select == 0;
+    const bool cf_kernel = P == 1 && a->f_gp == nullptr && config(CFG_Q1_RULE_KERNEL) == nullptr;
+    Geom2D g = plan2d_env(m, P, poisson_vec_ok(m, a, 4), chain_ok, cf_kernel, q1cf_pairs_ok(m, a));
+    if (!chain_ok) g.W = 1;
+    return g;
+}
+
+extern "C" int dn_poisson_plan2d(const dn_mesh* m, const dn_poisson_args* a, int* out) {
+    const int rc = validate_mesh(m);
+    if (rc) return rc;
+    if (!a || !out || m->nsd != 2) return DN_E_BADARG;
+    const Geom2D g = poisson_plan2d(m, a);
+    out[0] = g.T; out[1] = g.E; out[2] = g.R; out[3] = g.W; out[4] = g.pairs ? 1 : 0;
+    return 0;
 }
 
 extern "C" int dn_poisson_apply(const dn_mesh* m, const dn_poisson_args* a, void* stream) {
@@ -563,10 +597,7 @@
         return 0;
     }
     if (m->nsd == 2) {
-        const bool chain_ok = P == 1 && a->f_gp == nullptr && config(CFG_Q1_RULE_KERNEL) == nullptr && a->strip_select == 0;
-        const bool cf_kernel = P == 1 && a->f_gp == nullptr && config(CFG_Q1_RULE_KERNEL) == nullptr;
-        Geom2D g = plan2d_env(m, P, allow_e4, chain_ok, cf_kernel);
-        if (!chain_ok) g.W = 1;
+        Geom2D g = poisson_plan2d(m, a);
         pp.rows_per_strip = g.R;
         pp.nstrips = g.strips;
         g.strips = launched(g.strips);
@@ -600,10 +631,7 @@
     const bool e4 = poisson_vec_ok(m, a, 4);
     auto sel = [&](int total) { return a->strip_select == 1 ? std::min(total, 2) : (a->strip_select == 2 ? std::max(total - 2, 0) : total); };
     if (m->nsd == 2) {
-        const bool chain_ok = m->degree == 1 && a->f_gp == nullptr && config(CFG_Q1_RULE_KERNEL) == nullptr && a->strip_select == 0;
-        const bool cf_kernel = m->degree == 1 && a->f_gp == nullptr && config(CFG_Q1_RULE_KERNEL) == nullptr;
-        Geom2D g = plan2d_env(m, m->degree, e4, chain_ok, cf_kernel);
-        if (!chain_ok) g.W = 1;
+        const Geom2D g = poisson_plan2d(m, a);
         return (long long)g.chunks * ((sel(g.strips) + g.W - 1) / g.W) * m->batch;
     }
     Geom3D g = plan3d_env(m, q1n2_ok(m, a), q1n2_needed(a));
diff --git a/diffnet_amd/ops.py b/diffnet_amd/ops.py
--- a/diffnet_amd/ops.py
+++ b/diffnet_amd/ops.py
@@ -617,6 +617,11 @@
         if rc:
             _lib.check(rc, "dn_poisson_apply")
         return self.result
+
+    def launch_plan(self):
+        plan = (C.c_int32 * 5)()
+        _lib.check(_lib.lib().dn_poisson_plan2d(self._mesh_ref, self._args_ref, plan), "dn_poisson_plan2d")
+        return tuple(int(v) for v in plan)
 
     def fold(self, prev):
         if prev is None:
diff --git a/include/diffnet_hip.h b/include/diffnet_hip.h
--- a/include/diffnet_hip.h
+++ b/include/diffnet_hip.h
@@ -80,6 +80,7 @@
 int64_t dn_poisson_workspace_bytes(const dn_mesh *mesh);
 int dn_poisson_apply(const dn_mesh *mesh, const dn_poisson_args *args, void *stream);
 int dn_poisson_finish_sums(const dn_mesh *mesh, const dn_poisson_args *args, void *stream);
+int dn_poisson_plan2d(const dn_mesh *mesh, const dn_poisson_args *args, int32_t *plan);
 
 int dn_workspace_status(void *workspace, void *stream);
 
```

Measured after the change: 2577 billion elements*gauss_pts/s. 0.953x the previous value.
